# TropComplique/single-shot-detector

Hardware: AMD Instinct MI355X
Metric: images/sec at 896x640, MobileNet-v1 RetinaNet (whole hot path incl. decode + per-class NMS) (higher is better)
Workload: dtype f32

## Files before the change

single-shot-detector_amd/_lib.py:

```python
import ctypes
import os
import subprocess

_HERE = os.path.dirname(os.path.abspath(__file__))
_CSRC = os.path.join(_HERE, "csrc")
_SOURCES = ["abi.hip", "weights.hip", "plan.hip", "stages.hip", "igemm.hip", "igemm_lat.hip", "igemm16.hip", "dwpw_stream.hip", "sn_pw.hip", "front.hip",
            "elementwise.hip", "postprocess.hip", "loss.hip", "augment.hip", "update.hip", "train_head.hip", "wgrad.hip", "train_backbone.hip"]
_LIB_PATH = os.path.join(_CSRC, "libssd_hip.so")
_DIAG_PATH = os.path.join(_CSRC, "libssd_hip_diag.so")
_lib = None
_diag = False

HIPCC_FLAGS = ["--offload-arch=gfx950", "-O3", "-ffp-contract=off", "-fPIC", "-shared", "-std=c++17"]


class SsdError(RuntimeError):
    """A non-zero return code from libssd_hip.so (message from ssd_last_error())."""


def lib_path():
    return _LIB_PATH


def build(force=False, verbose=False, diag=False):
    srcs = [os.path.join(_CSRC, s) for s in _SOURCES]
    deps = srcs + [os.path.join(_CSRC, "ssd_internal.h"), os.path.join(_CSRC, "host.h"), os.path.join(_CSRC, "igemm_mfma16.h"),
                   os.path.join(_CSRC, "train_head.h"), os.path.join(_CSRC, "first_pixels.h"),
                   os.path.join(_HERE, "..", "include", "ssd_hip.h"),
                   os.path.join(_HERE, "..", "include", "ssd_hip_diag.h"), os.path.join(_CSRC, "exports.map")]
    target = _DIAG_PATH if diag else _LIB_PATH
    import hashlib
    hh = hashlib.sha256(" ".join(HIPCC_FLAGS + (["-DSSD_DIAG"] if diag else [])).encode())
    for d in deps:
        with open(d, "rb") as f:
            hh.update(f.read())
    digest = hh.hexdigest()
    stamp = target + ".sha"
    def fresh():
        if not (os.path.exists(target) and os.path.exists(stamp)):
            return False
        with open(stamp) as f:
            return f.read().strip() == digest
    if not force and fresh():
        return target
    import fcntl
    with open(os.path.join(_CSRC, ".build.lock"), "w") as lock:
        fcntl.flock(lock, fcntl.LOCK_EX)
        try:
            if not force and fresh():
                return target
            hipcc = os.environ.get("HIPCC", "/opt/rocm/bin/hipcc")
            tmp = "%s.tmp.%d" % (target, os.getpid())
            objdir = os.path.join(_CSRC, "build", "diag" if diag else "ship")
            os.makedirs(objdir, exist_ok=True)
            hdrs = deps[len(srcs):]
            cflags = [f for f in HIPCC_FLAGS if f != "-shared"] + (["-DSSD_DIAG"] if diag else [])
            jobs = []
            for src in srcs:
                obj = os.path.join(objdir, os.path.basename(src) + ".o")
                oh = hashlib.sha256(" ".join(cflags).encode())
                for d in [src] + hdrs:
                    with open(d, "rb") as f:
                        oh.update(f.read())
                ostamp, odig = obj + ".sha", oh.hexdigest()
                if force or not os.path.exists(obj) or not os.path.exists(ostamp) or open(ostamp).read().strip() != odig:
                    jobs.append(([hipcc] + cflags + ["-c", src, "-o", obj], ostamp, odig))
            if verbose:
                for j in jobs:
                    print(" ".join(j[0]))
            procs = [subprocess.Popen(j[0]) for j in jobs]
            rcs = [p.wait() for p in procs]
            if any(rcs):
                raise subprocess.CalledProcessError(max(rcs), "hipcc -c")
            for _cmd, ostamp, odig in jobs:
                with open(ostamp, "w") as f:
                    f.write(odig)
            objs = [os.path.join(objdir, os.path.basename(src) + ".o") for src in srcs]
            cmd = [hipcc, "--offload-arch=gfx950", "-shared", "-fPIC", "-Wl,--version-script=" + os.path.join(_CSRC, "exports.map"),
                   "-o", tmp] + objs
            if verbose:
                print(" ".join(cmd))
            subprocess.check_call(cmd)
            ctypes.CDLL(tmp)
            os.replace(tmp, target)
            with open(stamp, "w") as f:
                f.write(digest)
        finally:
            fcntl.flock(lock, fcntl.LOCK_UN)
    return target


_f = ctypes.POINTER(ctypes.c_float)
_i32p = ctypes.POINTER(ctypes.c_int32)
_vp = ctypes.c_void_p
_i = ctypes.c_int32


class SsdConfig(ctypes.Structure):
    _fields_ = [("backbone", ctypes.c_int32), ("depth_multiplier", ctypes.c_float),
                ("num_classes", ctypes.c_int32), ("score_threshold", ctypes.c_float),
                ("iou_threshold", ctypes.c_float), ("max_boxes_per_class", ctypes.c_int32),
                ("min_dimension", ctypes.c_int32), ("device", ctypes.c_int32)]


class SsdLossConfig(ctypes.Structure):
    _fields_ = [("alpha", ctypes.c_double), ("gamma", ctypes.c_float), ("positives_threshold", ctypes.c_float),
                ("negatives_threshold", ctypes.c_float), ("n_levels", ctypes.c_int32),
                ("anchors_per_level", ctypes.c_int64 * 8)]


class SsdUpdateTensor(ctypes.Structure):
    _fields_ = [("w", ctypes.c_void_p), ("grad", ctypes.c_void_p), ("m", ctypes.c_void_p), ("v", ctypes.c_void_p),
                ("ema", ctypes.c_void_p), ("count", ctypes.c_int64), ("decay", ctypes.c_int32), ("first_block", ctypes.c_int32)]


class SsdUpdateScalars(ctypes.Structure):
    _fields_ = [("alpha", ctypes.c_float), ("one_minus_beta1", ctypes.c_float), ("one_minus_beta2", ctypes.c_float),
                ("epsilon", ctypes.c_float), ("weight_decay", ctypes.c_float), ("one_minus_decay", ctypes.c_float)]


class SsdConvLevel(ctypes.Structure):
    _fields_ = [("H", ctypes.c_int32), ("W", ctypes.c_int32), ("x", ctypes.c_void_p), ("dy", ctypes.c_void_p), ("out", ctypes.c_void_p)]


class SsdBnLevel(ctypes.Structure):
    _fields_ = [("rows", ctypes.c_int64)] + [(n, ctypes.c_void_p) for n in (
        "x", "dy", "out", "gamma", "beta", "moving_mean", "moving_variance", "mean", "var", "invstd", "dgamma", "dbeta")]


SIGNATURES = {
    "ssd_create": (ctypes.c_int, [ctypes.POINTER(SsdConfig), ctypes.POINTER(_vp)]),
    "ssd_destroy": (None, [_vp]),
    "ssd_last_error": (ctypes.c_char_p, []),
    "ssd_load_weight": (ctypes.c_int, [_vp, ctypes.c_char_p, _f, ctypes.POINTER(ctypes.c_int64), _i]),
    "ssd_finalize": (ctypes.c_int, [_vp]),
    "ssd_forward": (ctypes.c_int, [_vp, _vp, _i, _i, _i, _vp, _vp, _vp, _vp, _vp]),
    "ssd_record_words": (ctypes.c_int32, [_vp]),
    "ssd_forward_records": (ctypes.c_int, [_vp, _vp, _i, _i, _i, _vp, _vp]),
    "ssd_forward_host": (ctypes.c_int, [_vp, _vp, _i, _i, _i, _vp, _vp]),
    "ssd_network_shape": (ctypes.c_int, [_vp, _i, _i, _i32p]),
    "ssd_forward_mixed": (ctypes.c_int, [_vp, _vp, _i, _i32p, ctypes.POINTER(ctypes.c_int64), _vp, _vp]),
    "ssd_forward_mixed_host": (ctypes.c_int, [_vp, ctypes.POINTER(ctypes.c_void_p), _i, _i32p, _vp, _vp]),
    "ssd_detect_host": (ctypes.c_int, [_vp, _vp, _i, _i, ctypes.c_float, _vp, _vp, _vp, _vp, _i, _i32p, _vp]),
    "ssd_get_tensor": (ctypes.c_int, [_vp, ctypes.c_char_p, _f, ctypes.c_int64, _i32p]),
    "ssd_get_tensor_dev": (ctypes.c_int, [_vp, ctypes.c_char_p, _vp, ctypes.c_int64, _i32p, _vp]),
    "ssd_plan_cache_stats": (ctypes.c_int, [_vp, ctypes.POINTER(ctypes.c_int64)]),
    "ssd_plan_cache_clear": (ctypes.c_int, [_vp]),
    "ssd_profile_enable": (ctypes.c_int, [_vp, _i]),
    "ssd_profile_read": (ctypes.c_int, [_vp, _i, ctypes.POINTER(ctypes.c_double),
                                        ctypes.POINTER(ctypes.c_int64),
                                        ctypes.POINTER(ctypes.c_double),
                                        ctypes.POINTER(ctypes.c_double)]),
    "ssd_profile_reset": (ctypes.c_int, [_vp]),
    "ssd_num_anchors": (ctypes.c_int32, [_i, _i]),
    "ssd_anchors": (ctypes.c_int, [_i, _i, _f]),
    "ssd_anchors_ex": (ctypes.c_int64, [_i, _i, _i, _i32p, ctypes.POINTER(ctypes.c_double), _i, ctypes.POINTER(ctypes.c_double),
                                        _i, ctypes.POINTER(ctypes.c_double), _f, ctypes.c_int64]),
    "ssd_conv2d": (ctypes.c_int, [_vp, _i, _i, _i, _i, _f, _i, _i, _i, _i, _i, _i, _f, _f, _f, _f,
                                  _vp, _i, _vp, _vp]),
    "ssd_conv2d_f16x3": (ctypes.c_int, [_vp, _i, _i, _i, _i, _f, _i, _i, _i, _i, _i, _i, _f, _f, _f, _f,
                                        _vp, _i, _vp, _vp]),
    "ssd_set_option": (ctypes.c_int, [_vp, ctypes.c_char_p, _i]),
    "ssd_get_option": (ctypes.c_int, [_vp, ctypes.c_char_p, _i32p]),
    "ssd_set_precision": (ctypes.c_int, [_vp, _i]),
    "ssd_get_precision": (ctypes.c_int, [_vp]),
    "ssd_status": (ctypes.c_int, [_vp, _i32p]),
    "ssd_depthwise3x3": (ctypes.c_int, [_vp, _i, _i, _i, _i, _f, _i, _i, _i, _i, _f, _f, _f, _i,
                                        _vp, _vp]),
    "ssd_dw_pw": (ctypes.c_int, [_vp, _i, _i, _i, _i, _f, _i, _f, _f, _f, _i, _f, _i, _f, _f, _f, _i, _vp, _vp]),
    "ssd_first_conv": (ctypes.c_int, [_vp, _i, _i, _i, _f, _i, _f, _f, _f, _i, _vp, _vp]),
    "ssd_front_block": (ctypes.c_int, [_vp, _i, _i, _i, _f, _i, _f, _f, _f, _i, _f, _f, _f, _f, _i, _f, _i, _f, _f, _f, _i, _vp, _vp]),
    "ssd_first_conv_maxpool": (ctypes.c_int, [_vp, _i, _i, _i, _f, _i, _f, _f, _f, _i, _vp, _vp]),
    "ssd_maxpool3x3s2": (ctypes.c_int, [_vp, _i, _i, _i, _i, _vp, _vp]),
    "ssd_concat_shuffle_split": (ctypes.c_int, [_vp, _vp, ctypes.c_int64, _i, _vp, _vp, _vp]),
    "ssd_shuffle_conv1x1": (ctypes.c_int, [_vp, _vp, ctypes.c_int64, _i, _f, _i, _f, _f, _f, _i, _vp, _vp]),
    "ssd_postprocess_workspace_bytes": (ctypes.c_size_t, [_i, _i, _i, _i]),
    "ssd_postprocess": (ctypes.c_int, [_vp, _vp, _vp, _i, _i, _i, ctypes.c_float, ctypes.c_float,
                                       _i, _f, _vp, _vp, _vp, _vp, _vp, ctypes.c_size_t, _vp]),
    "ssd_loss_workspace_bytes": (ctypes.c_size_t, [_i, _i, _i]),
    "ssd_training_targets": (ctypes.c_int, [_vp, _i, _vp, _vp, _vp, _i, _i, ctypes.POINTER(SsdLossConfig),
                                            _vp, _vp, _vp, _vp, ctypes.c_size_t, _vp]),
    "ssd_loss": (ctypes.c_int, [_vp, _vp, _vp, _i, _i, _i, _vp, _vp, _vp, _i, ctypes.POINTER(SsdLossConfig),
                                _vp, _vp, _vp, _vp, _vp, ctypes.c_size_t, _vp]),
    "ssd_loss_backward": (ctypes.c_int, [_vp, _vp, _i, _i, _i, _vp, _vp, _vp, _vp, _i, ctypes.POINTER(SsdLossConfig),
                                         _vp, _vp, _vp, _vp]),
    "ssd_augment": (ctypes.c_int, [_vp, _vp, _vp, _i, _i, _i, _i, _vp, _vp]),
    "ssd_train_update": (ctypes.c_int, [_vp, _vp, _i, ctypes.POINTER(SsdUpdateScalars), _vp]),
    "ssd_conv3x3_train_workspace_bytes": (ctypes.c_size_t, [ctypes.POINTER(SsdConvLevel), _i, _i, _i, _i]),
    "ssd_conv3x3_train_forward": (ctypes.c_int, [ctypes.POINTER(SsdConvLevel), _i, _i, _i, _i, _vp, _vp, _vp, ctypes.c_size_t, _vp]),
    "ssd_conv3x3_train_backward": (ctypes.c_int, [ctypes.POINTER(SsdConvLevel), _i, _i, _i, _i, _vp, _vp, _vp, _vp, ctypes.c_size_t, _vp]),
    "ssd_bn_relu_train_workspace_bytes": (ctypes.c_size_t, [ctypes.POINTER(SsdBnLevel), _i, _i]),
    "ssd_bn_relu_train_forward": (ctypes.c_int, [ctypes.POINTER(SsdBnLevel), _i, _i, _i, ctypes.c_float, ctypes.c_float, _vp,
                                                 ctypes.c_size_t, _vp]),
    "ssd_bn_relu_train_backward": (ctypes.c_int, [ctypes.POINTER(SsdBnLevel), _i, _i, _vp, ctypes.c_size_t, _vp]),
    "ssd_conv_train_workspace_bytes": (ctypes.c_size_t, [ctypes.POINTER(SsdConvLevel), _i, _i, _i, _i, _i, _i, _i]),
    "ssd_conv_train_forward": (ctypes.c_int, [ctypes.POINTER(SsdConvLevel), _i, _i, _i, _i, _i, _i, _vp, _vp, ctypes.POINTER(_vp), _vp,
                                              ctypes.c_size_t, _vp]),
    "ssd_conv_train_backward": (ctypes.c_int, [ctypes.POINTER(SsdConvLevel), _i, _i, _i, _i, _i, _i, _vp, _vp, _vp, _vp, ctypes.c_size_t, _vp]),
    "ssd_fpn_merge_backward": (ctypes.c_int, [_vp, _vp, _vp, _i, _i, _i, _i, _i, _vp, _vp]),
    "ssd_depthwise_train_forward": (ctypes.c_int, [_vp, _i, _i, _i, _i, _vp, _i, _vp, _vp]),
    "ssd_depthwise_train_workspace_bytes": (ctypes.c_size_t, [_i, _i, _i, _i, _i]),
    "ssd_depthwise_train_backward": (ctypes.c_int, [_vp, _vp, _i, _i, _i, _i, _vp, _i, _vp, _vp, _vp, ctypes.c_size_t, _vp]),
    "ssd_pointwise_train_workspace_bytes": (ctypes.c_size_t, [ctypes.POINTER(SsdConvLevel), _i, _i, _i, _i]),
    "ssd_pointwise_train_backward": (ctypes.c_int, [ctypes.POINTER(SsdConvLevel), _i, _i, _i, _i, _vp, _vp, _vp, ctypes.c_size_t, _vp]),
    "ssd_bn_act_train_forward": (ctypes.c_int, [ctypes.POINTER(SsdBnLevel), _i, _i, _i, _i, ctypes.c_float, ctypes.c_float, _vp,
                                                ctypes.c_size_t, _vp]),
    "ssd_bn_act_train_backward": (ctypes.c_int, [ctypes.POINTER(SsdBnLevel), _i, _i, _i, _vp, ctypes.c_size_t, _vp]),
    "ssd_first_conv_train_forward": (ctypes.c_int, [_vp, _i, _i, _i, _vp, _i, _vp, _vp]),
    "ssd_first_conv_train_workspace_bytes": (ctypes.c_size_t, [_i, _i, _i, _i]),
    "ssd_first_conv_train_backward": (ctypes.c_int, [_vp, _vp, _i, _i, _i, _i, _vp, _vp, ctypes.c_size_t, _vp]),
}


DIAG_SIGNATURES = {
    "ssd_bench_conv": (ctypes.c_int, [_i, _i, _i, _i, _i, _i, _i, _i, _i, _i,
                                      ctypes.POINTER(ctypes.c_double), ctypes.POINTER(ctypes.c_double)]),
    "ssd_bench_dwpw": (ctypes.c_int, [_i, _i, _i, _i, _i, _i, _i, _i, ctypes.POINTER(ctypes.c_double)]),
}


def use_diag():
    global _diag
    if _lib is not None and not _diag:
        raise RuntimeError("use_diag() after libssd_hip.so was loaded")
    _diag = True


def lib():
    global _lib
    if _lib is None:
        target = _DIAG_PATH if _diag else _LIB_PATH
        try:
            path = build(diag=_diag)
        except (FileNotFoundError, subprocess.CalledProcessError, OSError) as e:
            if not os.path.exists(target):
                raise RuntimeError("single-shot-detector_amd: %s is missing and cannot be built here (%r); there is no "
                                   "fallback" % (os.path.basename(target), e)) from e
            import warnings
            warnings.warn("single-shot-detector_amd: loading the existing %s without a freshness check (%r)"
                          % (os.path.basename(target), e))
            path = target
        _lib = ctypes.CDLL(path)
        sigs = dict(SIGNATURES, **DIAG_SIGNATURES) if _diag else SIGNATURES
        for name, (res, args) in sigs.items():
            fn = getattr(_lib, name)
            fn.restype = res
            fn.argtypes = args
    return _lib


def set_option(key, value, handle=None):
    check(lib().ssd_set_option(handle, key.encode(), int(value)))


def get_option(key, handle=None):
    v = ctypes.c_int32()
    check(lib().ssd_get_option(handle, key.encode(), ctypes.byref(v)))
    return v.value


def check(rc):
    if rc != 0:
        msg = lib().ssd_last_error()
        raise SsdError("libssd_hip error %d: %s" % (rc, msg.decode() if msg else "?"))
```

single-shot-detector_amd/csrc/abi.hip:

```cpp
#include "host.h"

#include <algorithm>
#include <cmath>
#include <cstdio>
#include <cstring>

static thread_local std::string g_err;
int ssd_fail(int code, const std::string &msg) { g_err = msg; return code; }
extern "C" const char *ssd_last_error(void) { return g_err.c_str(); }

static Options g_opts;
static std::mutex g_opts_mu;
static const char *const OPT_NAMES[OPT_COUNT] = {"streams", "h2d_chunks", "front_fuse", "fuse_dw", "backbone_split", "event_fence", "plan_cache_mb",
                                                 "igemm_tile", "igemm16", "igemm_96", "igemm_lat", "igemm_deep64", "lateral_split", "fpn_group", "fpn_p7_group",
                                                 "fpn_early_lat", "nsub", "nms_fast_max", "first_conv_px", "debug_sync"};
int ssd_opt_index(const char *key)
{
    for (int i = 0; i < OPT_COUNT; ++i)
        if (key && !strcmp(key, OPT_NAMES[i])) return i;
    return -1;
}
int ssd_opt(const ssd_handle *h, int key, int dflt)
{
    if (h && h->opts.v[key] != SSD_OPT_UNSET) return h->opts.v[key];
    const int g = g_opts.v[key];
    return g != SSD_OPT_UNSET ? g : dflt;
}
unsigned ssd_sync_event_flags(const ssd_handle *h)
{
    return hipEventDisableTiming | (ssd_opt(h, OPT_EVENT_FENCE, 0) ? 0u : (unsigned)hipEventDisableSystemFence);
}
int nms_fast_max(const ssd_handle *h)
{
    const int v = ssd_opt(h, OPT_NMS_FAST_MAX, -1);
    return v < 0 ? 0 : (v == 0 ? -1 : v);
}

static int make_handle_events(ssd_handle *h)
{
    if (h->ev_last) { (void)hipEventDestroy(h->ev_last); h->ev_last = nullptr; }
    HIPCHK(hipEventCreateWithFlags(&h->ev_last, ssd_sync_event_flags(h)));
    h->have_last = false;
    return SSD_OK;
}

extern "C" int ssd_set_option(ssd_handle *h, const char *key, int32_t value)
{
    const int k = ssd_opt_index(key);
    if (k < 0) return ssd_fail(SSD_ERR_INVALID, std::string("ssd_set_option: unknown option ") + (key ? key : "(null)"));
    if (k == OPT_IGEMM_TILE && !(value == SSD_OPT_UNSET || value == 0 || value == 64 || value == 128 || igemm_is_lat(value)))
        return ssd_fail(SSD_ERR_INVALID, "ssd_set_option: igemm_tile must be 0 (auto), 128, 64 or a wave tile of igemm_lat.hip (20 .. 27, 30)");
    if (k == OPT_PLAN_CACHE_MB && value < 0 && value != SSD_OPT_UNSET) return ssd_fail(SSD_ERR_INVALID, "ssd_set_option: plan_cache_mb must be >= 0");
    if (!h) {
        std::lock_guard<std::mutex> g(g_opts_mu);
        g_opts.v[k] = value;
        return SSD_OK;
    }
    std::lock_guard<std::mutex> g(h->mu);
    if (h->opts.v[k] == value) return SSD_OK;
    HIPCHK(hipSetDevice(h->cfg.device));
    if (k == OPT_PLAN_CACHE_MB) {
        h->opts.v[k] = value;
        return trim_plan_cache(h, h->cur);
    }
    HIPCHK(hipDeviceSynchronize());
    free_plans(h);
    h->opts.v[k] = value;
    if (k == OPT_EVENT_FENCE) SSDCHK(make_handle_events(h));
    return SSD_OK;
}

extern "C" int ssd_get_option(ssd_handle *h, const char *key, int32_t *value)
{
    const int k = ssd_opt_index(key);
    if (k < 0 || !value) return ssd_fail(SSD_ERR_INVALID, "ssd_get_option: unknown option or null argument");
    *value = ssd_opt(h, k, SSD_OPT_UNSET);
    return SSD_OK;
}

extern "C" int ssd_create(const ssd_config *cfg, ssd_handle **out)
{
    if (!cfg || !out) return ssd_fail(SSD_ERR_INVALID, "ssd_create: null argument");
    if (cfg->backbone != SSD_BACKBONE_MOBILENET && cfg->backbone != SSD_BACKBONE_SHUFFLENET)
        return ssd_fail(SSD_ERR_INVALID, "ssd_create: unknown backbone");
    if (cfg->num_classes < 1 || cfg->max_boxes_per_class < 1)
        return ssd_fail(SSD_ERR_INVALID, "ssd_create: num_classes and max_boxes_per_class must be >= 1");
    int ndev = 0;
    HIPCHK(hipGetDeviceCount(&ndev));
    if (cfg->device < 0 || cfg->device >= ndev) return ssd_fail(SSD_ERR_INVALID, "ssd_create: no such HIP device");
    HIPCHK(hipSetDevice(cfg->device));
    ssd_handle *h = new ssd_handle();
    h->cfg = *cfg;
    if (make_handle_events(h) != SSD_OK) {
        if (h->ev_last) (void)hipEventDestroy(h->ev_last);
        delete h;
        return ssd_fail(SSD_ERR_HIP, "ssd_create: cannot create events");
    }
    if (hipMalloc((void **)&h->flags_dev, sizeof(int)) != hipSuccess || hipMemset(h->flags_dev, 0, sizeof(int)) != hipSuccess) {
        delete h;
        return ssd_fail(SSD_ERR_HIP, "ssd_create: cannot allocate the status word");
    }
    if (const char *e = getenv("SSD_PRECISION")) {
        if (!strcmp(e, "f16x3")) h->precision = SSD_PRECISION_F16X3;
        else if (!strcmp(e, "f32")) h->precision = SSD_PRECISION_F32;
        else { (void)hipFree(h->flags_dev); delete h; return ssd_fail(SSD_ERR_INVALID, "SSD_PRECISION must be f32 or f16x3"); }
    }
    *out = h;
    return SSD_OK;
}

extern "C" int ssd_set_precision(ssd_handle *h, int32_t mode)
{
    if (!h || (mode != SSD_PRECISION_F32 && mode != SSD_PRECISION_F16X3)) return ssd_fail(SSD_ERR_INVALID, "ssd_set_precision: bad arguments");
    std::lock_guard<std::mutex> g(h->mu);
    if (mode == h->precision) return SSD_OK;
    HIPCHK(hipSetDevice(h->cfg.device));
    HIPCHK(hipDeviceSynchronize());
    free_plans(h);
    h->precision = mode;
    return SSD_OK;
}

extern "C" int ssd_get_precision(ssd_handle *h)
{
    if (!h) return SSD_ERR_INVALID;
    std::lock_guard<std::mutex> g(h->mu);
    return h->precision;
}

extern "C" int ssd_status(ssd_handle *h, int32_t *flags_out)
{
    if (!h || !flags_out) return ssd_fail(SSD_ERR_INVALID, "ssd_status: null argument");
    std::lock_guard<std::mutex> g(h->mu);
    HIPCHK(hipSetDevice(h->cfg.device));
    HIPCHK(hipDeviceSynchronize());
    int v = 0;
    HIPCHK(hipMemcpy(&v, h->flags_dev, sizeof(int), hipMemcpyDeviceToHost));
    if (v) HIPCHK(hipMemset(h->flags_dev, 0, sizeof(int)));
    *flags_out = v;
    return SSD_OK;
}

extern "C" void ssd_destroy(ssd_handle *h)
{
    if (!h) return;
    (void)hipSetDevice(h->cfg.device);
    (void)hipDeviceSynchronize();
    for (auto &e : h->evs) { (void)hipEventDestroy(e.a); (void)hipEventDestroy(e.b); }
    for (auto r : h->ref_evs) (void)hipEventDestroy(r);
    for (auto r : h->ev_pool) (void)hipEventDestroy(r);
    free_plans(h);
    if (h->ev_last) (void)hipEventDestroy(h->ev_last);
    if (h->ev_stage) (void)hipEventDestroy(h->ev_stage);
    if (h->stage_pin) (void)hipHostFree(h->stage_pin);
    if (h->stage_dev) (void)hipFree(h->stage_dev);
    if (h->flags_dev) (void)hipFree(h->flags_dev);
    h->wpool.free_all();
    delete h;
}

extern "C" int ssd_load_weight(ssd_handle *h, const char *name, const float *host, const int64_t *shape, int32_t ndim)
{
    if (!h || !name || !host || !shape || ndim < 1 || ndim > 4) return ssd_fail(SSD_ERR_INVALID, "ssd_load_weight: bad arguments");
    std::lock_guard<std::mutex> g(h->mu);
    if (h->finalized) return ssd_fail(SSD_ERR_STATE, "ssd_load_weight after ssd_finalize");
    Tensor t;
    int64_t n = 1;
    for (int i = 0; i < ndim; ++i) {
        if (shape[i] < 1) return ssd_fail(SSD_ERR_INVALID, "ssd_load_weight: non-positive dimension");
        t.shape.push_back(shape[i]);
        n *= shape[i];
    }
    t.data.assign(host, host + n);
    h->vars[name] = std::move(t);
    return SSD_OK;
}

extern "C" int ssd_finalize(ssd_handle *h)
{
    if (!h) return ssd_fail(SSD_ERR_INVALID, "ssd_finalize: null handle");
    std::lock_guard<std::mutex> g(h->mu);
    if (h->finalized) return ssd_fail(SSD_ERR_STATE, "ssd_finalize called twice");
    HIPCHK(hipSetDevice(h->cfg.device));
    SSDCHK(finalize_weights(h));
    h->vars.clear();
    h->finalized = true;
    return SSD_OK;
}

struct MixedSel { const MixedCall *mx; int netH, netW; long long max_bytes; };
struct Outputs { float *boxes; int32_t *labels; float *scores; int32_t *num_boxes; long long stride; };

static int forward_locked(ssd_handle *h, const uint8_t *images_dev, int32_t B, int32_t H, int32_t W, const Outputs &o, hipStream_t s,
                          const MixedSel *ms = nullptr)
{
    HIPCHK(hipSetDevice(h->cfg.device));
    if (ms) SSDCHK(select_plans_net(h, B, ms->netH, ms->netW, 0, ms->max_bytes));
    else SSDCHK(select_plans(h, B, H, W));
    if (h->have_last && h->last_stream != s) {
        if (!h->multi_stream) {
            h->multi_stream = true;
            hipStreamCaptureStatus cs = hipStreamCaptureStatusNone;
            const bool known = hipStreamIsCapturing(h->last_stream, &cs) == hipSuccess;
            if (known && cs == hipStreamCaptureStatusNone && hipEventRecord(h->ev_last, h->last_stream) == hipSuccess)
                HIPCHK(hipStreamWaitEvent(s, h->ev_last, 0));
            else { (void)hipGetLastError(); HIPCHK(hipDeviceSynchronize()); }
        } else {
            hipStreamCaptureStatus cs = hipStreamCaptureStatusNone;
            if (hipStreamIsCapturing(s, &cs) != hipSuccess) { (void)hipGetLastError(); cs = hipStreamCaptureStatusNone; }
            if (cs != hipStreamCaptureStatusNone)
                return ssd_fail(SSD_ERR_STATE, "ssd_forward: this handle's previous forward ran on another stream; a capturing stream cannot wait "
                                               "for it -- synchronise that stream (or use one handle per captured stream) before capturing");
            HIPCHK(hipStreamWaitEvent(s, h->ev_last, 0));
        }
        h->have_last = false;
    }
    h->mixed = ms ? ms->mx : nullptr;
    const int rc = enqueue_forward(h, images_dev, o.boxes, o.labels, o.scores, o.num_boxes, o.stride, s);
    h->mixed = nullptr;
    return rc;
}

static int forward_checked_locked(ssd_handle *h, const uint8_t *images_dev, int32_t B, int32_t H, int32_t W, const Outputs &o, void *stream,
                                  const MixedSel *ms = nullptr)
{
    if (!h->finalized) return ssd_fail(SSD_ERR_STATE, "ssd_forward before ssd_finalize");
    if (B < 1 || H < 1 || W < 1 || h->cfg.min_dimension < 128 || h->cfg.min_dimension % 128)
        return ssd_fail(SSD_ERR_INVALID, "ssd_forward: B, H, W must be positive and min_dimension a multiple of 128 (pipeline.py:152)");
    {
        const ResizeDims rd = resize_dims(H, W, h->cfg.min_dimension, 128);
        if ((long long)(rd.nh + rd.ph) * (rd.nw + rd.pw) > (1LL << 26))
            return ssd_fail(SSD_ERR_INVALID, "ssd_forward: aspect ratio too extreme (resized image exceeds 64 Mpixel)");
    }
    hipStream_t s = (hipStream_t)stream;
    const int rc = forward_locked(h, images_dev, B, H, W, o, s, ms);
    if (rc == SSD_OK) {
        hipStreamCaptureStatus cs = hipStreamCaptureStatusNone;
        if (hipStreamIsCapturing(s, &cs) != hipSuccess) { (void)hipGetLastError(); cs = hipStreamCaptureStatusNone; }
        if (cs == hipStreamCaptureStatusNone) {
            h->last_stream = s;
            h->have_last = true;
            if (h->multi_stream) HIPCHK(hipEventRecord(h->ev_last, s));
        }
    }
    return rc;
}

static int forward_checked(ssd_handle *h, const uint8_t *images_dev, int32_t B, int32_t H, int32_t W, const Outputs &o, void *stream)
{
    if (!h || !images_dev || !o.boxes || !o.labels || !o.scores || !o.num_boxes)
        return ssd_fail(SSD_ERR_INVALID, "ssd_forward: null argument");
    std::lock_guard<std::mutex> g(h->mu);
    return forward_checked_locked(h, images_dev, B, H, W, o, stream);
}

extern "C" int ssd_forward(ssd_handle *h, const uint8_t *images_dev, int32_t B, int32_t H, int32_t W, float *boxes_dev,
                           int32_t *labels_dev, float *scores_dev, int32_t *num_boxes_dev, void *stream)
{
    return forward_checked(h, images_dev, B, H, W, {boxes_dev, labels_dev, scores_dev, num_boxes_dev, 0}, stream);
}

extern "C" int32_t ssd_record_words(const ssd_handle *h)
{
    return h ? 6 * h->cfg.num_classes * h->cfg.max_boxes_per_class + 1 : 0;
}

static Outputs record_outputs(const ssd_handle *h, void *records)
{
    const long long T = (long long)h->cfg.num_classes * h->cfg.max_boxes_per_class;
    int32_t *r = (int32_t *)records;
    return {(float *)r, r + 5 * T, (float *)(r + 4 * T), r + 6 * T, 6 * T + 1};
}

extern "C" int ssd_forward_records(ssd_handle *h, const uint8_t *images_dev, int32_t B, int32_t H, int32_t W, void *records_dev, void *stream)
{
    if (!h || !records_dev) return ssd_fail(SSD_ERR_INVALID, "ssd_forward_records: null argument");
    if ((reinterpret_cast<uintptr_t>(records_dev) & 3) != 0) return ssd_fail(SSD_ERR_INVALID, "ssd_forward_records: records must be 4-byte aligned");
    return forward_checked(h, images_dev, B, H, W, record_outputs(h, records_dev), stream);
}

static int stage_acquire(ssd_handle *h)
{
    if (!h->stage_busy) return SSD_OK;
    const hipError_t e = h->stage_by_event && h->ev_stage ? hipEventSynchronize(h->ev_stage) : hipStreamSynchronize(h->stage_stream);
    if (e != hipSuccess) { (void)hipGetLastError(); HIPCHK(hipDeviceSynchronize()); }
    h->stage_busy = false;
    return SSD_OK;
}
static int stage_release(ssd_handle *h, hipStream_t s, bool by_event)
{
    if (by_event) {
        if (!h->ev_stage) HIPCHK(hipEventCreateWithFlags(&h->ev_stage, hipEventDisableTiming));
        hipStreamCaptureStatus cs = hipStreamCaptureStatusNone;
        if (hipStreamIsCapturing(s, &cs) != hipSuccess) { (void)hipGetLastError(); cs = hipStreamCaptureStatusNone; }
        if (cs == hipStreamCaptureStatusNone) HIPCHK(hipEventRecord(h->ev_stage, s));
        else by_event = false;
    }
    h->stage_stream = s;
    h->stage_stream_set = true;
    h->stage_by_event = by_event;
    h->stage_busy = true;
    return SSD_OK;
}

static int grow_stage(ssd_handle *h, size_t bytes)
{
    if (bytes <= h->stage_bytes) return SSD_OK;
    size_t cap = (size_t)2 << 20;
    while (cap < bytes) cap <<= 1;
    HIPCHK(hipDeviceSynchronize());
    if (h->stage_pin) { (void)hipHostFree(h->stage_pin); h->stage_pin = nullptr; }
    if (h->stage_dev) { (void)hipFree(h->stage_dev); h->stage_dev = nullptr; }
    h->stage_bytes = 0;
    HIPCHK(hipHostMalloc((void **)&h->stage_pin, cap + 256, hipHostMallocDefault));
    HIPCHK(hipMalloc((void **)&h->stage_dev, cap + 256));
    h->stage_bytes = cap;
    return SSD_OK;
}

static int stage_begin(ssd_handle *h, hipStream_t s, size_t bytes)
{
    SSDCHK(stage_acquire(h));
    if (h->stage_stream_set && h->stage_stream != s) {
        if (hipStreamSynchronize(h->stage_stream) != hipSuccess) { (void)hipGetLastError(); HIPCHK(hipDeviceSynchronize()); }
    }
    return grow_stage(h, bytes);
}

static int forward_host_impl(ssd_handle *h, const uint8_t *images_host, int32_t B, int32_t H, int32_t W, void *records, void *stream, bool stage_event)
{
    if (!h || !images_host || !records) return ssd_fail(SSD_ERR_INVALID, "ssd_forward_host: null argument");
    if (B < 1 || H < 1 || W < 1) return ssd_fail(SSD_ERR_INVALID, "ssd_forward_host: B, H, W must be positive");
    if ((reinterpret_cast<uintptr_t>(records) & 3) != 0) return ssd_fail(SSD_ERR_INVALID, "ssd_forward_host: records must be 4-byte aligned");
    std::lock_guard<std::mutex> g(h->mu);
    HIPCHK(hipSetDevice(h->cfg.device));
    hipStream_t s = (hipStream_t)stream;
    const size_t bytes = (size_t)B * H * W * 3;
    SSDCHK(stage_begin(h, s, bytes));
    int nchunk = ssd_opt(h, OPT_H2D_CHUNKS, 2);
    if (nchunk < 1) nchunk = 1;
    if (nchunk > 16) nchunk = 16;
    if (bytes < ((size_t)1 << 20)) nchunk = 1;
    const size_t step = ((bytes + nchunk - 1) / nchunk + 4095) & ~(size_t)4095;
    for (size_t lo = 0; lo < bytes; lo += step) {
        const size_t n = bytes - lo < step ? bytes - lo : step;
        memcpy(h->stage_pin + lo, images_host + lo, n);
        HIPCHK(hipMemcpyAsync(h->stage_dev + lo, h->stage_pin + lo, n, hipMemcpyHostToDevice, s));
    }
    SSDCHK(stage_release(h, s, stage_event));
    return forward_checked_locked(h, h->stage_dev, B, H, W, record_outputs(h, records), stream);
}

extern "C" int ssd_forward_host(ssd_handle *h, const uint8_t *images_host, int32_t B, int32_t H, int32_t W, void *records, void *stream)
{
    return forward_host_impl(h, images_host, B, H, W, records, stream, true);
}

static int prepare_mixed(ssd_handle *h, int32_t B, const int32_t *hw, const int64_t *offsets, MixedSel *ms, const char *who)
{
    if (B < 1 || B > SSD_MIXED_MAX)
        return ssd_fail(SSD_ERR_INVALID, std::string(who) + ": 1 .. " + std::to_string(SSD_MIXED_MAX) + " frames per mixed-size batch");
    if (h->cfg.min_dimension < 128 || h->cfg.min_dimension % 128) return ssd_fail(SSD_ERR_INVALID, std::string(who) + ": min_dimension must be a multiple of 128");
    MixedCall &mc = h->mixed_store;
    long long off = 0, max_bytes = 0;
    ms->mx = &mc; ms->netH = ms->netW = 0;
    for (int b = 0; b < B; ++b) {
        const int H = hw[2 * b], W = hw[2 * b + 1];
        if (H < 1 || W < 1) return ssd_fail(SSD_ERR_INVALID, std::string(who) + ": frame sizes must be positive");
        const ResizeDims rd = resize_dims(H, W, h->cfg.min_dimension, 128);
        const int nH = rd.nh + rd.ph, nW = rd.nw + rd.pw;
        if ((long long)nH * nW > (1LL << 26)) return ssd_fail(SSD_ERR_INVALID, std::string(who) + ": aspect ratio too extreme (resized image exceeds 64 Mpixel)");
        if (b == 0) { ms->netH = nH; ms->netW = nW; }
        else if (nH != ms->netH || nW != ms->netW)
            return ssd_fail(SSD_ERR_INVALID, std::string(who) + ": frame " + std::to_string(b) + " (" + std::to_string(H) + " x " + std::to_string(W) + ") resizes to " +
                                             std::to_string(nH) + " x " + std::to_string(nW) + ", frame 0 to " + std::to_string(ms->netH) + " x " +
                                             std::to_string(ms->netW) + ": the frames of one batch must share the network shape (group them by ssd_network_shape)");
        const long long bytes = (long long)H * W * 3;
        const long long o = offsets ? offsets[b] : off;
        if (o < 0 || o + bytes >= (1LL << 31)) return ssd_fail(SSD_ERR_INVALID, std::string(who) + ": the frames of a batch must lie within 2 GiB of the base pointer");
        FrameGeom &g = mc.geom.f[b];
        g.off = (unsigned)o; g.srcH = H; g.srcW = W; g.nh = rd.nh; g.nw = rd.nw;
        g.hs = (float)H / (float)rd.nh; g.ws = (float)W / (float)rd.nw;
        mc.scaler[b][0] = rd.box_scaler[0]; mc.scaler[b][1] = rd.box_scaler[1];
        off = o + ((bytes + 15) & ~15LL);
        max_bytes = bytes > max_bytes ? bytes : max_bytes;
    }
    ms->max_bytes = max_bytes;
    return SSD_OK;
}

extern "C" int ssd_network_shape(ssd_handle *h, int32_t height, int32_t width, int32_t *net_hw)
{
    if (!h || !net_hw || height < 1 || width < 1) return ssd_fail(SSD_ERR_INVALID, "ssd_network_shape: bad arguments");
    if (h->cfg.min_dimension < 128 || h->cfg.min_dimension % 128) return ssd_fail(SSD_ERR_INVALID, "ssd_network_shape: min_dimension must be a multiple of 128");
    const ResizeDims rd = resize_dims(height, width, h->cfg.min_dimension, 128);
    net_hw[0] = rd.nh + rd.ph; net_hw[1] = rd.nw + rd.pw;
    return SSD_OK;
}

extern "C" int ssd_forward_mixed(ssd_handle *h, const uint8_t *images_dev, int32_t B, const int32_t *hw_host, const int64_t *offsets_host,
                                 void *records_dev, void *stream)
{
    if (!h || !images_dev || !hw_host || !records_dev) return ssd_fail(SSD_ERR_INVALID, "ssd_forward_mixed: null argument");
    if ((reinterpret_cast<uintptr_t>(records_dev) & 3) != 0) return ssd_fail(SSD_ERR_INVALID, "ssd_forward_mixed: records must be 4-byte aligned");
    std::lock_guard<std::mutex> g(h->mu);
    MixedSel ms;
    SSDCHK(prepare_mixed(h, B, hw_host, offsets_host, &ms, "ssd_forward_mixed"));
    return forward_checked_locked(h, images_dev, B, hw_host[0], hw_host[1], record_outputs(h, records_dev), stream, &ms);
}

extern "C" int ssd_forward_mixed_host(ssd_handle *h, const uint8_t *const *frames_host, int32_t B, const int32_t *hw_host, void *records, void *stream)
{
    if (!h || !frames_host || !hw_host || !records) return ssd_fail(SSD_ERR_INVALID, "ssd_forward_mixed_host: null argument");
    if ((reinterpret_cast<uintptr_t>(records) & 3) != 0) return ssd_fail(SSD_ERR_INVALID, "ssd_forward_mixed_host: records must be 4-byte aligned");
    std::lock_guard<std::mutex> g(h->mu);
    MixedSel ms;
    SSDCHK(prepare_mixed(h, B, hw_host, nullptr, &ms, "ssd_forward_mixed_host"));
    for (int b = 0; b < B; ++b)
        if (!frames_host[b]) return ssd_fail(SSD_ERR_INVALID, "ssd_forward_mixed_host: null frame pointer");
    HIPCHK(hipSetDevice(h->cfg.device));
    hipStream_t s = (hipStream_t)stream;
    const MixedCall &mc = h->mixed_store;
    const size_t bytes = (size_t)mc.geom.f[B - 1].off + (size_t)hw_host[2 * (B - 1)] * hw_host[2 * (B - 1) + 1] * 3;
    SSDCHK(stage_begin(h, s, bytes));
    for (int b = 0; b < B; ++b) {
        const size_t n = (size_t)hw_host[2 * b] * hw_host[2 * b + 1] * 3, lo = mc.geom.f[b].off;
        memcpy(h->stage_pin + lo, frames_host[b], n);
        HIPCHK(hipMemcpyAsync(h->stage_dev + lo, h->stage_pin + lo, n, hipMemcpyHostToDevice, s));
    }
    SSDCHK(stage_release(h, s, true));
    return forward_checked_locked(h, h->stage_dev, B, hw_host[0], hw_host[1], record_outputs(h, records), stream, &ms);
}

extern "C" int ssd_detect_host(ssd_handle *h, const uint8_t *image_host, int32_t H, int32_t W, float score_threshold, void *record,
                               float *boxes_out, int32_t *labels_out, float *scores_out, int32_t capacity, int32_t *n_out, void *stream)
{
    if (!h || !record || !boxes_out || !labels_out || !scores_out || !n_out || capacity < 0) return ssd_fail(SSD_ERR_INVALID, "ssd_detect_host: bad arguments");
    {
        std::lock_guard<std::mutex> g(h->mu);
        bool known = false;
        for (int i = 0; i < h->n_rec_ok; ++i) known = known || h->detect_rec_ok[i] == record;
        if (!known) {
            HIPCHK(hipSetDevice(h->cfg.device));
            hipPointerAttribute_t at;
            memset(&at, 0, sizeof(at));
            const hipError_t pe = hipPointerGetAttributes(&at, record);
            if (pe != hipSuccess) (void)hipGetLastError();
            const bool host_visible = pe == hipSuccess && (at.type == hipMemoryTypeHost || at.type == hipMemoryTypeManaged || at.isManaged);
            if (!host_visible)
                return ssd_fail(SSD_ERR_INVALID, "ssd_detect_host: `record` must be pinned (hipHostMalloc / hipHostRegister) or managed host memory -- "
                                                 "a device pointer or pageable memory cannot be written by the GPU and read by this call");
            h->detect_rec_ok[h->n_rec_ok < 8 ? h->n_rec_ok++ : (h->rec_ok_next++ & 7)] = record;
        }
    }
    int rc = forward_host_impl(h, image_host, 1, H, W, record, stream, false);
    if (rc != SSD_OK) return rc;
    HIPCHK(hipStreamSynchronize((hipStream_t)stream));
    const Outputs r = record_outputs(h, record);
    const long long T = (r.stride - 1) / 6;
    const int32_t n = *r.num_boxes;
    if (n < 0 || n > T) return ssd_fail(SSD_ERR_STATE, "ssd_detect_host: the record's num_boxes is out of range (is `record` host-visible memory?)");
    int32_t k = 0;
    for (int32_t i = 0; i < n; ++i)
        if (r.scores[i] > score_threshold) {
            if (k >= capacity) return ssd_fail(SSD_ERR_INVALID, "ssd_detect_host: capacity too small");
            memcpy(boxes_out + 4 * (size_t)k, r.boxes + 4 * (size_t)i, 16);
            labels_out[k] = r.labels[i];
            scores_out[k] = r.scores[i];
            ++k;
        }
    *n_out = k;
    return SSD_OK;
}

extern "C" int ssd_get_tensor(ssd_handle *h, const char *name, float *dst, int64_t cap, int32_t *dims)
{
    if (!h || !name || !dst || !dims) return ssd_fail(SSD_ERR_INVALID, "ssd_get_tensor: null argument");
    std::lock_guard<std::mutex> g(h->mu);
    if (!h->cur) return ssd_fail(SSD_ERR_STATE, "ssd_get_tensor before ssd_forward");
    HIPCHK(hipSetDevice(h->cfg.device));
    HIPCHK(hipDeviceSynchronize());
    long long done = 0;
    int Btot = 0;
    for (Plan *pl : h->cur->plans) {
        auto it = pl->retained.find(name);
        if (it == pl->retained.end()) return ssd_fail(SSD_ERR_INVALID, std::string("ssd_get_tensor: unknown tensor ") + name);
        const Retained &r = it->second;
        const long long rows = (long long)r.B * r.H * r.W;
        if (cap < done + rows * r.C) return ssd_fail(SSD_ERR_INVALID, "ssd_get_tensor: destination too small");
        std::vector<float> tmp((size_t)rows * r.Cp);
        HIPCHK(hipMemcpy(tmp.data(), r.dev, tmp.size() * sizeof(float), hipMemcpyDeviceToHost));
        for (long long q = 0; q < rows; ++q)
            for (int c = 0; c < r.C; ++c) {
                const int pc = !r.permuted ? c : (r.split > 0 ? twopart_phys(c, r.split, r.Cp / 2) : ssd_phys_of_logical(c));
                if (r.fmt) {
                    const _Float16 *row = (const _Float16 *)&tmp[q * r.Cp];
                    dst[done + q * r.C + c] = (float)row[(pc >> 3) * 16 + (pc & 7)] + (float)row[(pc >> 3) * 16 + 8 + (pc & 7)];
                } else {
                    dst[done + q * r.C + c] = tmp[q * r.Cp + pc];
                }
            }
        done += rows * r.C;
        Btot += r.B;
        dims[1] = r.H; dims[2] = r.W; dims[3] = r.C;
    }
    dims[0] = Btot;
    return SSD_OK;
}

extern "C" int ssd_get_tensor_dev(ssd_handle *h, const char *name, float *dst_dev, int64_t cap, int32_t *dims, void *stream)
{
    if (!h || !name || !dst_dev || !dims) return ssd_fail(SSD_ERR_INVALID, "ssd_get_tensor_dev: null argument");
    std::lock_guard<std::mutex> g(h->mu);
    if (!h->cur) return ssd_fail(SSD_ERR_STATE, "ssd_get_tensor_dev before ssd_forward");
    HIPCHK(hipSetDevice(h->cfg.device));
    long long done = 0;
    int Btot = 0;
    for (Plan *pl : h->cur->plans) {
        auto it = pl->retained.find(name);
        if (it == pl->retained.end()) return ssd_fail(SSD_ERR_INVALID, std::string("ssd_get_tensor_dev: unknown tensor ") + name);
        const Retained &r = it->second;
        const long long rows = (long long)r.B * r.H * r.W;
        if (cap < done + rows * r.C) return ssd_fail(SSD_ERR_INVALID, "ssd_get_tensor_dev: destination too small");
        if (r.permuted) HIPCHK(launch_permute_channels(r.dev, rows, r.C, r.Cp, r.fmt ? 2 : 0, dst_dev + done, (hipStream_t)stream, r.fmt ? 0 : r.split));
        else HIPCHK(hipMemcpyAsync(dst_dev + done, r.dev, (size_t)rows * r.C * sizeof(float), hipMemcpyDeviceToDevice, (hipStream_t)stream));
        done += rows * r.C;
        Btot += r.B;
        dims[1] = r.H; dims[2] = r.W; dims[3] = r.C;
    }
    dims[0] = Btot;
    return SSD_OK;
}

extern "C" int ssd_plan_cache_stats(ssd_handle *h, int64_t *out)
{
    if (!h || !out) return ssd_fail(SSD_ERR_INVALID, "ssd_plan_cache_stats: null argument");
    std::lock_guard<std::mutex> g(h->mu);
    HIPCHK(hipSetDevice(h->cfg.device));
    size_t total = 0;
    for (const PlanSet *ps : h->cache) total += ps->bytes;
    out[0] = (int64_t)h->cache.size();
    out[1] = (int64_t)total;
    out[2] = (int64_t)plan_cache_limit_bytes(h);
    out[3] = h->cache_hits; out[4] = h->cache_misses; out[5] = h->cache_evictions;
    out[6] = h->cur ? h->cur->key.netH : 0;
    out[7] = h->cur ? h->cur->key.netW : 0;
    return SSD_OK;
}

extern "C" int ssd_plan_cache_clear(ssd_handle *h)
{
    if (!h) return ssd_fail(SSD_ERR_INVALID, "ssd_plan_cache_clear: null handle");
    std::lock_guard<std::mutex> g(h->mu);
    HIPCHK(hipSetDevice(h->cfg.device));
    HIPCHK(hipDeviceSynchronize());
    h->cache_evictions += (long long)h->cache.size();
    free_plans(h);
    h->n_rec_ok = 0;
    return SSD_OK;
}

extern "C" int ssd_profile_enable(ssd_handle *h, int32_t on)
{
    if (!h) return ssd_fail(SSD_ERR_INVALID, "null handle");
    std::lock_guard<std::mutex> g(h->mu);
    h->profiling = on != 0;
    return SSD_OK;
}

static int drain_events(ssd_handle *h)
{
    std::vector<std::vector<std::pair<float, float>>> iv(SSD_NCLS);
    int cur_fwd = -1;
    auto flush = [&]() {
        for (int c = 0; c < SSD_NCLS; ++c) {
            auto &v = iv[c];
            std::sort(v.begin(), v.end());
            float lo = 0, hi = -1;
            for (auto &p : v) {
                if (hi < 0) { lo = p.first; hi = p.second; }
                else if (p.first <= hi) { if (p.second > hi) hi = p.second; }
                else { h->acc_ms[c] += hi - lo; lo = p.first; hi = p.second; }
            }
            if (hi >= 0) h->acc_ms[c] += hi - lo;
            v.clear();
        }
    };
    for (auto &e : h->evs) {
        HIPCHK(hipEventSynchronize(e.b));
        if (e.fwd != cur_fwd) { flush(); cur_fwd = e.fwd; }
        float t0 = 0, t1 = 0;
        if (e.fwd >= 0 && e.fwd < (int)h->ref_evs.size()) {
            HIPCHK(hipEventElapsedTime(&t0, h->ref_evs[e.fwd], e.a));
            HIPCHK(hipEventElapsedTime(&t1, h->ref_evs[e.fwd], e.b));
        } else {
            HIPCHK(hipEventElapsedTime(&t1, e.a, e.b));
        }
        iv[e.cls].push_back({t0, t1});
        h->ev_pool.push_back(e.a);
        h->ev_pool.push_back(e.b);
    }
    flush();
    h->evs.clear();
    for (auto r : h->ref_evs) h->ev_pool.push_back(r);
    h->ref_evs.clear();
    return SSD_OK;
}

extern "C" int ssd_profile_read(ssd_handle *h, int32_t cls, double *total_ms, int64_t *launches, double *flops, double *bytes)
{
    if (!h || cls < 0 || cls >= SSD_NCLS) return ssd_fail(SSD_ERR_INVALID, "ssd_profile_read: bad arguments");
    std::lock_guard<std::mutex> g(h->mu);
    SSDCHK(drain_events(h));
    if (total_ms) *total_ms = h->acc_ms[cls];
    if (launches) *launches = h->acc_n[cls];
    if (flops) *flops = h->acc_flops[cls];
    if (bytes) *bytes = h->acc_bytes[cls];
    return SSD_OK;
}

extern "C" int ssd_profile_reset(ssd_handle *h)
{
    if (!h) return ssd_fail(SSD_ERR_INVALID, "null handle");
    std::lock_guard<std::mutex> g(h->mu);
    SSDCHK(drain_events(h));
    for (int i = 0; i < SSD_NCLS; ++i) { h->acc_ms[i] = h->acc_flops[i] = h->acc_bytes[i] = 0; h->acc_n[i] = 0; }
    return SSD_OK;
}
```

single-shot-detector_amd/csrc/host.h:

```cpp
#pragma once
#include "../../include/ssd_hip.h"
#include "ssd_internal.h"

#include <climits>
#include <functional>
#include <map>
#include <mutex>
#include <string>
#include <vector>

int ssd_fail(int code, const std::string &msg);
#define HIPCHK(expr)                                                                         \
    do {                                                                                     \
        hipError_t e_ = (expr);                                                              \
        if (e_ != hipSuccess)                                                                \
            return ssd_fail(SSD_ERR_HIP, std::string(#expr) + ": " + hipGetErrorString(e_)); \
    } while (0)
#define SSDCHK(expr)                                                                         \
    do {                                                                                     \
        int r_ = (expr);                                                                     \
        if (r_ != SSD_OK) return r_;                                                         \
    } while (0)

enum SsdOpt {
    OPT_STREAMS = 0,
    OPT_H2D_CHUNKS,
    OPT_FRONT_FUSE,
    OPT_FUSE_DW,
    OPT_BACKBONE_SPLIT,
    OPT_EVENT_FENCE,
    OPT_PLAN_CACHE_MB,
    OPT_IGEMM_TILE,
    OPT_IGEMM16,
    OPT_IGEMM_96,
    OPT_IGEMM_LAT,
    OPT_IGEMM_DEEP64,
    OPT_LATERAL_SPLIT,
    OPT_FPN_GROUP,
    OPT_FPN_P7_GROUP,
    OPT_FPN_EARLY_LAT,
    OPT_NSUB,
    OPT_NMS_FAST_MAX,
    OPT_FIRST_CONV_PX,
    OPT_DEBUG_SYNC,
    OPT_COUNT
};
#define SSD_OPT_UNSET INT_MIN
struct Options { int v[OPT_COUNT]; Options() { for (int &x : v) x = SSD_OPT_UNSET; } };
int ssd_opt(const struct ssd_handle *h, int key, int dflt);
int ssd_opt_index(const char *key);
unsigned ssd_sync_event_flags(const struct ssd_handle *h);

struct Tensor {
    std::vector<int64_t> shape;
    std::vector<float> data;
};

struct DevPool {
    std::vector<void *> ptrs;
    size_t bytes = 0;
    int alloc(void **out, size_t nbytes)
    {
        HIPCHK(hipMalloc(out, nbytes + 256));
        ptrs.push_back(*out);
        bytes += nbytes + 256;
        return SSD_OK;
    }
    template <class T> int upload(T **out, const std::vector<T> &v)
    {
        void *p = nullptr;
        SSDCHK(alloc(&p, v.size() * sizeof(T)));
        if (!v.empty()) HIPCHK(hipMemcpy(p, v.data(), v.size() * sizeof(T), hipMemcpyHostToDevice));
        *out = (T *)p;
        return SSD_OK;
    }
    void free_all()
    {
        for (void *p : ptrs) (void)hipFree(p);
        ptrs.clear();
        bytes = 0;
    }
};

static inline int round_up(int v, int m) { return (v + m - 1) / m * m; }

std::vector<int> phys_map(int C, int Cp);
std::vector<int> ident_map(int C, int Cp);
std::vector<int> twopart_map(int D, int Dp);
static inline int twopart_phys(int c, int D, int Dp) { return c < D ? ssd_phys_of_logical(c) : Dp + ssd_phys_of_logical(c - D); }

struct BnHost { std::vector<float> mean, sf, beta; };

struct ConvW {
    float *wt = nullptr, *mean = nullptr, *sf = nullptr, *beta = nullptr, *bias = nullptr;
    float *wlat = nullptr;
    float *wt16 = nullptr;
    float *wt16w = nullptr;
    int CoutPad16 = 0;
    float scale16 = 1.0f;
    int CinP = 0, CoutP = 0, CoutPad = 0, taps = 1, tile = IGEMM_128x128;
    int Cin_l = 0, Cout_l = 0;
};

struct DwW {
    float *w = nullptr, *mean = nullptr, *sf = nullptr, *beta = nullptr;
    float *pack = nullptr;
    int Cp = 0;
};

#define SSD_NCLS 8
#define SSD_FUSE_DW_DEFAULT 0xfu
#define SSD_FUSE_SHUFFLE_DEFAULT true
#ifdef SSD_DIAG
extern int g_force_tile;
extern long long *g_dbg_ts;
#else
static constexpr int g_force_tile = -1;
static constexpr long long *g_dbg_ts = nullptr;
#endif

std::vector<float> permute_rows(const float *w, int rows, int C, const std::vector<int> &map);
BnHost permute_bn(const float *mean, const float *sf, const float *beta, const std::vector<int> &map,
                  BnHost o = BnHost());
void conv_geometry(const struct ssd_handle *h, int taps, int CinP, int CoutP, int Cin_l, int Cout_l, ConvW &cw);
int pack_conv(const struct ssd_handle *h, DevPool &pool, const float *w, int k, int Cin_l, int Cout_l, const std::vector<int> &inmap,
              const std::vector<int> &outmap, ConvW &cw);
int upload_bn(DevPool &pool, const BnHost &b, ConvW &cw);
int upload_dw(DevPool &pool, const std::vector<float> &w, const BnHost &b, DwW &d);
int pack_dw(DevPool &pool, const std::vector<float> &w9, const BnHost &b, DwW &d);
int finalize_weights(struct ssd_handle *h);

struct Op {
    int cls;
    int stream = 0;
    std::vector<int> deps;
    hipEvent_t done = nullptr;
    double flops, bytes;
    std::function<hipError_t(hipStream_t)> run;
};

struct LevelDesc {
    int H, W, OH, OW;
    long long in_off, out_off, out_bstride;
    int out_rstride, param_off;
    long long res_off;
    long long wt_off = 0;
    int stride = 0, pad = -1;
};

struct ConvIO {
    const float *in = nullptr;
    float *out = nullptr;
    float *out2 = nullptr;
    const float *res = nullptr;
    int in_fmt = 0, out_fmt = 0, res_fmt = 0;
    int *flags = nullptr;
};
Op make_conv_op(const struct ssd_handle *h, const ConvW &cw, const ConvIO &io, int B, int stride, int pad, int act,
                const std::vector<LevelDesc> &lv, bool dense, unsigned *scan_bits = nullptr, float scan_lo = 0.0f,
                bool *scan_marked = nullptr);
Op make_dw_op(const DwW &d, const float *in, int B, int H, int W, int stride, int act, float *out, int Cl, int out16 = 0,
              int *flags = nullptr);
bool dwpws_eligible(const DwW &d, const ConvW &cw, int B, int H, int W, int stride);
Op make_dwpws_op(const DwW &d, const ConvW &cw, const float *in, int B, int H, int W, int stride, int dact, int act,
                 float *out, int out_rs = 0 );
Op make_pw_gather_op(const ConvW &cw, const float *base, long long base_bytes, const int *src, int rs, long long M, int act, float *out);
LevelDesc dense_level(int H, int W, int OH, int OW, int CoutP, long long in_off = 0, long long out_off = 0,
                      int param_off = 0, long long res_off = 0);
float conservative_logit_bound(float thr);
int nms_fast_max(const struct ssd_handle *h);

struct ResizeDims { int nh, nw, ph, pw; float box_scaler[4]; };
ResizeDims resize_dims(int height, int width, int min_dimension, int divisor);
extern const int A_STRIDES[5];
extern const int MB_STRIDE[13];

struct Retained { const float *dev; int B, H, W, C, Cp; bool permuted; int fmt = 0;
                  int split = 0;  };

struct EvPair { hipEvent_t a, b; int cls; int fwd; };

struct Plan {
    int B = 0, img0 = 0, N = 0;
    DevPool pool;
    std::vector<Op> ops;
    PostArgs post;
    std::map<std::string, Retained> retained;
    hipStream_t s_aux = nullptr;
    hipStream_t s_bb[2] = {nullptr, nullptr};
    hipEvent_t ev_join = nullptr, ev_begin = nullptr;
    bool need_begin = false;
};

struct SrcGeom { int srcH = 0, srcW = 0, nh = 0, nw = 0; float box_scaler[4] = {1, 1, 1, 1}; };

struct MixedCall { MixedGeom geom; float scaler[SSD_MIXED_MAX][2]; };

struct PlanKey {
    int B = 0, netH = 0, netW = 0, ident = 0, nsub = 0;
    bool operator==(const PlanKey &o) const { return B == o.B && netH == o.netH && netW == o.netW && ident == o.ident && nsub == o.nsub; }
};
struct PlanSet {
    PlanKey key;
    std::vector<Plan *> plans;
    size_t bytes = 0;
    unsigned long long last_use = 0;
};

struct ssd_handle {
    ssd_config cfg;
    std::mutex mu;
    Options opts;
    std::map<std::string, Tensor> vars;
    bool finalized = false;
    DevPool wpool;
    DwW first;
    int firstCp = 0, firstAct = SSD_ACT_RELU6;
    std::vector<DwW> dw;
    std::vector<ConvW> pw;
    ConvW lat[3], pconv[5];
    ConvW pgroup;
    ConvW tower[2][4], final_[2];
    int c_ch[3] = {0, 0, 0};
    int c_split[3] = {0, 0, 0};
    struct SnStage { int pw = 0, dw = 0, units = 0; };
    SnStage sn_stage[3];
    int precision = SSD_PRECISION_F32;
    int *flags_dev = nullptr;
    std::vector<PlanSet *> cache;
    PlanSet *cur = nullptr;
    unsigned long long use_clock = 0;
    long long cache_hits = 0, cache_misses = 0, cache_evictions = 0;
    const uint8_t *cur_images = nullptr;
    SrcGeom src;
    const MixedCall *mixed = nullptr;
    MixedCall mixed_store;
    hipStream_t last_stream = nullptr;
    bool have_last = false;
    bool multi_stream = false;
    hipEvent_t ev_last = nullptr;
    const void *detect_rec_ok[8] = {nullptr};
    int n_rec_ok = 0, rec_ok_next = 0;
    uint8_t *stage_pin = nullptr, *stage_dev = nullptr;
    size_t stage_bytes = 0;
    hipStream_t stage_stream = nullptr;
    bool stage_busy = false, stage_stream_set = false;
    bool stage_by_event = false;
    hipEvent_t ev_stage = nullptr;
    bool profiling = false;
    std::vector<EvPair> evs;
    std::vector<hipEvent_t> ref_evs;
    std::vector<hipEvent_t> ev_pool;
    double acc_ms[SSD_NCLS] = {0}, acc_flops[SSD_NCLS] = {0}, acc_bytes[SSD_NCLS] = {0};
    long long acc_n[SSD_NCLS] = {0};
};

void free_plans(ssd_handle *h);
int select_plans(ssd_handle *h, int B, int H, int W);
int select_plans_net(ssd_handle *h, int B, int netH, int netW, int ident, long long max_src_bytes);
int trim_plan_cache(ssd_handle *h, const PlanSet *keep);
size_t plan_cache_limit_bytes(const ssd_handle *h);
int enqueue_forward(ssd_handle *h, const uint8_t *images_dev, float *boxes_dev, int32_t *labels_dev, float *scores_dev,
                    int32_t *num_boxes_dev, long long out_stride, hipStream_t s);
```

single-shot-detector_amd/csrc/plan.hip:

```cpp
#include "host.h"
#include <chrono>

#include <algorithm>
#include <cmath>
#include <cstdio>
#include <cstring>

Op make_conv_op(const ssd_handle *h, const ConvW &cw, const ConvIO &io, int B, int stride, int pad, int act,
                const std::vector<LevelDesc> &lv, bool dense, unsigned *scan_bits, float scan_lo, bool *scan_marked)
{
    const float *in = io.in, *res = io.res;
    float *out = io.out, *out2 = io.out2;
    const int in_fmt = io.in_fmt, out_fmt = io.out_fmt, res_fmt = io.res_fmt;
    int *flags = io.flags;
    IgemmArgs a;
    memset(&a, 0, sizeof(a));
    a.in = in; a.wt = in_fmt ? cw.wt16 : cw.wt; a.out = out; a.out2 = out2;
    a.wt_lat = in_fmt ? nullptr : cw.wlat;
    a.in_fmt = in_fmt; a.out_fmt = out_fmt; a.res_fmt = res ? res_fmt : 0;
    a.acc_scale = in_fmt ? cw.scale16 : 1.0f;
    a.flags = flags;
    a.mean = cw.mean; a.sf = cw.sf; a.beta = cw.beta; a.bias = cw.bias; a.res = res;
    a.B = B; a.Cin = cw.CinP; a.Cout = cw.CoutP; a.CoutPad = cw.CoutPad; a.taps = cw.taps;
    a.stride = stride; a.pad = pad; a.act = act;
// ... 450 lines not shown
}

struct StageGeo { int ch, cw, oh, ow, D, Dp, n_units; long long tbytes[2], toff[2], soff, total; };

static void sn_stage_geo(const ssd_handle *h, int H, int W, const int nb[2], StageGeo geo[3])
{
    int ch = H / 2 / 2, cw = W / 2 / 2;
    for (int st = 0; st < 3; ++st) {
        StageGeo &g = geo[st];
        g.ch = ch; g.cw = cw; g.oh = ch / 2; g.ow = cw / 2; g.n_units = h->sn_stage[st].units;
        const ConvW &after = h->pw[h->sn_stage[st].pw + 1];
        g.Dp = after.CoutP; g.D = after.Cout_l;
        long long off = 0;
        for (int c = 0; c < 2; ++c) {
            g.tbytes[c] = (long long)nb[c] * g.oh * g.ow * g.Dp * 4;
            g.toff[c] = off;
            off += g.tbytes[c] * g.n_units;
        }
        g.soff = off;
        g.total = off + (long long)(nb[0] + nb[1]) * g.oh * g.ow * 2 * g.Dp * 4;
        ch = g.oh; cw = g.ow;
    }
}

static int shufflenet_chain(Builder &b, const StageGeo *geo, float *const *stage, int c, int b0, int nb, float *C5, std::vector<Op> &ops)
{
    ssd_handle *const h = b.h;
    const int H = b.H, W = b.W, h2 = H / 2, w2 = W / 2, h4 = h2 / 2, w4 = w2 / 2, fc = h->firstCp, first_img = b.img0 + b0;
    bool sn_fuse = SSD_FUSE_SHUFFLE_DEFAULT;
    if (ssd_opt(h, OPT_FUSE_DW, -1) >= 0) sn_fuse = ssd_opt(h, OPT_FUSE_DW, -1) != 0;
    float *MP, *MID = nullptr;
    SSDCHK(b.falloc(&MP, (long long)nb * h4 * w4 * fc));
    auto pair = [&](const DwW &d, const ConvW &cw, const float *in, int hh, int ww, int stride, float *out, int out_rs) -> int {
        if (sn_fuse && dwpws_eligible(d, cw, nb, hh, ww, stride)) {
            ops.push_back(make_dwpws_op(d, cw, in, nb, hh, ww, stride, SSD_ACT_NONE, SSD_ACT_RELU, out, out_rs));
            return SSD_OK;
        }
        if (!MID) SSDCHK(b.falloc(&MID, (long long)nb * h4 * w4 * std::max(fc, 32)));
        const int oh = hh / stride, ow = ww / stride;
        if ((long long)nb * oh * ow * d.Cp > (long long)nb * h4 * w4 * std::max(fc, 32)) return ssd_fail(SSD_ERR_INVALID, "ssd_forward: depthwise scratch too small");
        ops.push_back(make_dw_op(d, in, nb, hh, ww, stride, SSD_ACT_NONE, MID, cw.Cin_l));
        LevelDesc lv = dense_level(oh, ow, oh, ow, cw.CoutP);
        lv.out_rstride = out_rs > 0 ? out_rs : cw.CoutP;
        lv.out_bstride = (long long)oh * ow * lv.out_rstride;
        ops.push_back(make_conv_op(h, cw, {MID, out}, nb, 1, 0, SSD_ACT_RELU, {lv}, true));
        return SSD_OK;
    };
    {
        const DwW f = h->first;
        const int act = h->firstAct;
        const FusedFront pool = [nb, H, W, f, act, MP](const uint8_t *img, const int *src, const MixedGeom *mixed, int first, hipStream_t s) {
            return launch_front_pool(img, nb, H, W, f.w, f.Cp, f.mean, f.sf, f.beta, act, MP, s, src, mixed, first);
        };
        if (front_fuse(h, b.ident && h->first.mean && front_pool_supports(b.B, H, W, fc))) {
            Op op;
            op.cls = 3;
            op.flops = 2.0 * 27 * (double)nb * h2 * w2 * 24;
            op.bytes = (double)nb * H * W * 3 + (double)nb * h4 * w4 * 24 * 4.0;
            op.run = [pool, h, first_img, H, W](hipStream_t s) { return pool(h->cur_images + (size_t)first_img * H * W * 3, nullptr, nullptr, 0, s); };
            ops.push_back(op);
        } else {
            float *F;
            SSDCHK(b.falloc(&F, (long long)nb * h2 * w2 * fc));
            const bool rt = front_fuse(h, !b.ident && h->first.mean && front_pool_supports(nb, H, W, fc));
            const FirstLayer fl = first_layer_op(b, first_img, nb, 24, rt ? pool : FusedFront(), F);
            ops.push_back(fl.op);
            Op mp;
            mp.cls = 5; mp.flops = 0;
            mp.bytes = ((double)nb * h2 * w2 + (double)nb * h4 * w4) * 24 * 4.0;
            const std::function<bool()> fused_now = fl.fused_now;
            mp.run = [fused_now, F, nb, h2, w2, fc, MP](hipStream_t s) { return fused_now() ? hipSuccess : launch_maxpool(F, nb, h2, w2, fc, MP, s); };
            ops.push_back(mp);
        }
    }
    const float *cur = MP;
    for (int st = 0; st < 3; ++st) {
        const StageGeo &g = geo[st];
        const ConvW *pw = &h->pw[h->sn_stage[st].pw];
        const DwW *dw = &h->dw[h->sn_stage[st].dw];
        const ConvW &before = pw[0], &after = pw[1], &after2 = pw[2];
        const DwW &d1 = dw[0], &d2 = dw[1];
        pw += 3; dw += 2;
        const int D = g.D, Dp = g.Dp, n_units = g.n_units;
        const long long rows = (long long)nb * g.oh * g.ow;
        float *t1, *U;
        SSDCHK(b.falloc(&t1, (long long)nb * g.ch * g.cw * before.CoutP));
        SSDCHK(b.falloc(&U, rows * Dp));
        float *sb = stage[st];
        auto tensor_off = [&](int p) { return g.toff[c] + (long long)p * g.tbytes[c]; };
        float *S_chain = sb + g.soff / 4 + (long long)b0 * g.oh * g.ow * 2 * Dp;
        struct Src { int prod, col; };
        std::vector<Src> x(D), y(D);
        for (int d = 0; d < D; ++d) { x[d] = Src{0, d}; y[d] = Src{1, d}; }
        auto table = [&](const std::vector<Src> &v) {
            std::vector<int> t(Dp, -1);
            for (int d = 0; d < D; ++d) t[ssd_phys_of_logical(d)] = (int)(tensor_off(v[d].prod) + (long long)ssd_phys_of_logical(v[d].col) * 4);
            return t;
        };
        std::vector<const int *> src_dev(n_units + 1, nullptr);
        for (int j = 2; j <= n_units; ++j) {
            std::vector<Src> z(2 * D);
            for (int d = 0; d < D; ++d) { z[2 * d] = x[d]; z[2 * d + 1] = y[d]; }
            std::vector<Src> xin(z.begin(), z.begin() + D);
            int *dv;
            SSDCHK(b.pl.pool.upload(&dv, table(xin)));
            src_dev[j] = dv;
            for (int d = 0; d < D; ++d) { x[d] = Src{j, d}; y[d] = z[D + d]; }
        }
        int *ysrc;
        SSDCHK(b.pl.pool.upload(&ysrc, table(y)));
        ops.push_back(make_conv_op(h, before, {cur, t1}, nb, 1, 0, SSD_ACT_RELU, {dense_level(g.ch, g.cw, g.ch, g.cw, before.CoutP)}, true));
        SSDCHK(pair(d1, after, t1, g.ch, g.cw, 2, sb + tensor_off(1) / 4, 0));
        SSDCHK(pair(d2, after2, cur, g.ch, g.cw, 2, sb + tensor_off(0) / 4, 0));
        for (int j = 2; j <= n_units; ++j, pw += 2, dw += 1) {
            const ConvW &b2 = pw[0], &a2 = pw[1];
            const DwW &dd = dw[0];
            if (b2.CinP != Dp || b2.taps != 1 || !b2.mean || b2.bias || !pw_gather_supports(b2.CinP, b2.CoutP, rows, Dp * 4, g.total, rows * b2.CoutP * 4))
                return ssd_fail(SSD_ERR_INVALID, "ssd_forward: a ShuffleNet unit's conv1x1_before is not a shape of the gathering kernel (sn_pw.hip)");
#ifdef SSD_DIAG
            if (const char *e = getenv("SSD_ABL_SKIP_PWG")) { if ((atoi(e) >> st) & 1) goto skip_before; }
#endif
            ops.push_back(make_pw_gather_op(b2, sb, g.total, src_dev[j], Dp * 4, rows, SSD_ACT_RELU, U));
#ifdef SSD_DIAG
        skip_before:
#endif
            if (j < n_units) SSDCHK(pair(dd, a2, U, g.oh, g.ow, 1, sb + tensor_off(j) / 4, 0));
            else SSDCHK(pair(dd, a2, U, g.oh, g.ow, 1, S_chain, 2 * Dp));
        }
        {
            Op gop;
            gop.cls = 5; gop.flops = 0; gop.bytes = 2.0 * rows * D * 4.0;
            const int rs = Dp * 4, ors = 2 * Dp;
            float *ydst = S_chain + Dp;
            gop.run = [sb, ysrc, rs, rows, Dp, ydst, ors](hipStream_t s) { return launch_gather_rows(sb, ysrc, rs, rows, Dp, ydst, ors, s); };
            ops.push_back(gop);
        }
        cur = S_chain;
    }
    const StageGeo &g2 = geo[2];
    const ConvW &c5w = h->pw.back();
    ConvIO io{cur, C5 + (long long)b0 * g2.oh * g2.ow * c5w.CoutP};
    io.out_fmt = b.X16; io.flags = b.FL;
    ops.push_back(make_conv_op(h, c5w, io, nb, 1, 0, SSD_ACT_RELU, {dense_level(g2.oh, g2.ow, g2.oh, g2.ow, c5w.CoutP)}, true));
    return SSD_OK;
}

static int shufflenet_backbone(Builder &b, Backbone &bb)
{
    ssd_handle *h = b.h;
    const int B = b.B;
    const int nchain = backbone_chains(h, B, 2);
    const int nb_of[2] = {nchain == 2 ? B / 2 : B, nchain == 2 ? B - B / 2 : 0};
    StageGeo geo[3];
    sn_stage_geo(h, b.H, b.W, nb_of, geo);
    for (const StageGeo &g : geo)
        if (g.total >= (1LL << 31)) return ssd_fail(SSD_ERR_INVALID, "ssd_forward: ShuffleNet stage allocation past 2 GiB (sub-batch split failed)");
    float *stage[3];
    for (int st = 0; st < 3; ++st) SSDCHK(b.falloc(&stage[st], geo[st].total / 4));
    const StageGeo &g2 = geo[2];
    const ConvW &c5w = h->pw.back();
    SSDCHK(b.falloc(&bb.C5, (long long)B * g2.oh * g2.ow * c5w.CoutP));
    std::vector<Op> chain_ops[2];
    for (int c = 0; c < nchain; ++c) SSDCHK(shufflenet_chain(b, geo, stage, c, c == 0 ? 0 : nb_of[0], nb_of[c], bb.C5, chain_ops[c]));
    for (int st = 0; st < 2; ++st) {
        float *S = stage[st] + geo[st].soff / 4;
        if (st == 0) bb.C3 = S; else bb.C4 = S;
        b.pl.retained[st == 0 ? "c3" : "c4"] = Retained{S, B, geo[st].oh, geo[st].ow, 2 * geo[st].D, 2 * geo[st].Dp, true, 0, geo[st].D};
    }
    b.pl.retained["c5"] = Retained{bb.C5, B, g2.oh, g2.ow, c5w.Cout_l, c5w.CoutP, true, b.X16};
    interleave_chains(b.pl, chain_ops, nchain, bb);
    return SSD_OK;
}

struct Fpn {
    Pyr py;
    float *P;
    int id_p3, id_p4, id_p7;
};

static LevelDesc pyr_level(const Pyr &py, int in, int out)
{
    LevelDesc d = dense_level(py.h[in], py.w[in], py.h[out], py.w[out], 256);
    d.out_off = py.off[out];
    return d;
}

static int fpn(Builder &b, const Backbone &bb, Fpn &f)
{
    ssd_handle *h = b.h;
    const int B = b.B, X16 = b.X16;
    f.py = make_pyr(B, b.H, b.W, 256);
    const Pyr &py = f.py;
    float *P, *X5, *X4, *X3, *T6;
    SSDCHK(b.falloc(&P, py.total));
    SSDCHK(b.falloc(&X5, (long long)B * py.h[2] * py.w[2] * 256));
    SSDCHK(b.falloc(&X4, (long long)B * py.h[1] * py.w[1] * 256));
    SSDCHK(b.falloc(&X3, (long long)B * py.h[0] * py.w[0] * 256));
    SSDCHK(b.falloc(&T6, (long long)B * py.h[3] * py.w[3] * 256));
    f.P = P;
    auto lvl = [&](int l) { return dense_level(py.h[l], py.w[l], py.h[l], py.w[l], 256); };
    const int id_c5 = bb.last[0] >= 0 ? bb.last[0] : (int)b.pl.ops.size() - 1;
    bool grouped = false;
    if (!X16 && h->pgroup.wt) {
        const long long b64 = (((long long)B * py.h[0] * py.w[0] + 63) / 64) * (256 / 64);
        grouped = b64 <= 640;
        const int pin = ssd_opt(h, OPT_FPN_GROUP, -1);
        if (pin >= 0) grouped = pin != 0;
    }
    const bool swap67 = grouped && B <= 2;
    const bool p7grouped = swap67 && ssd_opt(h, OPT_FPN_P7_GROUP, 1) != 0;
    const int s_lat = swap67 ? 2 : 0;
    bool early = swap67 && !X16 && bb.id_c4 >= 0;
    { const int pin = ssd_opt(h, OPT_FPN_EARLY_LAT, -1); if (pin >= 0) early = early && pin != 0; }
    float *L4T = nullptr;
    if (early) {
        SSDCHK(b.falloc(&L4T, (long long)B * py.h[1] * py.w[1] * 256));
        b.push(b.conv(h->lat[0], {bb.C3, X3}, 1, 0, SSD_ACT_NONE, {lvl(0)}), s_lat, {bb.id_c4});
        b.push(b.conv(h->lat[1], {bb.C4, L4T}, 1, 0, SSD_ACT_NONE, {lvl(1)}), s_lat);
    }
    std::vector<int> l5_deps;
    for (int c = 1; c < 4; ++c) if (bb.last[c] >= 0) l5_deps.push_back(bb.last[c]);
    if (swap67) l5_deps.push_back(id_c5);
    const int id_l5 = b.push(b.conv(h->lat[2], b.io16(bb.C5, X5), 1, 0, SSD_ACT_NONE, {lvl(2)}), s_lat, l5_deps);
    std::vector<int> p6_deps = {id_c5};
    for (int c = 1; c < 4; ++c) if (c != 2 && bb.last[c] >= 0) p6_deps.push_back(bb.last[c]);
    {
        ConvIO io = b.io16(bb.C5, P);
        io.out2 = T6 - py.off[3];
        b.push(b.conv(h->pconv[3], io, 2, 1, SSD_ACT_RELU, {pyr_level(py, 2, 3)}), swap67 ? 0 : 2, p6_deps);
    }
    f.id_p7 = p7grouped ? -1 : b.push(b.conv(h->pconv[4], b.io16(T6, P), 2, 1, SSD_ACT_RELU, {pyr_level(py, 3, 4)}), swap67 ? 0 : 2);
    if (!grouped)
        b.push(b.conv(h->pconv[2], b.io16(X5, P), 1, 1, SSD_ACT_RELU, {pyr_level(py, 2, 2)}), 1, {id_l5});
    int LF = X16 && h->lat[1].tile == IGEMM_128x128 && h->lat[0].tile == IGEMM_128x128 ? 2 : 0;
    if (!ssd_opt(h, OPT_LATERAL_SPLIT, 1)) LF = 0;
    auto lateral = [&](const ConvW &cw, const float *c, float *x, const float *up, int l) {
        ConvIO io = b.io16(c, x);
        io.in_fmt = LF; io.res = up; io.res_fmt = X16;
        return b.conv(cw, io, 1, 0, SSD_ACT_NONE, {lvl(l)});
    };
    int id_l4, id_merge = -1;
    if (early) {
        Op m;
        m.cls = 5; m.flops = 0;
        m.bytes = ((double)B * py.h[0] * py.w[0] * 2 + (double)B * py.h[1] * py.w[1] * 2 + (double)B * py.h[2] * py.w[2]) * 256 * 4.0;
        const int mh = py.h[0], mw = py.w[0];
        m.run = [X5, L4T, X4, X3, B, mh, mw](hipStream_t s) { return launch_fpn_merge(X5, L4T, X4, X3, B, mh, mw, 256, s); };
        id_l4 = id_merge = b.push(m, s_lat);
    } else {
        id_l4 = b.push(lateral(h->lat[1], bb.C4, X4, X5, 1), s_lat);
    }
    if (!grouped) f.id_p4 = b.push(b.conv(h->pconv[1], b.io16(X4, P), 1, 1, SSD_ACT_RELU, {pyr_level(py, 1, 1)}), 1, {id_l4});
    const int id_l3 = early ? id_merge : b.push(lateral(h->lat[0], bb.C3, X3, X4, 0), s_lat);
    if (!grouped) {
        f.id_p3 = b.push(b.conv(h->pconv[0], b.io16(X3, P), 1, 1, SSD_ACT_RELU, {pyr_level(py, 0, 0)}), 0);
    } else {
        const ConvW &g = h->pgroup;
        const float *xin[3] = {X3, X4, X5};
        std::vector<LevelDesc> lv3;
        for (int l = 0; l < 3; ++l) {
            LevelDesc d = pyr_level(py, l, l);
            d.in_off = xin[l] - X3;
            d.param_off = l * g.CoutP;
            d.wt_off = (long long)l * g.taps * g.CoutPad * g.CinP;
            lv3.push_back(d);
        }
        if (p7grouped) {
            LevelDesc d = pyr_level(py, 3, 4);
            d.in_off = T6 - X3;
            d.param_off = 3 * g.CoutP;
            d.wt_off = (long long)3 * g.taps * g.CoutPad * g.CinP;
            d.stride = 2; d.pad = 1;
            lv3.push_back(d);
        }
        std::vector<int> gdeps;
        if (swap67) gdeps.push_back(id_l3);
        f.id_p3 = f.id_p4 = b.push(b.conv(g, {X3, P}, 1, 1, SSD_ACT_RELU, lv3), 0, gdeps);
        if (p7grouped) f.id_p7 = f.id_p3;
    }
    for (int l = 0; l < 5; ++l) {
        char nm[8];
        snprintf(nm, sizeof nm, "p%d", l + 3);
        b.pl.retained[nm] = Retained{P + py.off[l], B, py.h[l], py.w[l], 256, 256, true, X16};
    }
    return SSD_OK;
}

static int heads(Builder &b, const Backbone &bb, const Fpn &f)
{
    ssd_handle *h = b.h;
    Plan &pl = b.pl;
    const Pyr &py = f.py;
    const int B = b.B, C = h->cfg.num_classes, A = 6;
    long long N = 0, aoff[5];
    for (int l = 0; l < 5; ++l) { aoff[l] = N; N += (long long)py.h[l] * py.w[l] * A; }
    pl.N = (int)N;
    float *logits, *codes;
    SSDCHK(b.falloc(&logits, (long long)B * N * C));
    SSDCHK(b.falloc(&codes, (long long)B * N * 4));
    std::vector<float> anc((size_t)N * 4);
    SSDCHK(ssd_anchors(b.H, b.W, anc.data()));
    float *anc_dev;
    SSDCHK(pl.pool.upload(&anc_dev, anc));
    float *TAB[2][2];
    unsigned char *keys_home = nullptr;
    {
        const size_t slot = scratch_slot((size_t)py.total * sizeof(float));
        unsigned char *tb = bb.scratch;
        size_t tb_bytes = bb.scratch_bytes;
        if (!bb.scratch || 4 * slot > bb.scratch_bytes) {
            SSDCHK(pl.pool.alloc((void **)&tb, 4 * slot));
            tb_bytes = 4 * slot;
        }
        for (int t = 0; t < 2; ++t)
            for (int k = 0; k < 2; ++k) TAB[t][k] = (float *)(tb + (size_t)(2 * t + k) * slot);
        if (post_keys_bytes(B, (int)N, C) <= tb_bytes) keys_home = tb;
    }
    void *ws;
    const size_t wsb = post_workspace_bytes(B, (int)N, C, h->cfg.max_boxes_per_class, keys_home == nullptr);
    SSDCHK(pl.pool.alloc(&ws, wsb));
    PostArgs &p = pl.post;
    memset(&p, 0, sizeof(p));
    p.logits = logits; p.codes = codes; p.anchors = anc_dev;
    p.B = B; p.N = (int)N; p.C = C;
    p.score_thr = h->cfg.score_threshold; p.iou_thr = h->cfg.iou_threshold;
    p.max_per_class = h->cfg.max_boxes_per_class;
    p.fast_max = nms_fast_max(h);
    for (int k = 0; k < 4; ++k) p.box_scaler[k] = 1.0f;
    post_carve(p, ws, keys_home);
    HIPCHK(hipMemset(p.scan_bits, 0, post_scan_bitmap_bytes(B, (int)N, C)));
    HIPCHK(hipMemset(p.counts, 0, (size_t)B * C * sizeof(int)));
    p.self_clean = 1;
    std::vector<Op> tower_ops[2];
    bool all_marked = true;
    for (int t = 0; t < 2; ++t) {
        const float *in = f.P;
        int cur = 0;
        for (int i = 0; i < 4; ++i) {
            std::vector<LevelDesc> lv;
            for (int l = 0; l < 5; ++l) lv.push_back(dense_level(py.h[l], py.w[l], py.h[l], py.w[l], 256, py.off[l], py.off[l], l * 256));
            tower_ops[t].push_back(b.conv(h->tower[t][i], b.io16(in, TAB[t][cur]), 1, 1, SSD_ACT_RELU, lv));
            in = TAB[t][cur];
            cur ^= 1;
        }
        const int per = t == 0 ? 4 : C;
        const bool can_mark = t == 1 && ((long long)N * C) % 8 == 0 && (6 * C) % 8 == 0;
        std::vector<LevelDesc> lv;
        for (int l = 0; l < 5; ++l) {
            LevelDesc d = dense_level(py.h[l], py.w[l], py.h[l], py.w[l], 0, py.off[l]);
            d.out_off = aoff[l] * per;
            d.out_bstride = N * per;
            d.out_rstride = A * per;
            d.param_off = 0;
            lv.push_back(d);
        }
        ConvIO io = b.io16(in, t == 0 ? codes : logits);
        io.out_fmt = 0;
        bool marked = false;
        Op fop = make_conv_op(h, h->final_[t], io, B, 1, 1, SSD_ACT_NONE, lv, false, can_mark ? p.scan_bits : nullptr,
                              conservative_logit_bound(h->cfg.score_threshold), &marked);
        if (t == 1) all_marked = all_marked && marked;
        tower_ops[t].push_back(fop);
    }
    p.scan_fused = all_marked ? 1 : 0;
    for (size_t i = 0; i < tower_ops[0].size(); ++i)
        for (int t = 1; t >= 0; --t) {
            std::vector<int> deps;
            if (i == 0) { deps.push_back(t == 0 ? f.id_p4 : f.id_p3); deps.push_back(f.id_p7); }
            b.push(tower_ops[t][i], t, deps);
        }
    pl.retained["encoded_boxes"] = Retained{codes, B, 1, (int)N, 4, 4, false};
    pl.retained["class_predictions"] = Retained{logits, B, 1, (int)N, C, C, false};
    return SSD_OK;
}

static int build_plan(ssd_handle *h, Plan &pl, int B, int H, int W, bool ident, int img0)
{
    pl.B = B;
    pl.img0 = img0;
    Builder b{h, pl, B, H, W, ident, img0, h->precision == SSD_PRECISION_F16X3 ? 1 : 0, h->flags_dev};
    Backbone bb;
    SSDCHK(h->cfg.backbone == SSD_BACKBONE_MOBILENET ? mobilenet_backbone(b, bb) : shufflenet_backbone(b, bb));
    Fpn f;
    SSDCHK(fpn(b, bb, f));
    SSDCHK(heads(b, bb, f));
    bool seen[4] = {true, false, false, false};
    for (const Op &op : pl.ops) {
        if (!seen[op.stream] && op.deps.empty()) pl.need_begin = true;
        seen[op.stream] = true;
    }
    for (const Op &op : pl.ops)
        for (int d : op.deps)
            if (!pl.ops[d].done) HIPCHK(hipEventCreateWithFlags(&pl.ops[d].done, ssd_sync_event_flags(h)));
    return SSD_OK;
}

float conservative_logit_bound(float thr)
{
    if (!(thr > 0.0f)) return -INFINITY;
    if (!(thr < 1.0f)) return INFINITY;
    const double l = log((double)thr / (1.0 - (double)thr));
    return (float)(l - 1e-3 * (1.0 + fabs(l)));
}

static hipError_t pool_event(ssd_handle *h, hipEvent_t *e)
{
    if (!h->ev_pool.empty()) { *e = h->ev_pool.back(); h->ev_pool.pop_back(); return hipSuccess; }
    return hipEventCreate(e);
}

static hipError_t run_op(ssd_handle *h, const Op &op, hipStream_t s)
{
    if (ssd_opt(h, OPT_DEBUG_SYNC, 0)) {
        fprintf(stderr, "[ssd] op class %d stream %d flops %.3g bytes %.3g ...", op.cls, op.stream, op.flops, op.bytes);
        fflush(stderr);
        (void)hipDeviceSynchronize();
        const auto t0 = std::chrono::steady_clock::now();
        hipError_t r = op.run(s);
        hipError_t r2 = hipDeviceSynchronize();
        const double us = std::chrono::duration<double, std::micro>(std::chrono::steady_clock::now() - t0).count();
        fprintf(stderr, " %s  %.1f us alone (launch + wait included): %.1f TFLOP/s, %.2f TB/s\n", r == hipSuccess && r2 == hipSuccess ? "ok" : "FAILED",
                us, op.flops / us * 1e-6, op.bytes / us * 1e-6);
        return r != hipSuccess ? r : r2;
    }
    if (!h->profiling) return op.run(s);
    EvPair e;
    e.cls = op.cls;
    e.fwd = (int)h->ref_evs.size() - 1;
    hipError_t r = pool_event(h, &e.a);
    if (r != hipSuccess) return r;
    r = pool_event(h, &e.b);
    if (r != hipSuccess) return r;
    (void)hipEventRecord(e.a, s);
    r = op.run(s);
    (void)hipEventRecord(e.b, s);
    h->evs.push_back(e);
    h->acc_flops[op.cls] += op.flops;
    h->acc_bytes[op.cls] += op.bytes;
    h->acc_n[op.cls] += 1;
    return r;
}

size_t plan_cache_limit_bytes(const ssd_handle *h)
{
    const int mb = ssd_opt(h, OPT_PLAN_CACHE_MB, 0);
    if (mb > 0) return (size_t)mb << 20;
    static std::mutex mu;
    static std::map<int, size_t> total;
    std::lock_guard<std::mutex> lk(mu);
    auto it = total.find(h->cfg.device);
    if (it != total.end()) return it->second;
    size_t fr = 0, tot = 0;
    if (hipMemGetInfo(&fr, &tot) != hipSuccess) { (void)hipGetLastError(); tot = (size_t)64 << 30; }
    return total[h->cfg.device] = tot / 4;
}

int trim_plan_cache(ssd_handle *h, const PlanSet *keep)
{
    const size_t limit = plan_cache_limit_bytes(h);
    bool drained = false;
    for (;;) {
        size_t total = 0;
        for (const PlanSet *ps : h->cache) total += ps->bytes;
        if ((total <= limit && h->cache.size() <= 64) || h->cache.size() <= 1) break;
        size_t victim = h->cache.size();
        for (size_t i = 0; i < h->cache.size(); ++i)
            if (h->cache[i] != keep && (victim == h->cache.size() || h->cache[i]->last_use < h->cache[victim]->last_use)) victim = i;
        if (victim == h->cache.size()) break;
        if (!drained) { HIPCHK(hipDeviceSynchronize()); drained = true; }
        if (h->cur == h->cache[victim]) h->cur = nullptr;
        free_planset(h->cache[victim]);
        h->cache.erase(h->cache.begin() + victim);
        h->cache_evictions += 1;
    }
    return SSD_OK;
}

static int build_planset(ssd_handle *h, PlanSet &ps)
{
    const PlanKey &key = ps.key;
    int img0 = 0;
    for (int k = 0; k < key.nsub; ++k) {
        const int bk = key.B / key.nsub + (k < key.B % key.nsub ? 1 : 0);
        Plan *pl = new Plan();
        ps.plans.push_back(pl);
        {
            static std::mutex pool_mu;
            static std::map<int, std::vector<hipStream_t>> pool;
            std::lock_guard<std::mutex> lk(pool_mu);
            std::vector<hipStream_t> &pv = pool[h->cfg.device];
            if (pv.size() < 3) pv.resize(3, nullptr);
            for (int i = 0; i < 3; ++i)
                if (!pv[i]) HIPCHK(hipStreamCreateWithFlags(&pv[i], hipStreamNonBlocking));
            pl->s_aux = pv[0];
            pl->s_bb[0] = pv[1];
            pl->s_bb[1] = pv[2];
        }
        HIPCHK(hipEventCreateWithFlags(&pl->ev_join, ssd_sync_event_flags(h)));
        HIPCHK(hipEventCreateWithFlags(&pl->ev_begin, ssd_sync_event_flags(h)));
        SSDCHK(build_plan(h, *pl, bk, key.netH, key.netW, key.ident != 0, img0));
        img0 += bk;
        ps.bytes += pl->pool.bytes;
    }
    return SSD_OK;
}

int select_plans(ssd_handle *h, int B, int H, int W)
{
    const ResizeDims rd = resize_dims(H, W, h->cfg.min_dimension, 128);
    const int netH = rd.nh + rd.ph, netW = rd.nw + rd.pw;
    const int ident = (H == netH && W == netW && rd.nh == H && rd.nw == W) ? 1 : 0;
    h->src.srcH = H; h->src.srcW = W; h->src.nh = rd.nh; h->src.nw = rd.nw;
    for (int k = 0; k < 4; ++k) h->src.box_scaler[k] = rd.box_scaler[k];
    return select_plans_net(h, B, netH, netW, ident, (long long)H * W * 3);
}

int select_plans_net(ssd_handle *h, int B, int netH, int netW, int ident, long long max_src_bytes)
{
    PlanKey key;
    key.B = B;
    key.netH = netH;
    key.netW = netW;
    key.ident = ident;
    int nsub = 1;
    { const int v = ssd_opt(h, OPT_NSUB, 0); if (v >= 1 && v <= 8) nsub = v; }
    {
        const int nH = key.netH, nW = key.netW;
        const int cmax = h->cfg.backbone == SSD_BACKBONE_MOBILENET && !h->pw.empty() ? std::max(h->firstCp, h->pw[0].CoutP) : h->firstCp;
        long long per_img = (long long)(nH / 2) * (nW / 2) * cmax * 4;
        const Pyr py1 = make_pyr(1, nH, nW, 256);
        per_img = std::max(per_img, py1.total * 4);
        per_img = std::max(per_img, (long long)ssd_num_anchors(nH, nW) * std::max(h->cfg.num_classes, 4) * 4);
        per_img = std::max(per_img, max_src_bytes);
        if (h->cfg.backbone == SSD_BACKBONE_SHUFFLENET) {
            const int one[2] = {1, 0};
            StageGeo geo[3];
            sn_stage_geo(h, nH, nW, one, geo);
            for (const StageGeo &g : geo) per_img = std::max(per_img, g.total);
        }
        const long long bmax = ((1LL << 31) - 1) / per_img;
        if (bmax < 1) return ssd_fail(SSD_ERR_INVALID, "ssd_forward: image too large for one launch");
        const int need = (int)((B + bmax - 1) / bmax);
        if (need > nsub) nsub = need;
    }
    if (nsub > B) nsub = B;
    key.nsub = nsub;
    h->use_clock += 1;
    if (h->cur && h->cur->key == key) {
        h->cur->last_use = h->use_clock;
        h->cache_hits += 1;
        return SSD_OK;
    }
    for (PlanSet *ps : h->cache)
        if (ps->key == key) {
            ps->last_use = h->use_clock;
            h->cur = ps;
            h->cache_hits += 1;
            return SSD_OK;
        }
    h->cache_misses += 1;
    PlanSet *ps = new PlanSet();
    ps->key = key;
    ps->last_use = h->use_clock;
    int rc = build_planset(h, *ps);
    if (rc == SSD_ERR_HIP && !h->cache.empty()) {
        (void)hipGetLastError();
        free_planset(ps);
        HIPCHK(hipDeviceSynchronize());
        h->cache_evictions += (long long)h->cache.size();
        free_plans(h);
        ps = new PlanSet();
        ps->key = key;
        ps->last_use = h->use_clock;
        rc = build_planset(h, *ps);
    }
    if (rc != SSD_OK) {
        const std::string msg = ssd_last_error();
        (void)hipDeviceSynchronize();
        free_planset(ps);
        return ssd_fail(rc, msg);
    }
    h->cache.push_back(ps);
    h->cur = ps;
    return trim_plan_cache(h, ps);
}

int enqueue_forward(ssd_handle *h, const uint8_t *images_dev, float *boxes_dev, int32_t *labels_dev,
                           float *scores_dev, int32_t *num_boxes_dev, long long out_stride, hipStream_t s)
{
    if (!h->cur) return ssd_fail(SSD_ERR_STATE, "enqueue_forward: no plan selected");
    h->cur_images = images_dev;
    if (h->profiling) {
        hipEvent_t ref;
        HIPCHK(pool_event(h, &ref));
        HIPCHK(hipEventRecord(ref, s));
        h->ref_evs.push_back(ref);
    }
    const int T = h->cfg.num_classes * h->cfg.max_boxes_per_class;
    const std::vector<Plan *> &plans = h->cur->plans;
    for (size_t k = 0; k < plans.size(); ++k) {
        Plan &pl = *plans[k];
        if (pl.need_begin) HIPCHK(hipEventRecord(pl.ev_begin, s));
        const bool single = ssd_opt(h, OPT_STREAMS, 0) == 1;
        bool used[4] = {true, false, false, false};
        for (const Op &op : pl.ops) {
            const int os = single ? 0 : op.stream;
            hipStream_t st = os == 0 ? s : (os == 1 ? pl.s_aux : pl.s_bb[os - 2]);
            if (!used[os] && op.deps.empty())
                HIPCHK(hipStreamWaitEvent(st, pl.ev_begin, 0));
            used[os] = true;
            for (int d : op.deps)
                if (!single && pl.ops[d].stream != op.stream) HIPCHK(hipStreamWaitEvent(st, pl.ops[d].done, 0));
            HIPCHK(run_op(h, op, st));
            if (op.done && !single) HIPCHK(hipEventRecord(op.done, st));
        }
        if (used[1]) {
            HIPCHK(hipEventRecord(pl.ev_join, pl.s_aux));
            HIPCHK(hipStreamWaitEvent(s, pl.ev_join, 0));
        }
        PostArgs p = pl.post;
        for (int q = 0; q < 4; ++q) p.box_scaler[q] = h->src.box_scaler[q];
        if (h->mixed) {
            p.per_image_scaler = 1;
            for (int b = 0; b < pl.B && pl.img0 + b < SSD_MIXED_MAX; ++b) {
                p.scaler_img[b][0] = h->mixed->scaler[pl.img0 + b][0];
                p.scaler_img[b][1] = h->mixed->scaler[pl.img0 + b][1];
            }
        }
        p.out_stride = out_stride;
        p.boxes = boxes_dev + (out_stride ? (size_t)pl.img0 * out_stride : (size_t)pl.img0 * T * 4);
        p.labels = labels_dev + (out_stride ? (size_t)pl.img0 * out_stride : (size_t)pl.img0 * T);
        p.scores = scores_dev + (out_stride ? (size_t)pl.img0 * out_stride : (size_t)pl.img0 * T);
        p.num = num_boxes_dev + (out_stride ? (size_t)pl.img0 * out_stride : (size_t)pl.img0);
        p.logit_lo = conservative_logit_bound(p.score_thr);
        Op pop;
        pop.cls = 4;
        pop.flops = 0;
        pop.bytes = (double)pl.B * p.N * (p.C + 8) * 4.0;
        pop.run = [p](hipStream_t st) { return launch_postprocess(p, st); };
        HIPCHK(run_op(h, pop, s));
    }
    return SSD_OK;
}
```

single-shot-detector_amd/csrc/ssd_internal.h:

```cpp
#pragma once
#include <hip/hip_runtime.h>
#include <stdint.h>

__host__ __device__ static inline int ssd_phys_of_logical(int l) { int o = l & ~7, r = l & 7; return o + ((r & 1) ? 4 + (r >> 1) : (r >> 1)); }
__host__ __device__ static inline int ssd_logical_of_phys(int p) { int o = p & ~7, r = p & 7; return o + (r < 4 ? 2 * r : 2 * (r - 4) + 1); }

#define SSD_MAX_LEVELS 10

#include <atomic>
static inline hipError_t ssd_allow_lds(const void *fn, int bytes, std::atomic<unsigned> &done)
{
    int dev = 0;
    hipError_t e = hipGetDevice(&dev);
    if (e != hipSuccess) return e;
    if (dev >= 0 && dev < 32 && ((done.load(std::memory_order_relaxed) >> dev) & 1u)) return hipSuccess;
    e = hipFuncSetAttribute(fn, hipFuncAttributeMaxDynamicSharedMemorySize, bytes);
    if (e == hipSuccess && dev >= 0 && dev < 32) done.fetch_or(1u << dev, std::memory_order_relaxed);
    return e;
}

struct UDiv { unsigned mag; int sh; };
static inline UDiv ssd_udiv_make(unsigned d)
{
    UDiv u;
    if (d <= 1) { u.mag = 0; u.sh = -1; return u; }
    int l = 0;
    while ((1u << l) < d) ++l;
    u.mag = (unsigned)((((unsigned long long)1 << (31 + l)) + d - 1) / d);
    u.sh = l - 1;
    return u;
}

struct IgemmLevel {
    int H, W;
    int OH, OW;
    int M;
    int tile_begin;
    int param_off;
    int out_rstride;
    long long in_off;
    long long out_off;
    long long out_bstride;
    long long res_off;
    long long wt_off;
    UDiv dP, dOW;
    int stride, pad;
};

struct IgemmArgs {
    const float *in;
    const float *wt;
    const float *wt_lat;
    float *out;
    float *out2;
    const float *mean, *sf, *beta;
    const float *bias;
    const float *res;
    int B, Cin, Cout, CoutPad;
    int taps;
    int stride, pad;
    int act;
    int nlevels;
    int n_tiles_n;
    UDiv dN;
    int n_major;
    int tiles_m;
    UDiv dM;
    int dense_out;
    int in_fmt;
    int out_fmt;
    int res_fmt;
    float acc_scale;
    int *flags;
    float scan_lo;
    unsigned *scan_bits;
    long long *ts;
    IgemmLevel lv[SSD_MAX_LEVELS];
};

enum IgemmTile { IGEMM_128x128 = 0, IGEMM_128x64 = 1, IGEMM_128x32 = 2, IGEMM_128x256 = 3, IGEMM_256x128 = 4, IGEMM_64x64 = 5, IGEMM_128x96 = 6,
                 IGEMM_64x64D = 7  };
int igemm_tile_bm(int tile);
int igemm_tile_bn(int tile);
hipError_t launch_igemm(int tile, const IgemmArgs &a, int total_tiles_m, hipStream_t s);
enum IgemmLatTile { IGEMM_LAT_1x1 = 20, IGEMM_LAT_1x2 = 21, IGEMM_LAT_2x1 = 22, IGEMM_LAT_2x2 = 23,
                    IGEMM_LAT_W2_1x1 = 24, IGEMM_LAT_W4_1x1 = 25, IGEMM_LAT_W4_2x1 = 26, IGEMM_LAT_W4_1x2 = 27,
                    IGEMM_LAT_1x1_IL = 28, IGEMM_LAT_1x1_D8 = 29, IGEMM_LAT_1x1_D16 = 30, IGEMM_LAT_1x1_NM = 31, IGEMM_LAT_1x1_D8_NM = 32 };
#ifdef SSD_DIAG
static inline bool igemm_is_lat(int tile) { return tile >= IGEMM_LAT_1x1 && tile <= 36; }
#else
static inline bool igemm_is_lat(int tile) { return (tile >= IGEMM_LAT_1x1 && tile <= IGEMM_LAT_W4_1x2) || tile == IGEMM_LAT_1x1_D16; }
#endif
int igemm_lat_bm(int tile);
int igemm_lat_bn(int tile);
bool igemm_lat_n_major(int tile);
bool igemm_lat_supports(const IgemmArgs &a);
hipError_t launch_igemm_lat(int tile, const IgemmArgs &a, int total_tiles_m, hipStream_t s);
#define IGEMM16_TILE 100
hipError_t launch_igemm16(const IgemmArgs &a, int total_tiles_m, hipStream_t s);

struct DwPwSArgs {
    const float *in;
    const float *dwpack;
    const float *wt;
    const float *mean, *sf, *beta;
    float *out;
    int out_rs;
    int B, H, W, K, OH, OW, Cout, wt_rows;
    int pad;
    int dact, act;
    int tiles_y, tiles_x, m_tiles, n_tiles;
    int out_bytes;
    long long *ts;
    int abl;
};
int dwpws_tile_m(int stride);
int dwpws_tile_n(int stride, int CoutP);
hipError_t launch_dwpw_stream(int stride, const DwPwSArgs &a, hipStream_t s);

struct PwGArgs {
    const float *base;
    int base_bytes;
    const int *src;
    int rs;
    const float *wt;
    const float *mean, *sf, *beta;
    float *out;
    int out_rs, out_bytes;
    int M, K, Cout, wt_rows, act;
    int m_tiles, n_tiles;
};
int pw_gather_tile_n(int CoutP);
bool pw_gather_supports(int K, int CoutP, long long M, int rs, long long base_bytes, long long out_bytes);
hipError_t launch_pw_gather(const PwGArgs &a, hipStream_t s);

#define SSD_MIXED_MAX 64
struct FrameGeom { unsigned off; int srcH, srcW, nh, nw; float hs, ws; };
struct MixedGeom { FrameGeom f[SSD_MIXED_MAX]; };
inline FrameGeom frame_geom(int srcH, int srcW, int nh, int nw) { return {0u, srcH, srcW, nh, nw, (float)srcH / (float)nh, (float)srcW / (float)nw}; }
inline unsigned frame_base_round(const uint8_t *&img, unsigned long long &bytes)
{
    const unsigned adj = (unsigned)((uintptr_t)img & 3u);
    img -= adj;
    bytes = (bytes + adj + 3) & ~3ull;
    return adj;
}
inline unsigned frame_base_align(const uint8_t *&img, unsigned long long bytes, FrameGeom &g)
{
    g.off += frame_base_round(img, bytes);
    return (unsigned)bytes;
}
inline unsigned frame_base_align(const uint8_t *&img, unsigned long long bytes, MixedGeom &mg, int first, int B)
{
    const unsigned adj = frame_base_round(img, bytes);
    for (int b = first; b < first + B; ++b) mg.f[b].off += adj;
    return (unsigned)bytes;
}
struct FrontArgs {
    const uint8_t *img;
    const float *w0, *m0, *s0, *b0;
    const float *dwpack;
    const float *wt;
    const float *mean, *sf, *beta;
    float *out;
    int B, H, W;
    int act0, dact, act;
    int tiles_y, tiles_x;
    int resized;
    int srcH, srcW, nh, nw;
    const MixedGeom *mixed;
    int mixed_first;
};
bool front_supports(int B, int H, int W, int C0, int K, int Cout);
bool front_gen_supports(int B, int srcH, int srcW, int nh, int nw);
bool front_mixed_supports(const MixedGeom &mg, int first, int B, int H, int W, unsigned *end_bytes = nullptr);
int front_tile_y();
int front_tile_x();
hipError_t launch_front(const FrontArgs &q, hipStream_t s);
bool front_pool_supports(int B, int H, int W, int C0);
hipError_t launch_front_pool(const uint8_t *img, int B, int H, int W, const float *w0, int C0, const float *m0, const float *s0, const float *b0,
                             int act0, float *out, hipStream_t s, const int *src = nullptr ,
                             const MixedGeom *mixed = nullptr, int first = 0);

hipError_t launch_first_conv(const uint8_t *img, int B, int srcH, int srcW, int nh, int nw, int H, int W,
                             const float *w , int Cout, const float *mean, const float *sf,
                             const float *beta, int act, float *out, hipStream_t s,
                             int variant = 0 );
hipError_t launch_first_conv_mixed(const uint8_t *img, const MixedGeom &mg, int first, int B, int H, int W, const float *w, int Cout,
                                   const float *mean, const float *sf, const float *beta, int act, float *out, hipStream_t s, int variant = 0);
hipError_t launch_depthwise(const float *in, int B, int H, int W, int C, const float *w ,
                            int stride, int pad, int OH, int OW, const float *mean, const float *sf,
                            const float *beta, int act, float *out, hipStream_t s, int out16 = 0 ,
                            int *flags = nullptr );
hipError_t launch_maxpool(const float *in, int B, int H, int W, int C, float *out, hipStream_t s);
hipError_t launch_fpn_merge(const float *x5, const float *l4, float *x4, float *x3, int B, int H3, int W3, int C, hipStream_t s);
hipError_t launch_gather_channels(const float *x, int xs, const float *y, int ys, long long rows, const int *tab,
                                  int Cout, float *out, hipStream_t s);
hipError_t launch_permute_channels(const float *in, long long rows, int C, int Cpad, int to_phys, float *out,
                                   hipStream_t s, int split = 0 );
hipError_t launch_gather_rows(const float *base, const int *src, int rs, long long rows, int Cw, float *out, int ors, hipStream_t s);

struct PostArgs {
    const float *logits, *codes, *anchors;
    int B, N, C;
    float score_thr, iou_thr;
    float logit_lo;
    int max_per_class;
    int fast_max;
    int mid_max;
    int self_clean;
    float box_scaler[4];
    int per_image_scaler;
    float scaler_img[SSD_MIXED_MAX][2];
    float *boxes; int32_t *labels; float *scores; int32_t *num;
    long long out_stride;
    unsigned long long *keys;
    int *counts;
    float *dec;
    float *cls_boxes;
    float *cls_scores;
    int *cls_counts;
    unsigned *scan_bits;
    int scan_fused;
};
size_t post_workspace_bytes(int B, int N, int C, int max_per_class, bool with_keys = true);
size_t post_keys_bytes(int B, int N, int C);
size_t post_scan_bitmap_bytes(int B, int N, int C);
void post_carve(PostArgs &p, void *ws, void *keys_elsewhere = nullptr);
hipError_t launch_postprocess(const PostArgs &p, hipStream_t s);
```

single-shot-detector_amd/csrc/weights.hip:

```cpp
#include "host.h"

#include <cmath>
#include <cstdio>
#include <cstring>

std::vector<int> phys_map(int C, int Cp)
{
    std::vector<int> m(Cp);
    for (int p = 0; p < Cp; ++p) {
        int l = ssd_logical_of_phys(p);
        m[p] = l < C ? l : -1;
    }
    return m;
}
std::vector<int> ident_map(int C, int Cp)
{
    std::vector<int> m(Cp);
    for (int p = 0; p < Cp; ++p) m[p] = p < C ? p : -1;
    return m;
}

std::vector<int> twopart_map(int D, int Dp)
{
    std::vector<int> m(2 * Dp, -1);
    for (int part = 0; part < 2; ++part)
        for (int p = 0; p < Dp; ++p) {
            const int l = ssd_logical_of_phys(p);
            if (l < D) m[part * Dp + p] = part * D + l;
        }
    return m;
}

std::vector<float> permute_rows(const float *w, int rows, int C, const std::vector<int> &map)
{
    const size_t Cp = map.size();
    std::vector<float> t((size_t)rows * Cp, 0.0f);
    for (int r = 0; r < rows; ++r)
        for (size_t p = 0; p < Cp; ++p)
            if (map[p] >= 0) t[r * Cp + p] = w[(size_t)r * C + map[p]];
    return t;
}

BnHost permute_bn(const float *mean, const float *sf, const float *beta, const std::vector<int> &map, BnHost o)
{
    if (!mean) return o;
    for (int p : map) {
        o.mean.push_back(p < 0 ? 0.f : mean[p]);
        o.sf.push_back(p < 0 ? 0.f : sf[p]);
        o.beta.push_back(p < 0 ? 0.f : beta[p]);
    }
    return o;
}

static void bn_pack(const float *gamma, const float *beta, const float *mean, const float *var, int C,
                    const std::vector<int> &outmap, BnHost &o)
{
    const float eps = 1e-3f;
    std::vector<float> sf(C);
    for (int c = 0; c < C; ++c) {
        float s = 1.0f / sqrtf(var[c] + eps);
        sf[c] = gamma[c] * s;
    }
    o = permute_bn(mean, sf.data(), beta, outmap, std::move(o));
}

static int pick_tile(const ssd_handle *h, int CoutP)
{
    if (CoutP <= 32) return IGEMM_128x32;
    if (CoutP <= 64) return IGEMM_128x64;
    if (ssd_opt(h, OPT_IGEMM_96, 1) && CoutP % 128 != 0 && CoutP % 96 == 0) return IGEMM_128x96;
    return IGEMM_128x128;
}

void conv_geometry(const ssd_handle *h, int taps, int CinP, int CoutP, int Cin_l, int Cout_l, ConvW &cw)
{
    cw.taps = taps;
    cw.CinP = CinP;
    cw.CoutP = CoutP;
    cw.tile = g_force_tile >= 0 ? g_force_tile : pick_tile(h, cw.CoutP);
    cw.CoutPad = round_up(cw.CoutP, igemm_tile_bn(cw.tile));
    cw.Cin_l = Cin_l;
    cw.Cout_l = Cout_l;
}

int pack_conv(const ssd_handle *h, DevPool &pool, const float *w, int k, int Cin_l, int Cout_l, const std::vector<int> &inmap,
                     const std::vector<int> &outmap, ConvW &cw)
{
    conv_geometry(h, k * k, (int)inmap.size(), (int)outmap.size(), Cin_l, Cout_l, cw);
    std::vector<float> t((size_t)cw.taps * cw.CoutPad * cw.CinP, 0.0f);
    for (int tap = 0; tap < cw.taps; ++tap)
        for (int n = 0; n < cw.CoutP; ++n) {
            if (outmap[n] < 0) continue;
            float *dst = &t[((size_t)tap * cw.CoutPad + n) * cw.CinP];
            for (int p = 0; p < cw.CinP; ++p)
                if (inmap[p] >= 0) dst[p] = w[((size_t)tap * Cin_l + inmap[p]) * Cout_l + outmap[n]];
        }
    SSDCHK(pool.upload(&cw.wt, t));
    {
        const int KC = cw.CinP / 32, NT = cw.CoutPad / 16;
        std::vector<float> wl(t.size());
        for (int tap = 0; tap < cw.taps; ++tap)
            for (int ct = 0; ct < NT; ++ct)
                for (int kc = 0; kc < KC; ++kc)
                    for (int hf = 0; hf < 2; ++hf)
                        for (int l = 0; l < 64; ++l)
                            for (int e = 0; e < 4; ++e) {
                                const int i = l & 15, kk = l >> 4, cl = 4 * (4 * hf + e) + kk;
                                const int phys = kc * 32 + ssd_phys_of_logical(cl);
                                wl[((((size_t)(tap * NT + ct) * KC + kc) * 2 + hf) * 64 + l) * 4 + e] =
                                    t[((size_t)tap * cw.CoutPad + ct * 16 + i) * cw.CinP + phys];
                            }
        SSDCHK(pool.upload(&cw.wlat, wl));
    }
    float mx = 0.0f;
    for (float v : t) mx = fmaxf(mx, fabsf(v));
    int sh = 0;
    if (mx > 0.0f && std::isfinite(mx)) sh = 8 - ilogbf(mx);
    sh = sh > 100 ? 100 : (sh < -100 ? -100 : sh);
    cw.scale16 = ldexpf(1.0f, -sh);
    std::vector<uint16_t> t16(t.size() * 2);
    for (size_t r = 0; r < t.size() / 8; ++r)
        for (int e = 0; e < 8; ++e) {
            const float x = ldexpf(t[r * 8 + e], sh);
            const _Float16 hh = (_Float16)x;
            const _Float16 ll = (_Float16)(x - (float)hh);
            memcpy(&t16[r * 16 + e], &hh, 2);
            memcpy(&t16[r * 16 + 8 + e], &ll, 2);
        }
    uint16_t *d16 = nullptr;
    SSDCHK(pool.upload(&d16, t16));
    cw.wt16 = (float *)d16;
    cw.CoutPad16 = cw.CoutPad;
    if (cw.CoutP >= 256 && cw.CoutPad % 256 != 0) {
        cw.CoutPad16 = round_up(cw.CoutP, 256);
        const size_t rowh = (size_t)cw.CinP * 2;
        std::vector<uint16_t> w16((size_t)cw.taps * cw.CoutPad16 * rowh, 0);
        for (int tap = 0; tap < cw.taps; ++tap)
            memcpy(&w16[(size_t)tap * cw.CoutPad16 * rowh], &t16[(size_t)tap * cw.CoutPad * rowh], (size_t)cw.CoutPad * rowh * 2);
        uint16_t *dw = nullptr;
        SSDCHK(pool.upload(&dw, w16));
        cw.wt16w = (float *)dw;
    }
    return SSD_OK;
}

int upload_bn(DevPool &pool, const BnHost &b, ConvW &cw)
{
    SSDCHK(pool.upload(&cw.mean, b.mean));
    SSDCHK(pool.upload(&cw.sf, b.sf));
    return pool.upload(&cw.beta, b.beta);
}

int pack_dw(DevPool &pool, const std::vector<float> &w9, const BnHost &b, DwW &d)
{
    if (d.Cp % 32 || b.mean.empty()) return SSD_OK;
    const int KC = d.Cp / 32;
    std::vector<float> p((size_t)KC * 12 * 32);
    for (int s = 0; s < KC; ++s)
        for (int c = 0; c < 32; ++c) {
            for (int t = 0; t < 9; ++t) p[((size_t)s * 12 + t) * 32 + c] = w9[(size_t)t * d.Cp + s * 32 + c];
            p[((size_t)s * 12 + 9) * 32 + c] = b.mean[s * 32 + c];
            p[((size_t)s * 12 + 10) * 32 + c] = b.sf[s * 32 + c];
            p[((size_t)s * 12 + 11) * 32 + c] = b.beta[s * 32 + c];
        }
    return pool.upload(&d.pack, p);
}

int upload_dw(DevPool &pool, const std::vector<float> &w, const BnHost &b, DwW &d)
{
    if (!w.empty()) SSDCHK(pool.upload(&d.w, w));
    if (!b.mean.empty()) SSDCHK(pool.upload(&d.mean, b.mean));
    if (!b.sf.empty()) SSDCHK(pool.upload(&d.sf, b.sf));
    if (!b.beta.empty()) SSDCHK(pool.upload(&d.beta, b.beta));
    return w.size() == (size_t)9 * d.Cp ? pack_dw(pool, w, b, d) : SSD_OK;
}

static const Tensor *getvar(ssd_handle *h, const std::string &n, std::initializer_list<int64_t> shape)
{
    auto it = h->vars.find(n);
    if (it == h->vars.end()) { ssd_fail(SSD_ERR_WEIGHT, "missing variable " + n); return nullptr; }
    const Tensor &t = it->second;
    std::vector<int64_t> want(shape);
    if (t.shape != want) {
        std::string s = "variable " + n + " has shape [";
        for (auto d : t.shape) s += std::to_string(d) + ",";
        s += "] expected [";
        for (auto d : want) s += std::to_string(d) + ",";
        ssd_fail(SSD_ERR_WEIGHT, s + "]");
        return nullptr;
    }
    return &t;
}

static int get_bn(ssd_handle *h, const std::string &scope, int C, const std::vector<int> &outmap, BnHost &o)
{
    const Tensor *g = getvar(h, scope + "/gamma", {C}), *b = getvar(h, scope + "/beta", {C});
    const Tensor *m = getvar(h, scope + "/moving_mean", {C}), *v = getvar(h, scope + "/moving_variance", {C});
    if (!g || !b || !m || !v) return SSD_ERR_WEIGHT;
    bn_pack(g->data.data(), b->data.data(), m->data.data(), v->data.data(), C, outmap, o);
    return SSD_OK;
}

static int load_conv(ssd_handle *h, const std::string &wname, const std::string &bnscope, int k, int Cin, int Cout,
                     ConvW &cw, bool out_identity = false, int in_split = 0)
{
    const Tensor *w = getvar(h, wname, {k, k, Cin, Cout});
    if (!w) return SSD_ERR_WEIGHT;
    std::vector<int> inmap = in_split > 0 ? twopart_map(in_split, round_up(in_split, 32)) : phys_map(Cin, round_up(Cin, 32));
    std::vector<int> outmap = out_identity ? ident_map(Cout, Cout) : phys_map(Cout, round_up(Cout, 32));
    SSDCHK(pack_conv(h, h->wpool, w->data.data(), k, Cin, Cout, inmap, outmap, cw));
    if (!bnscope.empty()) {
        BnHost b;
        SSDCHK(get_bn(h, bnscope, Cout, outmap, b));
        SSDCHK(upload_bn(h->wpool, b, cw));
    }
    return SSD_OK;
}

static int load_dw(ssd_handle *h, const std::string &scope, const std::string &bnname, int C, DwW &d, int in_split = 0)
{
    const Tensor *w = getvar(h, scope + "/depthwise_weights", {3, 3, C, 1});
    if (!w) return SSD_ERR_WEIGHT;
    d.Cp = in_split > 0 ? 2 * round_up(in_split, 32) : round_up(C, 32);
    std::vector<int> map = in_split > 0 ? twopart_map(in_split, round_up(in_split, 32)) : phys_map(C, d.Cp);
    BnHost b;
    SSDCHK(get_bn(h, scope + "/" + bnname, C, map, b));
    return upload_dw(h->wpool, permute_rows(w->data.data(), 9, C, map), b, d);
}

static int load_first(ssd_handle *h, const std::string &scope, const std::string &bnname, int Cout)
{
    const Tensor *w = getvar(h, scope + "/weights", {3, 3, 3, Cout});
    if (!w) return SSD_ERR_WEIGHT;
    const int Cp = round_up(Cout, 32);
    std::vector<int> map = phys_map(Cout, Cp);
    h->first.Cp = h->firstCp = Cp;
    BnHost b;
    SSDCHK(get_bn(h, scope + "/" + bnname, Cout, map, b));
    return upload_dw(h->wpool, permute_rows(w->data.data(), 27, Cout, map), b, h->first);
}

const int MB_STRIDE[13] = {1, 2, 1, 2, 1, 2, 1, 1, 1, 1, 1, 2, 1};
static const int MB_FILT[13] = {64, 128, 128, 256, 256, 512, 512, 512, 512, 512, 512, 1024, 1024};
static int mb_depth(int x, float dm) { int v = (int)(x * dm); return v > 8 ? v : 8; }

static int shuffle_initial_depth(float dm)
{
    if (dm == 0.5f) return 48;
    if (dm == 1.0f) return 116;
    if (dm == 1.5f) return 176;
    if (dm == 2.0f) return 224;
    return -1;
}

static int finalize_mobilenet(ssd_handle *h)
{
    const float dm = h->cfg.depth_multiplier;
    int c = mb_depth(32, dm);
    SSDCHK(load_first(h, "MobilenetV1/Conv2d_0", "BatchNorm", c));
    h->firstAct = SSD_ACT_RELU6;
    h->dw.resize(13);
    h->pw.resize(13);
    for (int i = 0; i < 13; ++i) {
        char s[96];
        snprintf(s, sizeof s, "MobilenetV1/Conv2d_%d_depthwise", i + 1);
        SSDCHK(load_dw(h, s, "BatchNorm", c, h->dw[i]));
        const int f = mb_depth(MB_FILT[i], dm);
        snprintf(s, sizeof s, "MobilenetV1/Conv2d_%d_pointwise", i + 1);
        SSDCHK(load_conv(h, std::string(s) + "/weights", std::string(s) + "/BatchNorm", 1, c, f, h->pw[i]));
        c = f;
        if (i == 4) h->c_ch[0] = c;
        if (i == 10) h->c_ch[1] = c;
        if (i == 12) h->c_ch[2] = c;
    }
    return SSD_OK;
}

static int finalize_shufflenet(ssd_handle *h)
{
    const int D0 = shuffle_initial_depth(h->cfg.depth_multiplier);
    if (D0 < 0) return ssd_fail(SSD_ERR_INVALID, "shufflenet depth_multiplier must be 0.5, 1.0, 1.5 or 2.0");
    SSDCHK(load_first(h, "ShuffleNetV2/Conv1", "batch_norm", 24));
    h->firstAct = SSD_ACT_RELU;
    const int units[3] = {4, 8, 4};
    int cin = 24, out = D0, split = 0;
    for (int st = 0; st < 3; ++st) {
        const int D = out / 2;
        h->sn_stage[st] = ssd_handle::SnStage{(int)h->pw.size(), (int)h->dw.size(), units[st]};
        char base[64];
        snprintf(base, sizeof base, "ShuffleNetV2/Stage%d", st + 2);
        std::string u1 = std::string(base) + "/unit_1";
        ConvW cw; DwW d;
        SSDCHK(load_conv(h, u1 + "/conv1x1_before/weights", u1 + "/conv1x1_before/batch_norm", 1, cin, cin, cw, false, split)); h->pw.push_back(cw);
        SSDCHK(load_dw(h, u1 + "/depthwise", "batch_norm", cin, d)); h->dw.push_back(d);
        cw = ConvW();
        SSDCHK(load_conv(h, u1 + "/conv1x1_after/weights", u1 + "/conv1x1_after/batch_norm", 1, cin, D, cw)); h->pw.push_back(cw);
        d = DwW();
        SSDCHK(load_dw(h, u1 + "/second_branch/depthwise", "batch_norm", cin, d, split)); h->dw.push_back(d);
        cw = ConvW();
        SSDCHK(load_conv(h, u1 + "/second_branch/conv1x1_after/weights", u1 + "/second_branch/conv1x1_after/batch_norm", 1, cin, D, cw, false, split)); h->pw.push_back(cw);
        for (int j = 2; j <= units[st]; ++j) {
            std::string u = std::string(base) + "/unit_" + std::to_string(j);
            cw = ConvW();
            SSDCHK(load_conv(h, u + "/conv1x1_before/weights", u + "/conv1x1_before/batch_norm", 1, D, D, cw)); h->pw.push_back(cw);
            if (!pw_gather_supports(cw.CinP, cw.CoutP, 1, cw.CinP * 4, cw.CinP * 4, cw.CoutP * 4))
                return ssd_fail(SSD_ERR_INVALID, "ssd_finalize: " + u + "/conv1x1_before (" + std::to_string(D) + " -> " + std::to_string(D) +
                                                 " channels) is not a shape of the gathering 1x1 kernel (sn_pw.hip: 32 <= padded input channels <= 512)");
            d = DwW();
            SSDCHK(load_dw(h, u + "/depthwise", "batch_norm", D, d)); h->dw.push_back(d);
            cw = ConvW();
            SSDCHK(load_conv(h, u + "/conv1x1_after/weights", u + "/conv1x1_after/batch_norm", 1, D, D, cw)); h->pw.push_back(cw);
        }
        cin = out;
        split = D;
        if (st == 0) { h->c_ch[0] = out; h->c_split[0] = D; }
        if (st == 1) { h->c_ch[1] = out; h->c_split[1] = D; }
        out *= 2;
    }
    const int fin = h->cfg.depth_multiplier == 2.0f ? 2048 : 1024;
    ConvW cw;
    SSDCHK(load_conv(h, "ShuffleNetV2/Conv5/weights", "ShuffleNetV2/Conv5/batch_norm", 1, cin, fin, cw, false, split));
    h->pw.push_back(cw);
    h->c_ch[2] = fin;
    return SSD_OK;
}

static int finalize_fpn_heads(ssd_handle *h)
{
    for (int i = 0; i < 3; ++i) {
        char n[48];
        snprintf(n, sizeof n, "fpn/lateral%d/kernel", i + 3);
        SSDCHK(load_conv(h, n, "", 1, h->c_ch[i], 256, h->lat[i], false, h->c_split[i]));
    }
    for (int i = 0; i < 5; ++i) {
        char n[48], b[48];
        snprintf(n, sizeof n, "fpn/p%d/kernel", i + 3);
        snprintf(b, sizeof b, "fpn/p%d_batch_norm", i + 3);
        SSDCHK(load_conv(h, n, b, 3, i == 3 ? h->c_ch[2] : 256, 256, h->pconv[i]));
    }
    {
        const int src_of[4] = {0, 1, 2, 4};
        ConvW &g = h->pgroup;
        g = h->pconv[0];
        g.wt16 = g.wt16w = nullptr;
        const bool have_lat = h->pconv[0].wlat && h->pconv[1].wlat && h->pconv[2].wlat && h->pconv[4].wlat;
        g.wlat = nullptr;
        const size_t wn = (size_t)g.taps * g.CoutPad * g.CinP, pn = (size_t)g.CoutP;
        for (int i = 1; i < 4; ++i)
            if (h->pconv[src_of[i]].CoutPad != g.CoutPad || h->pconv[src_of[i]].CinP != g.CinP || h->pconv[src_of[i]].CoutP != g.CoutP)
                return ssd_fail(SSD_ERR_WEIGHT, "fpn p3 / p4 / p5 / p7 kernels differ in shape");
        SSDCHK(h->wpool.alloc((void **)&g.wt, 4 * wn * sizeof(float)));
        SSDCHK(h->wpool.alloc((void **)&g.mean, 4 * pn * sizeof(float)));
        SSDCHK(h->wpool.alloc((void **)&g.sf, 4 * pn * sizeof(float)));
        SSDCHK(h->wpool.alloc((void **)&g.beta, 4 * pn * sizeof(float)));
        if (have_lat) SSDCHK(h->wpool.alloc((void **)&g.wlat, 4 * wn * sizeof(float)));
        for (int i = 0; i < 4; ++i) {
            const ConvW &src = h->pconv[src_of[i]];
            if (have_lat) HIPCHK(hipMemcpy(g.wlat + i * wn, src.wlat, wn * sizeof(float), hipMemcpyDeviceToDevice));
            HIPCHK(hipMemcpy(g.wt + i * wn, src.wt, wn * sizeof(float), hipMemcpyDeviceToDevice));
            HIPCHK(hipMemcpy(g.mean + i * pn, src.mean, pn * sizeof(float), hipMemcpyDeviceToDevice));
            HIPCHK(hipMemcpy(g.sf + i * pn, src.sf, pn * sizeof(float), hipMemcpyDeviceToDevice));
            HIPCHK(hipMemcpy(g.beta + i * pn, src.beta, pn * sizeof(float), hipMemcpyDeviceToDevice));
        }
    }
    const char *nets[2] = {"box_net", "class_net"};
    const int A = 6, C = h->cfg.num_classes;
    for (int t = 0; t < 2; ++t) {
        for (int i = 0; i < 4; ++i) {
            char n[64];
            snprintf(n, sizeof n, "%s/conv3x3_%d/kernel", nets[t], i);
            ConvW &cw = h->tower[t][i];
            SSDCHK(load_conv(h, n, "", 3, 256, 256, cw));
            BnHost b;
            std::vector<int> outmap = phys_map(256, 256);
            for (int l = 3; l <= 7; ++l) {
                char s[80];
                snprintf(s, sizeof s, "%s/batch_norm_%d_for_level_%d", nets[t], i, l);
                SSDCHK(get_bn(h, s, 256, outmap, b));
            }
            SSDCHK(upload_bn(h->wpool, b, cw));
        }
        const int Cout = t == 0 ? 4 * A : C * A;
        const std::string scope = std::string(nets[t]) + (t == 0 ? "/encoded_boxes" : "/logits");
        ConvW &cw = h->final_[t];
        SSDCHK(load_conv(h, scope + "/kernel", "", 3, 256, Cout, cw, true));
        const Tensor *bias = getvar(h, scope + "/bias", {Cout});
        if (!bias) return SSD_ERR_WEIGHT;
        std::vector<float> bpad(bias->data);
        bpad.resize((size_t)round_up(Cout, 4), 0.0f);
        SSDCHK(h->wpool.upload(&cw.bias, bpad));
    }
    return SSD_OK;
}

int finalize_weights(ssd_handle *h)
{
    int r = h->cfg.backbone == SSD_BACKBONE_MOBILENET ? finalize_mobilenet(h) : finalize_shufflenet(h);
    if (r == SSD_OK) r = finalize_fpn_heads(h);
    if (r != SSD_OK) {
        h->wpool.free_all();
        h->dw.clear(); h->pw.clear();
    }
    return r;
}
```

single-shot-detector_amd/evaluation.py:

```python
import os

import numpy as np

from .coco_eval import Evaluator
from .config import load_loss_config
from .ssd import (AnchorGenerator, batch_multiclass_non_max_suppression, mixed_batches, network_input_size, split_records,
                  ssd_loss, _torch)

_METRIC_NAMES = ("AP", "precision", "recall", "mean_iou_for_TP", "best_threshold", "total_FP", "total_FN")


def l2_sum(weights):
    s = 0.0
    for name in sorted(weights):
        if ("weights" in name or "kernel" in name) and "depthwise_weights" not in name:
            k = np.asarray(weights[name], np.float64).reshape(-1)
            s += float(np.dot(k, k)) / 2.0
    return s


def regularization_loss(weights, weight_decay):
    return np.float32(float(weight_decay) * l2_sum(weights))


def total_loss(localization, classification, regularization, loss_config):
    lw = np.float32(loss_config["localization_loss_weight"]) * np.float32(localization)
    cw = np.float32(loss_config["classification_loss_weight"]) * np.float32(classification)
    return np.float32(float(lw) + float(cw) + float(regularization))


class _Run:

    def __init__(self, engine):
        self.engine = engine
        self.anchors = {}

    def anchors_for(self, shape):
        a = self.anchors.get(shape)
        if a is None:
            gen = AnchorGenerator()
            t = _torch().from_numpy(gen(*shape)).to("cuda:%d" % self.engine.device)
            a = self.anchors[shape] = (t, list(gen.num_anchors_per_feature_map))
        return a

    def __call__(self, frames, gts, loss_config):
        torch = _torch()
        eng, p = self.engine, self.engine.params
        dev = "cuda:%d" % eng.device
        shape = eng.network_shape(frames[0].shape[0], frames[0].shape[1])
        anchors, per_level = self.anchors_for(shape)
        B, N, C = len(frames), int(anchors.shape[0]), int(p["num_classes"])
        eng.forward_mixed([torch.from_numpy(np.require(f, np.uint8, ["C", "W"])).to(dev) for f in frames])
        logits = eng.get_tensor_dev("class_predictions", (B, N, C))
        codes = eng.get_tensor_dev("encoded_boxes", (B, N, 4))
        G = max(1, max(len(g[1]) for g in gts))
        boxes = np.zeros((B, G, 4), np.float32)
        labels = np.zeros((B, G), np.int32)
        num = np.zeros((B,), np.int32)
        scaled = []
        for b, (f, (gb, gl)) in enumerate(zip(frames, gts)):
            bs = network_input_size(f.shape[0], f.shape[1], p["min_dimension"])[2]
            s = np.asarray(gb, np.float32).reshape(-1, 4) * bs
            scaled.append(s)
            boxes[b, :len(s)] = s
            labels[b, :len(s)] = gl
            num[b] = len(s)
        _losses, per_image = ssd_loss(logits, codes, anchors, {"boxes": boxes, "labels": labels, "num_boxes": num},
                                      gamma=loss_config["gamma"], alpha=loss_config["alpha"], anchors_per_level=per_level)
        pb, ps, pc, pn = batch_multiclass_non_max_suppression(codes, anchors, logits, p["score_threshold"], p["iou_threshold"],
                                                              p["max_boxes_per_class"], box_scaler=None)
        per_image, pb, ps, pc, pn = (t.cpu().numpy() for t in (per_image, pb, ps, pc, pn))
        out = []
        for b in range(B):
            n = int(pn[b])
            out.append((per_image[b, :3], scaled[b], (pb[b, :n], pc[b, :n], ps[b, :n])))
        return out


def image_losses(per_image_row, regularization, loss_config):
    norm = max(np.float32(per_image_row[2]), np.float32(1.0))
    loc = np.float32(per_image_row[0]) / norm
    cls = np.float32(per_image_row[1]) / norm
    return loc, cls, total_loss(loc, cls, regularization, loss_config)


def evaluate(detector, val_dataset, config, max_batch=32, read_workers=None, decode=None, group=None, chunk=256):
    from concurrent.futures import ThreadPoolExecutor
    from . import tfrecords
    from .distributed import ChunkAssignment
    lc = load_loss_config(config)
    eng = detector.engine
    reg = detector.regularization_loss(lc["weight_decay"])
    if decode is None:
        decode = tfrecords.decode_image
    data = tfrecords.read_dataset(val_dataset) if isinstance(val_dataset, (str, os.PathLike)) else val_dataset
    evaluator = Evaluator(int(eng.params["num_classes"]))
    run = _Run(eng)
    sums = np.zeros(4, np.float64)
    count = 0
    workers = max(1, int(read_workers if read_workers is not None else min(16, os.cpu_count() or 1)))
    if group is None:
        world, rank = 1, 0
    else:
        import torch.distributed as dist
        world, rank = dist.get_world_size(group), dist.get_rank(group)
    assign = ChunkAssignment(world, rank, chunk)

    def run_items(items):
        results = [None] * len(items)
        for part in mixed_batches(eng, [frame.shape[:2] for frame, _gb, _gl in items], max_batch):
            with eng.lock:
                res = run([items[i][0] for i in part], [(items[i][1], items[i][2]) for i in part], lc)
            for i, r in zip(part, res):
                results[i] = r
        return results

    def add(result, gl):
        nonlocal count, sums
        row, gt_scaled, (bx, lb, sc) = result
        loc, cls, tot = image_losses(row, reg, lc)
        sums = sums + np.array([float(tot), float(loc), float(cls), float(reg)])
        count += 1
        evaluator.add_image(gt_scaled, gl, bx, lb, sc)

    def flush(items):
        own = [(f.result(), gb, gl) for f, gb, gl in items[rank * chunk:(rank + 1) * chunk]]
        results = run_items(own)
        if group is not None:
            results = _exchange(eng, own, results, items, group, chunk)
        for result, (_f, _gb, gl) in zip(results, items):
            add(result, gl)

    with ThreadPoolExecutor(max_workers=workers) as pool:
        items = []
        for i, (img, gb, gl) in enumerate(data):
            items.append((pool.submit(decode, img) if assign.mine(i) else None, gb, gl))
            if len(items) == world * chunk:
                flush(items)
                items = []
        if items:
            flush(items)
    if count == 0:
        raise ValueError("the validation dataset is empty")
    means = sums / count
    out = {"loss": float(np.float32(means[0])), "localization_loss": float(np.float32(means[1])),
           "classification_loss": float(np.float32(means[2])), "regularization_loss": float(np.float32(means[3]))}
    m = evaluator.evaluate()
    if evaluator.num_classes == 1:
        for k in _METRIC_NAMES:
            out["metrics/" + k] = float(np.float32(m[0][k]))
    else:
        out["metrics/mAP"] = float(np.float32(m["mAP"]))
    out["num_images"] = count
    return out


def _exchange(eng, own, results, items, group, chunk):
    import torch.distributed as dist
    from .distributed import gather_records
    torch = _torch()
    world, rank = dist.get_world_size(group), dist.get_rank(group)
    per = min(chunk, len(items))
    rows = np.zeros((per, 5 + eng.record_words), np.int32)
    boxes, labels, scores, num = split_records(rows[:, 5:])
    for j, ((frame, _gb, _gl), (row, _s, (bx, lb, sc))) in enumerate(zip(own, results)):
        n = len(sc)
        rows[j, 0:3] = np.asarray(row[:3], np.float32).view(np.int32)
        rows[j, 3:5] = frame.shape[:2]
        boxes[j, :n], labels[j, :n], scores[j, :n], num[j] = bx, lb, sc, n
    dev = torch.device("cuda", eng.device) if dist.get_backend(group) == "nccl" else torch.device("cpu")
    got = gather_records(torch.from_numpy(rows).to(dev), group).cpu().numpy()
    boxes, labels, scores, num = split_records(got[:, 5:])
    out = []
    for q, (_f, gb, _gl) in enumerate(items):
        r, j = divmod(q, chunk)
        i, n = r * per + j, int(num[r * per + j])
        bs = network_input_size(int(got[i, 3]), int(got[i, 4]), eng.params["min_dimension"])[2]
        out.append((got[i, 0:3].view(np.float32), np.asarray(gb, np.float32).reshape(-1, 4) * bs,
                    (boxes[i, :n], labels[i, :n], scores[i, :n])))
    return out


def main(argv=None):
    import argparse
    import json
    import sys
    from .detector import Detector
    ap = argparse.ArgumentParser(description="train.py's evaluation of a checkpoint: validation loss and AP")
    ap.add_argument("model_path", help="checkpoint prefix / model_dir / frozen graph / .npz")
    ap.add_argument("--config", required=True, help="the reference's JSON config")
    ap.add_argument("--val_dataset", default=None, help="directory of .tfrecords shards (default: the config's val_dataset)")
    ap.add_argument("--use_ema", action="store_true", help="the moving averages, as RestoreMovingAverageHook restores them")
    ap.add_argument("--max_batch", type=int, default=32)
    ap.add_argument("--gpus", type=int, default=1,
                    help="processes to shard the images over: N > 1 starts torch.distributed.run with N ranks as a child process "
                         "(rank r on device LOCAL_RANK %% device_count; RCCL only when every rank has a device of its own, else "
                         "gloo); inside such a launch the collective path runs, also at N = 1")
    a = ap.parse_args(argv)
    if a.gpus < 1:
        ap.error("--gpus must be >= 1")
    if a.gpus > 1 and "WORLD_SIZE" not in os.environ:
        from .distributed import launch_local
        sys.exit(launch_local(a.gpus, "ssd_amd.evaluation", sys.argv[1:] if argv is None else list(argv)))
    val = a.val_dataset or json.load(open(a.config))["val_dataset"]
    if "WORLD_SIZE" not in os.environ:
        with Detector(a.model_path, config=a.config, use_ema=a.use_ema) as det:
            print(json.dumps(evaluate(det, val, a.config, max_batch=a.max_batch), sort_keys=True))
        return
    import torch.distributed as dist
    from .distributed import init_node_process_group
    if a.gpus != int(os.environ["WORLD_SIZE"]):
        raise SystemExit("--gpus (%d) != WORLD_SIZE (%s)" % (a.gpus, os.environ["WORLD_SIZE"]))
    device, _backend = init_node_process_group()
    try:
        with Detector(a.model_path, config=a.config, use_ema=a.use_ema, visible_device_list=str(device)) as det:
            res = evaluate(det, val, a.config, max_batch=a.max_batch, group=dist.group.WORLD)
        if dist.get_rank() == 0:
            print(json.dumps(res, sort_keys=True), flush=True)
    finally:
        dist.destroy_process_group()


if __name__ == "__main__":
    main()
```

single-shot-detector_amd/ssd.py:

```python
import ctypes
import threading

import numpy as np

from . import _lib
from ._lib import SsdConfig, SsdLossConfig, check, lib

ACT = {None: 0, "none": 0, "relu": 1, "relu6": 2}


def _torch():
    import torch
    if not torch.cuda.is_available():
        raise RuntimeError("single-shot-detector_amd needs an AMD GPU (HIP device): there is "
                           "no CPU path")
    return torch


def _stream(torch):
    return ctypes.c_void_p(torch.cuda.current_stream().cuda_stream)


def _ptr(t):
    return ctypes.c_void_p(t.data_ptr())
# ... 521 lines not shown
        torch = _torch()
        if records.dtype != torch.int32 or tuple(records.shape) != (B, self.record_words) or not records.is_contiguous():
            raise ValueError("records must be a contiguous int32 tensor [B, %d]" % self.record_words)
        if not (records.is_cuda or records.is_pinned()):
            raise ValueError("records must live in device memory or in pinned host memory")

    def _out_slot(self, B, index=0):
        torch = _torch()
        slot = self._static.get(("out", B, index))
        if slot is None:
            block = self.new_records(B, "cuda:%d" % self.device)
            pin_out = torch.empty(block.shape, dtype=torch.int32).pin_memory()
            slot = {"block": block, "views": self.record_views(block), "pin_out": pin_out, "host": self.record_views(pin_out.numpy())}
            while sum(1 for k in self._static if k[0] == "out") >= 32:
                self._static.pop(next(k for k in self._static if k[0] == "out"))
            self._static[("out", B, index)] = slot
        return slot

    def _in_slot(self, shape, index=0, pinned=False):
        torch = _torch()
        n = 1
        for d in shape:
            n *= int(d)
        slot = self._static.setdefault(("in", index), {"cap": 0, "dev": None, "pin": None, "ev": None, "events": None})
        if n > slot["cap"] or (pinned and slot["pin"] is None):
            cap = max(slot["cap"], 2 << 20)
            while cap < n:
                cap <<= 1
            torch.cuda.synchronize(self.device)
            slot["dev"] = torch.empty((cap,), dtype=torch.uint8, device="cuda:%d" % self.device)
            slot["pin"] = torch.empty((cap,), dtype=torch.uint8).pin_memory() if pinned or slot["pin"] is not None else None
            slot["cap"] = cap
        dev_in = slot["dev"][:n].view(shape)
        pin_in = slot["pin"][:n].view(shape) if slot["pin"] is not None else None
        return slot, dev_in, pin_in

    def forward_cached(self, images):
        torch = _torch()
        if isinstance(images, np.ndarray):
            images = torch.from_numpy(np.ascontiguousarray(images))
        if images.dtype != torch.uint8 or images.dim() != 4 or images.shape[3] != 3:
            raise ValueError("images must be uint8 with shape [B,H,W,3]")
        with self.lock:
            slot, dev_in, _ = self._in_slot(tuple(images.shape))
            out = self._out_slot(int(images.shape[0]))
            cur = torch.cuda.current_stream()
            if slot["ev"] is not None:
                cur.wait_event(slot["ev"])
            else:
                slot["ev"] = torch.cuda.Event()
            dev_in.copy_(images, non_blocking=True)
            res = self.forward(dev_in, records=out["block"])
            slot["ev"].record(cur)
            return res

    def detect_host(self, images):
        torch = _torch()
        images = np.asarray(images)
        if images.dtype != np.uint8 or images.ndim != 4 or images.shape[3] != 3:
            raise ValueError("images must be a uint8 array of shape [B, height, width, 3]")
        with self.lock:
            src = np.ascontiguousarray(images)
            B, H, W, _ = src.shape
            return self._host_result(self._out_slot(B), B, lambda rec: check(
                lib().ssd_forward_host(self._h, src.ctypes.data, B, H, W, _ptr(rec), _stream(torch))))

    def _host_result(self, slot, B, enqueue, wait=True):
        torch = _torch()
        zc = B <= self.zero_copy_max_batch
        enqueue(slot["pin_out"] if zc else slot["block"])
        if not zc:
            slot["pin_out"].copy_(slot["block"], non_blocking=True)
        if not wait:
            if slot.get("done") is None:
                slot["done"] = torch.cuda.Event()
            slot["done"].record()
            return slot
        torch.cuda.current_stream().synchronize()
        return slot["host"]

    def detect_one(self, image, score_threshold):
        torch = _torch()
        H, W, _ = image.shape
        with self.lock:
            slot = self._out_slot(1)
            src = np.ascontiguousarray(image)
            sc = slot.get("one")
            if sc is None:
                T = self.T
                sc = (np.empty((T, 4), np.float32), np.empty((T,), np.int32), np.empty((T,), np.float32), ctypes.c_int32(0))
                sc = slot["one"] = sc + tuple(a.ctypes.data for a in sc[:3]) + (ctypes.byref(sc[3]), _ptr(slot["pin_out"]))
            check(lib().ssd_detect_host(self._h, src.ctypes.data, H, W, score_threshold, sc[8], sc[4], sc[5], sc[6],
                                        sc[0].shape[0], sc[7], _stream(torch)))
            n = sc[3].value
            return sc[0][:n].copy(), sc[1][:n].copy(), sc[2][:n].copy()

    MIXED_MAX = 64

    def network_shape(self, height, width):
        return network_input_size(height, width, self.params["min_dimension"])[:2]

    def forward_mixed(self, frames, records=None):
        torch = _torch()
        with self.lock:
            if records is not None:
                self._check_records(records, len(frames[1]) if isinstance(frames, tuple) else len(frames))
            if isinstance(frames, tuple):
                flat, hw, offsets = frames
                _check_dev(torch, flat, torch.uint8, "frames")
            else:
                hw = [(int(f.shape[0]), int(f.shape[1])) for f in frames]
                offsets, total = [], 0
                for h_, w_ in hw:
                    offsets.append(total)
                    total += (h_ * w_ * 3 + 15) & ~15
                _, flat, _ = self._in_slot((max(total, 16),), index=4)
                for f, o, (h_, w_) in zip(frames, offsets, hw):
                    _check_dev(torch, f, torch.uint8, "frames")
                    if f.dim() != 3 or f.shape[2] != 3:
                        raise ValueError("every frame must have shape [H, W, 3]")
                    flat[o:o + h_ * w_ * 3].view(h_, w_, 3).copy_(f, non_blocking=True)
            B = len(hw)
            if records is None:
                records = self.new_records(B, flat.device)
            hw_c = (ctypes.c_int32 * (2 * B))(*[v for pair in hw for v in pair])
            off_c = (ctypes.c_int64 * B)(*offsets) if offsets is not None else None
            check(lib().ssd_forward_mixed(self._h, _ptr(flat), B, hw_c, off_c, _ptr(records), _stream(torch)))
            return self.record_views(records)

    def detect_host_mixed(self, images, wait=True, index=0):
        with self.lock:
            enqueue = self._mixed_host_call(images)
            return self._host_result(self._out_slot(len(images), index), len(images), enqueue, wait)

    def forward_mixed_host(self, images, records):
        with self.lock:
            enqueue = self._mixed_host_call(images)
            self._check_records(records, len(images))
            enqueue(records)
            return self.record_views(records)

    def _mixed_host_call(self, images):
        torch = _torch()
        srcs = [np.ascontiguousarray(host_frame(im, "every image")) for im in images]

        def enqueue(records):
            B = len(srcs)
            ptrs = (ctypes.c_void_p * B)(*[im.ctypes.data for im in srcs])
            hw_c = (ctypes.c_int32 * (2 * B))(*[int(v) for im in srcs for v in im.shape[:2]])
            check(lib().ssd_forward_mixed_host(self._h, ptrs, B, hw_c, _ptr(records), _stream(torch)))
        return enqueue

    def detect_stream(self, batches):
        torch = _torch()
        dev = torch.device("cuda", self.device)
        if self._copy_streams is None:
            self._copy_streams = (torch.cuda.Stream(dev), torch.cuda.Stream(dev))
        s_in, s_out = self._copy_streams
        s_c = torch.cuda.current_stream(dev)
        pending = None
        k = 0

        def collect(p):
            oslot, e = p
            e["d2h"].synchronize()
            return tuple(np.array(v) for v in oslot["host"])

        for images in batches:
            images = np.asarray(images)
            if images.dtype != np.uint8 or images.ndim != 4 or images.shape[3] != 3:
                raise ValueError("every batch must be a uint8 array of shape [B, height, width, 3]")
            key = tuple(images.shape)
            j = k & 1
            islot, dev_in, pin_in = self._in_slot(key, index=1 + j, pinned=True)
            oslot = self._out_slot(key[0], index=1 + j)
            e = islot["events"]
            if e is None:
                e = islot["events"] = {n: torch.cuda.Event() for n in ("h2d", "cmp", "d2h")}
                for n in e:
                    e[n].record(s_c)
            e["h2d"].synchronize()
            e["d2h"].synchronize()
            np.copyto(pin_in.numpy(), images)
            with torch.cuda.stream(s_in):
                s_in.wait_event(e["cmp"])
                dev_in.copy_(pin_in, non_blocking=True)
                e["h2d"].record(s_in)
            s_c.wait_event(e["h2d"])
            self.forward(dev_in, records=oslot["block"])
            e["cmp"].record(s_c)
            with torch.cuda.stream(s_out):
                s_out.wait_event(e["cmp"])
                oslot["pin_out"].copy_(oslot["block"], non_blocking=True)
                e["d2h"].record(s_out)
            if pending is not None:
                yield collect(pending)
            pending = (oslot, e)
            k += 1
        if pending is not None:
            yield collect(pending)

    def plan_cache_stats(self):
        v = (ctypes.c_int64 * 8)()
        with self.lock:
            check(lib().ssd_plan_cache_stats(self._h, v))
        return {"plans": v[0], "arena_bytes": v[1], "budget_bytes": v[2], "hits": v[3], "misses": v[4], "evictions": v[5],
                "last_network_shape": [v[6], v[7]]}

    def plan_cache_clear(self):
        with self.lock:
            check(lib().ssd_plan_cache_clear(self._h))

    def get_tensor(self, name):
        dims = (ctypes.c_int32 * 4)()
        cap = 1 << 20
        while True:
            buf = np.empty((cap,), np.float32)
            with self.lock:
                rc = lib().ssd_get_tensor(self._h, name.encode(),
                                          buf.ctypes.data_as(ctypes.POINTER(ctypes.c_float)), cap, dims)
            if rc != 0 and b"too small" in (lib().ssd_last_error() or b"") and cap < (1 << 34):
                cap *= 8
                continue
            check(rc)
            n = dims[0] * dims[1] * dims[2] * dims[3]
            return buf[:n].reshape(dims[0], dims[1], dims[2], dims[3]).copy()

    def get_tensor_dev(self, name, shape):
        torch = _torch()
        out = torch.empty(tuple(shape), dtype=torch.float32, device="cuda:%d" % self.device)
        dims = (ctypes.c_int32 * 4)()
        with self.lock:
            check(lib().ssd_get_tensor_dev(self._h, name.encode(), _ptr(out), out.numel(), dims,
                                           _stream(torch)))
        return out

    def profile_enable(self, on=True):
        check(lib().ssd_profile_enable(self._h, 1 if on else 0))

    def profile_reset(self):
        check(lib().ssd_profile_reset(self._h))

    def profile_read(self):
        names = ["conv3x3_mfma", "pointwise_mfma", "depthwise", "first_conv", "postprocess", "other",
                 "depthwise_pointwise_fused", "conv3x3_f16x3_tile256"]
        out = {}
        for i, n in enumerate(names):
            ms, cnt = ctypes.c_double(), ctypes.c_int64()
            fl, by = ctypes.c_double(), ctypes.c_double()
            check(lib().ssd_profile_read(self._h, i, ctypes.byref(ms), ctypes.byref(cnt),
                                         ctypes.byref(fl), ctypes.byref(by)))
            out[n] = {"ms": ms.value, "launches": cnt.value, "flops": fl.value, "bytes": by.value}
        return out


def network_input_size(height, width, min_dimension, divisor=128):
    scale = np.float32(min_dimension / min(height, width))
    if height >= width:
        nh, nw = int(np.rint(np.float32(height) * scale)), int(min_dimension)
        ph, pw = -(-nh // divisor) * divisor - nh, 0
    else:
        nw, nh = int(np.rint(np.float32(width) * scale)), int(min_dimension)
        pw, ph = -(-nw // divisor) * divisor - nw, 0
    box_scaler = np.array([nh / (nh + ph), nw / (nw + pw)] * 2, np.float32)
    return nh + ph, nw + pw, box_scaler


class RetinaNetFeatureExtractor:

    def __init__(self, engine):
        self.engine = engine

    def __call__(self, images):
        B, H, W, _ = images.shape
        self.outputs = self.engine.forward(images)
        nh, nw, _bs = network_input_size(H, W, self.engine.params["min_dimension"])
        self.image_size = (nh, nw)
        return [self.engine.get_tensor_dev("p%d" % l, (B, -(-nh // s), -(-nw // s), 256)) for l, s in zip(range(3, 8), (8, 16, 32, 64, 128))]


class BackboneFeatures:

    def __init__(self, engine):
        self.engine = engine
        from .variables import variable_shapes
        shapes = variable_shapes(engine.params)
        self.channels = [shapes["fpn/lateral%d/kernel" % l][2] for l in (3, 4, 5)]

    def __call__(self, images):
        B, H, W, _ = images.shape
        self.engine.forward(images)
        nh, nw, _bs = network_input_size(H, W, self.engine.params["min_dimension"])
        self.image_size = (nh, nw)
        return [self.engine.get_tensor_dev("c%d" % l, (B, -(-nh // s), -(-nw // s), c)) for l, s, c in zip((3, 4, 5), (8, 16, 32), self.channels)]


class RetinaNetBoxPredictor:

    def __init__(self, engine, num_classes=None):
        self.engine = engine
        self.num_classes = engine.params["num_classes"] if num_classes is None else num_classes
        if self.num_classes != engine.params["num_classes"]:
            raise ValueError("num_classes differs from the engine's configuration")

    def __call__(self, image_features):
        B = image_features[0].shape[0]
        N = sum(int(f.shape[1]) * int(f.shape[2]) * 6 for f in image_features)
        return {"encoded_boxes": self.engine.get_tensor_dev("encoded_boxes", (B, N, 4)),
                "class_predictions": self.engine.get_tensor_dev("class_predictions", (B, N, self.num_classes))}


class SSD:

    def __init__(self, images, feature_extractor, anchor_generator=None, box_predictor=None, num_classes=None):
        torch = _torch()
        if isinstance(feature_extractor, Engine):
            engine = feature_extractor
            feature_extractor = RetinaNetFeatureExtractor(engine)
            box_predictor = RetinaNetBoxPredictor(engine, num_classes)
        if anchor_generator is None:
            anchor_generator = AnchorGenerator()
        if box_predictor is None:
            raise TypeError("SSD(images, feature_extractor, anchor_generator, box_predictor, num_classes)")
        self.engine = feature_extractor.engine
        self.num_classes = self.engine.params["num_classes"] if num_classes is None else num_classes
        if self.num_classes != self.engine.params["num_classes"]:
            raise ValueError("num_classes differs from the engine's configuration")
        feature_maps = feature_extractor(images)
        image_height, image_width = feature_extractor.image_size
        self.anchors = torch.from_numpy(anchor_generator(image_height, image_width)).to(images.device)
        self.num_anchors_per_feature_map = anchor_generator.num_anchors_per_feature_map
        self.raw_predictions = box_predictor(feature_maps)
        self.box_scaler = network_input_size(images.shape[1], images.shape[2], self.engine.params["min_dimension"])[2]

    def get_predictions(self, score_threshold=0.05, iou_threshold=0.5, max_boxes_per_class=20):
        boxes, scores, classes, num = batch_multiclass_non_max_suppression(
            self.raw_predictions["encoded_boxes"], self.anchors,
            self.raw_predictions["class_predictions"], score_threshold=score_threshold,
            iou_threshold=iou_threshold, max_boxes_per_class=max_boxes_per_class, box_scaler=self.box_scaler)
        return {"boxes": boxes, "labels": classes, "scores": scores, "num_boxes": num}

    def loss(self, groundtruth, params):
        losses, per_image = ssd_loss(self.raw_predictions["class_predictions"], self.raw_predictions["encoded_boxes"],
                                     self.anchors, groundtruth, gamma=params["gamma"], alpha=params["alpha"],
                                     anchors_per_level=self.num_anchors_per_feature_map)
        self.localization_losses_per_image = per_image[:, 0]
        self.classification_losses_per_image = per_image[:, 1]
        self.matches_per_image = per_image[:, 2]
        self.matches_per_level = per_image[:, 3:]
        return {"localization_loss": losses[0], "classification_loss": losses[1]}
```

Measured before the change: 814.2.

## Screen class-logit conv with fp16 upper bound and compute only surviving outputs

Adds a logit-screening path for the final classification conv. An fp16 MFMA pass computes a conservative upper bound on each logit, rounding inputs up and splitting weights into positive and negative parts. Only 8-channel groups whose bound reaches the score threshold are compacted into lists and computed exactly in fp32. This aims to skip most of the dense classification-head conv, whose logits mostly fall below the threshold. It adds convert, screen and compact kernels, and the full dense logits are rebuilt lazily when a caller asks for class_predictions, with the evaluation and predictor paths turning screening off.

```diff
diff --git a/single-shot-detector_amd/_lib.py b/single-shot-detector_amd/_lib.py
--- a/single-shot-detector_amd/_lib.py
+++ b/single-shot-detector_amd/_lib.py
@@ -4,7 +4,7 @@
 
 _HERE = os.path.dirname(os.path.abspath(__file__))
 _CSRC = os.path.join(_HERE, "csrc")
-_SOURCES = ["abi.hip", "weights.hip", "plan.hip", "stages.hip", "igemm.hip", "igemm_lat.hip", "igemm16.hip", "dwpw_stream.hip", "sn_pw.hip", "front.hip",
+_SOURCES = ["abi.hip", "weights.hip", "plan.hip", "stages.hip", "igemm.hip", "igemm_lat.hip", "igemm16.hip", "logit_screen.hip", "dwpw_stream.hip", "sn_pw.hip", "front.hip",
             "elementwise.hip", "postprocess.hip", "loss.hip", "augment.hip", "update.hip", "train_head.hip", "wgrad.hip", "train_backbone.hip"]
 _LIB_PATH = os.path.join(_CSRC, "libssd_hip.so")
 _DIAG_PATH = os.path.join(_CSRC, "libssd_hip_diag.so")
diff --git a/single-shot-detector_amd/csrc/abi.hip b/single-shot-detector_amd/csrc/abi.hip
--- a/single-shot-detector_amd/csrc/abi.hip
+++ b/single-shot-detector_amd/csrc/abi.hip
@@ -13,7 +13,7 @@
 static std::mutex g_opts_mu;
 static const char *const OPT_NAMES[OPT_COUNT] = {"streams", "h2d_chunks", "front_fuse", "fuse_dw", "backbone_split", "event_fence", "plan_cache_mb",
                                                  "igemm_tile", "igemm16", "igemm_96", "igemm_lat", "igemm_deep64", "lateral_split", "fpn_group", "fpn_p7_group",
-                                                 "fpn_early_lat", "nsub", "nms_fast_max", "first_conv_px", "debug_sync"};
+                                                 "fpn_early_lat", "nsub", "nms_fast_max", "first_conv_px", "debug_sync", "logits_screen"};
 int ssd_opt_index(const char *key)
 {
     for (int i = 0; i < OPT_COUNT; ++i)
@@ -488,6 +488,10 @@
         const Retained &r = it->second;
         const long long rows = (long long)r.B * r.H * r.W;
         if (cap < done + rows * r.C) return ssd_fail(SSD_ERR_INVALID, "ssd_get_tensor: destination too small");
+        if (pl->screened && !pl->logits_whole && !strcmp(name, "class_predictions")) {
+            SSDCHK(materialize_logits(h, *pl, nullptr));
+            HIPCHK(hipDeviceSynchronize());
+        }
         std::vector<float> tmp((size_t)rows * r.Cp);
         HIPCHK(hipMemcpy(tmp.data(), r.dev, tmp.size() * sizeof(float), hipMemcpyDeviceToHost));
         for (long long q = 0; q < rows; ++q)
@@ -522,6 +526,7 @@
         const Retained &r = it->second;
         const long long rows = (long long)r.B * r.H * r.W;
         if (cap < done + rows * r.C) return ssd_fail(SSD_ERR_INVALID, "ssd_get_tensor_dev: destination too small");
+        if (!strcmp(name, "class_predictions")) SSDCHK(materialize_logits(h, *pl, (hipStream_t)stream));
         if (r.permuted) HIPCHK(launch_permute_channels(r.dev, rows, r.C, r.Cp, r.fmt ? 2 : 0, dst_dev + done, (hipStream_t)stream, r.fmt ? 0 : r.split));
         else HIPCHK(hipMemcpyAsync(dst_dev + done, r.dev, (size_t)rows * r.C * sizeof(float), hipMemcpyDeviceToDevice, (hipStream_t)stream));
         done += rows * r.C;
diff --git a/single-shot-detector_amd/csrc/host.h b/single-shot-detector_amd/csrc/host.h
--- a/single-shot-detector_amd/csrc/host.h
+++ b/single-shot-detector_amd/csrc/host.h
@@ -43,6 +43,7 @@
     OPT_NMS_FAST_MAX,
     OPT_FIRST_CONV_PX,
     OPT_DEBUG_SYNC,
+    OPT_LOGITS_SCREEN,
     OPT_COUNT
 };
 #define SSD_OPT_UNSET INT_MIN
@@ -98,6 +99,8 @@
     float *wt16w = nullptr;
     int CoutPad16 = 0;
     float scale16 = 1.0f;
+    unsigned short *wscr = nullptr;
+    float *scst = nullptr;
     int CinP = 0, CoutP = 0, CoutPad = 0, taps = 1, tile = IGEMM_128x128;
     int Cin_l = 0, Cout_l = 0;
 };
@@ -110,6 +113,7 @@
 
 #define SSD_NCLS 8
 #define SSD_FUSE_DW_DEFAULT 0xfu
+#define SSD_SCREEN_MIN_ROWS 32768
 #define SSD_FUSE_SHUFFLE_DEFAULT true
 #ifdef SSD_DIAG
 extern int g_force_tile;
@@ -124,7 +128,7 @@
                   BnHost o = BnHost());
 void conv_geometry(const struct ssd_handle *h, int taps, int CinP, int CoutP, int Cin_l, int Cout_l, ConvW &cw);
 int pack_conv(const struct ssd_handle *h, DevPool &pool, const float *w, int k, int Cin_l, int Cout_l, const std::vector<int> &inmap,
-              const std::vector<int> &outmap, ConvW &cw);
+              const std::vector<int> &outmap, ConvW &cw, const float *screen_bias = nullptr );
 int upload_bn(DevPool &pool, const BnHost &b, ConvW &cw);
 int upload_dw(DevPool &pool, const std::vector<float> &w, const BnHost &b, DwW &d);
 int pack_dw(DevPool &pool, const std::vector<float> &w9, const BnHost &b, DwW &d);
@@ -190,6 +194,8 @@
     hipStream_t s_bb[2] = {nullptr, nullptr};
     hipEvent_t ev_join = nullptr, ev_begin = nullptr;
     bool need_begin = false;
+    bool screened = false, logits_whole = true;
+    Op logits_dense;
 };
 
 struct SrcGeom { int srcH = 0, srcW = 0, nh = 0, nw = 0; float box_scaler[4] = {1, 1, 1, 1}; };
@@ -260,5 +266,6 @@
 int select_plans_net(ssd_handle *h, int B, int netH, int netW, int ident, long long max_src_bytes);
 int trim_plan_cache(ssd_handle *h, const PlanSet *keep);
 size_t plan_cache_limit_bytes(const ssd_handle *h);
+int materialize_logits(ssd_handle *h, Plan &pl, hipStream_t s);
 int enqueue_forward(ssd_handle *h, const uint8_t *images_dev, float *boxes_dev, int32_t *labels_dev, float *scores_dev,
                     int32_t *num_boxes_dev, long long out_stride, hipStream_t s);
diff --git a/single-shot-detector_amd/csrc/logit_screen.hip b/single-shot-detector_amd/csrc/logit_screen.hip
--- /dev/null
+++ b/single-shot-detector_amd/csrc/logit_screen.hip
@@ -0,0 +1,391 @@
+#include "ssd_internal.h"
+#include <type_traits>
+
+typedef float v16f __attribute__((ext_vector_type(16)));
+typedef float v4f __attribute__((ext_vector_type(4)));
+typedef unsigned v4u __attribute__((ext_vector_type(4)));
+typedef _Float16 v8h __attribute__((ext_vector_type(8)));
+typedef __attribute__((address_space(3))) void *lds_ptr_t;
+
+__device__ __forceinline__ unsigned f16_up_bits(float x)
+{
+    if (!(x >= 0.0f)) return 0x7e00u;
+    if (x == 0.0f) return 0u;
+    const _Float16 h = (_Float16)x;
+    unsigned b = (unsigned)__builtin_bit_cast(unsigned short, h);
+    if ((float)h < x) b += 1u;
+    return b < 0x0400u ? 0x0400u : b;
+}
+
+__global__ __launch_bounds__(256) void logit_convert_kernel(const float *__restrict__ x, unsigned short *__restrict__ x16, long long n8,
+                                                            int *__restrict__ counts, int ncounts)
+{
+    if (blockIdx.x == 0 && (int)threadIdx.x < ncounts) counts[threadIdx.x] = 0;
+    for (long long i = (long long)blockIdx.x * 256 + threadIdx.x; i < n8; i += (long long)gridDim.x * 256) {
+        const v4f a = *(const v4f *)(x + i * 8), b = *(const v4f *)(x + i * 8 + 4);
+        v4u o;
+        o[0] = f16_up_bits(a[0]) | (f16_up_bits(a[1]) << 16);
+        o[1] = f16_up_bits(a[2]) | (f16_up_bits(a[3]) << 16);
+        o[2] = f16_up_bits(b[0]) | (f16_up_bits(b[1]) << 16);
+        o[3] = f16_up_bits(b[2]) | (f16_up_bits(b[3]) << 16);
+        *(v4u *)(x16 + i * 8) = o;
+    }
+}
+
+__device__ __forceinline__ ScreenLevel screen_level_of_tile(const ScreenArgs &a, int tile_m)
+{
+    ScreenLevel L = a.lv[0];
+#pragma unroll
+    for (int i = 1; i < SCREEN_MAX_LEVELS; ++i)
+        if (i < a.nlevels && tile_m >= a.lv[i].tile_begin) L = a.lv[i];
+    return L;
+}
+__device__ __forceinline__ ScreenLevel screen_level_of_row(const ScreenArgs &a, int r)
+{
+    ScreenLevel L = a.lv[0];
+#pragma unroll
+    for (int i = 1; i < SCREEN_MAX_LEVELS; ++i)
+        if (i < a.nlevels && r >= a.lv[i].row_begin) L = a.lv[i];
+    return L;
+}
+
+__global__ __launch_bounds__(256, 1) void logit_screen_kernel(const ScreenArgs a)
+{
+    constexpr int BM = 256;
+    constexpr int A_BYTES = BM * 128;
+    constexpr int STAGE = (BM + 256) * 128;
+    extern __shared__ __attribute__((aligned(16))) unsigned char lds[];
+
+    const int tid = threadIdx.x, lane = tid & 63;
+    const int wave = __builtin_amdgcn_readfirstlane(tid >> 6);
+    const int wave_m = wave >> 1, wave_n = wave & 1;
+    int swz;
+    {
+        const int nblk = gridDim.x, bid = blockIdx.x;
+        const int q = nblk >> 3, r = nblk & 7, xcd = bid & 7;
+        swz = (xcd < r ? xcd * (q + 1) : r * (q + 1) + (xcd - r) * q) + (bid >> 3);
+    }
+    const int tile_n = swz % a.NT;
+    const int tile_m = swz / a.NT;
+    const ScreenLevel L = screen_level_of_tile(a, tile_m);
+    const int H = L.H, W = L.W, P = L.P, M = L.M;
+    const int Cin = a.Cin;
+    const int m0 = (tile_m - L.tile_begin) * BM;
+
+    const __amdgpu_buffer_rsrc_t arsrc = __builtin_amdgcn_make_buffer_rsrc(
+        (void *)(a.x16 + L.in_off), 0, (int)((long long)a.B * P * Cin * 2), 0x00020000);
+    const __amdgpu_buffer_rsrc_t brsrc = __builtin_amdgcn_make_buffer_rsrc(
+        (void *)a.w16, 0, (int)((long long)9 * a.NT * 256 * Cin * 2), 0x00020000);
+    constexpr unsigned OOB = 0x80000000u;
+
+    int abase[8], aiy0[8], aix0[8];
+    unsigned offc[8];
+    int boff[8];
+#pragma unroll
+    for (int u = 0; u < 8; ++u) {
+        const int row = wave * 64 + u * 8 + (lane >> 3);
+        const int chunk = (lane & 7) ^ ((row >> 1) & 7);
+        const int m = m0 + row;
+        const bool rowok = m < M;
+        const int mm = rowok ? m : 0;
+        const int b = mm / P, p = mm - b * P;
+        const int oy = p / W, ox = p - oy * W;
+        abase[u] = b * P * Cin * 2 + chunk * 16;
+        aiy0[u] = rowok ? oy - 1 : -(1 << 20);
+        aix0[u] = ox - 1;
+        boff[u] = (tile_n * 256 + row) * Cin * 2 + chunk * 16;
+    }
+    auto tap_offsets = [&](int t) {
+        const int tky = t / 3, tkx = t - 3 * tky;
+#pragma unroll
+        for (int u = 0; u < 8; ++u) {
+            const int iy = aiy0[u] + tky, ix = aix0[u] + tkx;
+            const bool ok = ((unsigned)iy < (unsigned)H) & ((unsigned)ix < (unsigned)W);
+            offc[u] = ok ? (unsigned)(abase[u] + (iy * W + ix) * Cin * 2) : OOB;
+        }
+    };
+    const int b_tapstride = a.NT * 256 * Cin * 2;
+    const int KC = Cin >> 6;
+    const int KS = 9 * KC;
+    auto dma = [&](int stage, int tap, int kc) {
+        unsigned char *abuf = lds + stage * STAGE + wave * 64 * 128;
+        unsigned char *bbuf = lds + stage * STAGE + A_BYTES + wave * 64 * 128;
+        const int so = kc * 128, bso = tap * b_tapstride + kc * 128;
+#pragma unroll
+        for (int u = 0; u < 8; ++u)
+            __builtin_amdgcn_raw_ptr_buffer_load_lds(arsrc, (lds_ptr_t)(abuf + u * 1024), 16, (int)offc[u], so, 0, 0);
+#pragma unroll
+        for (int u = 0; u < 8; ++u)
+            __builtin_amdgcn_raw_ptr_buffer_load_lds(brsrc, (lds_ptr_t)(bbuf + u * 1024), 16, boff[u], bso, 0, 0);
+    };
+    int roff[4];
+#pragma unroll
+    for (int s = 0; s < 4; ++s) {
+        const int chunk = 2 * s + (lane >> 5);
+        roff[s] = (lane & 31) * 128 + ((chunk ^ (((lane & 31) >> 1) & 7)) << 4);
+    }
+    v16f acc[4][4];
+#pragma unroll
+    for (int i = 0; i < 4; ++i)
+#pragma unroll
+        for (int j = 0; j < 4; ++j)
+#pragma unroll
+            for (int r = 0; r < 16; ++r) acc[i][j][r] = 0.0f;
+
+    tap_offsets(0);
+    dma(0, 0, 0);
+    for (int ks = 0; ks < KS; ++ks) {
+        const int cur = ks & 1;
+        asm volatile("s_waitcnt vmcnt(0) lgkmcnt(0)" ::: "memory");
+        __builtin_amdgcn_s_barrier();
+        __builtin_amdgcn_sched_barrier(0);
+        if (ks + 1 < KS) {
+            const int kc = __builtin_amdgcn_readfirstlane((ks + 1) / 9), tap = ks + 1 - 9 * kc;
+            tap_offsets(tap);
+            dma(cur ^ 1, tap, kc);
+        }
+        const unsigned char *ab = lds + cur * STAGE + wave_m * 4 * 4096;
+        const unsigned char *bb = lds + cur * STAGE + A_BYTES + wave_n * 4 * 4096;
+#pragma unroll
+        for (int s = 0; s < 4; ++s) {
+            v4f fa[4], fb[4];
+#pragma unroll
+            for (int i = 0; i < 4; ++i) fa[i] = *(const v4f *)(ab + i * 4096 + roff[s]);
+#pragma unroll
+            for (int j = 0; j < 4; ++j) fb[j] = *(const v4f *)(bb + j * 4096 + roff[s]);
+#pragma unroll
+            for (int i = 0; i < 4; ++i)
+#pragma unroll
+                for (int j = 0; j < 4; ++j)
+                    acc[i][j] = __builtin_amdgcn_mfma_f32_32x32x16_f16(__builtin_bit_cast(v8h, fa[i]), __builtin_bit_cast(v8h, fb[j]), acc[i][j], 0, 0, 0);
+        }
+    }
+
+    asm volatile("s_waitcnt vmcnt(0) lgkmcnt(0)" ::: "memory");
+    __syncthreads();
+    float *mine = (float *)lds + wave * 4096;
+    const float *Pp = (const float *)lds + (wave_m * 2) * 4096, *Np = Pp + 4096;
+    float cst[4];
+    bool colok[4];
+#pragma unroll
+    for (int j = 0; j < 4; ++j) {
+        const int col = tile_n * 128 + j * 32 + (lane & 31);
+        colok[j] = col < a.Cout;
+        cst[j] = colok[j] ? a.cst[col] : 0.0f;
+    }
+    const float lo = a.lo;
+    const int rstride = a.out_rstride;
+    const long long bstride = a.out_bstride, out_off = L.out_off;
+    auto pass = [&](auto itag) __attribute__((always_inline)) {
+        constexpr int i = decltype(itag)::value;
+#pragma unroll
+        for (int j = 0; j < 4; ++j)
+#pragma unroll
+            for (int r = 0; r < 16; ++r) mine[(r * 4 + j) * 64 + lane] = acc[i][j][r];
+        __syncthreads();
+        const int rbase = m0 + wave_m * 128 + i * 32;
+#pragma unroll 1
+        for (int r = wave_n * 8; r < wave_n * 8 + 8; ++r) {
+            const int rowl = rbase + (r & 3) + 8 * (r >> 2) + 4 * (lane >> 5);
+#pragma unroll
+            for (int j = 0; j < 4; ++j) {
+                const float Pv = Pp[(r * 4 + j) * 64 + lane], Nv = Np[(r * 4 + j) * 64 + lane];
+                const float t1 = Pv * 1.001953125f, t2 = Nv * 0.998046875f;
+                const float U = ((t1 - t2) + cst[j]) + 3.814697265625e-06f * ((Pv + Nv) + __builtin_fabsf(cst[j]));
+                const bool flag = colok[j] && rowl < M && !(U < lo);
+                const unsigned long long mask = __ballot(flag);
+                if (mask != 0ull && lane < 8) {
+                    const unsigned byte = (unsigned)(mask >> (8 * lane)) & 0xffu;
+                    const int row = rbase + (r & 3) + 8 * (r >> 2) + 4 * (lane >> 2);
+                    const int col8 = tile_n * 128 + j * 32 + (lane & 3) * 8;
+                    if (byte && row < M && col8 < a.Cout) {
+                        const int b = row / P, p = row - b * P;
+                        const unsigned oct = (unsigned)((out_off + (long long)b * bstride + (long long)p * rstride + col8) >> 3);
+                        atomicOr(a.bits + (oct >> 5), 1u << (oct & 31));
+                    }
+                }
+            }
+        }
+        __syncthreads();
+    };
+    pass(std::integral_constant<int, 0>{});
+    pass(std::integral_constant<int, 1>{});
+    pass(std::integral_constant<int, 2>{});
+    pass(std::integral_constant<int, 3>{});
+}
+
+__global__ __launch_bounds__(256) void logit_compact_kernel(const ScreenArgs a, long long nwords)
+{
+    __shared__ int lcnt[SCREEN_MAX_OCT], lbase[SCREEN_MAX_OCT];
+    __shared__ unsigned short slot[256 * 32];
+    const int NO = a.Cout >> 3;
+    const unsigned NC = (unsigned)a.out_bstride;
+    for (long long w0 = (long long)blockIdx.x * 256; w0 < nwords; w0 += (long long)gridDim.x * 256) {
+        const long long w = w0 + threadIdx.x;
+        const unsigned bits = w < nwords ? a.bits[w] : 0u;
+        if (!__syncthreads_or(bits != 0u)) continue;
+        if ((int)threadIdx.x < NO) lcnt[threadIdx.x] = 0;
+        __syncthreads();
+        auto decode = [&](int bpos, int &o) -> int {
+            const unsigned e = ((unsigned)w * 32u + (unsigned)bpos) * 8u;
+            const unsigned b = e / NC, rem = e - b * NC;
+            int lvl = 0;
+#pragma unroll
+            for (int i = 1; i < SCREEN_MAX_LEVELS; ++i)
+                if (i < a.nlevels && rem >= (unsigned)a.lv[i].out_off) lvl = i;
+            const unsigned within = rem - (unsigned)a.lv[lvl].out_off;
+            const unsigned p = within / (unsigned)a.out_rstride;
+            o = (int)((within - p * (unsigned)a.out_rstride) >> 3);
+            return a.lv[lvl].row_begin + (int)b * a.lv[lvl].P + (int)p;
+        };
+        for (unsigned rest = bits; rest; rest &= rest - 1) {
+            const int bpos = __builtin_ctz(rest);
+            int o;
+            (void)decode(bpos, o);
+            slot[threadIdx.x * 32 + bpos] = (unsigned short)atomicAdd(&lcnt[o], 1);
+        }
+        __syncthreads();
+        if ((int)threadIdx.x < NO) lbase[threadIdx.x] = lcnt[threadIdx.x] ? atomicAdd(a.counts + threadIdx.x, lcnt[threadIdx.x]) : 0;
+        __syncthreads();
+        for (unsigned rest = bits; rest; rest &= rest - 1) {
+            const int bpos = __builtin_ctz(rest);
+            int o;
+            const int row = decode(bpos, o);
+            a.lists[(long long)o * a.rows_total + lbase[o] + slot[threadIdx.x * 32 + bpos]] = row;
+        }
+        __syncthreads();
+    }
+}
+
+#define FILL_CHUNK 64
+__global__ __launch_bounds__(512) void logit_fill_kernel(const ScreenArgs a)
+{
+    extern __shared__ __attribute__((aligned(16))) unsigned char lds[];
+    float *wl = (float *)lds;
+    __shared__ int cbeg[SCREEN_MAX_OCT + 1];
+    const int NO = a.Cout >> 3;
+    if (threadIdx.x == 0) {
+        int t = 0;
+        for (int o = 0; o < NO; ++o) { cbeg[o] = t; t += (a.counts[o] + FILL_CHUNK - 1) / FILL_CHUNK; }
+        cbeg[NO] = t;
+    }
+    __syncthreads();
+    const int total = cbeg[NO];
+    const int Cin = a.Cin, K = 9 * Cin;
+    const int c = threadIdx.x & 7;
+    int staged = -1, o = 0;
+    float bias = 0.0f;
+    for (int ch = blockIdx.x; ch < total; ch += gridDim.x) {
+        while (cbeg[o + 1] <= ch) ++o;
+        if (o != staged) {
+            __syncthreads();
+            for (int idx = threadIdx.x; idx < K * 8; idx += 512) {
+                const int k = idx % Cin, cc = (idx / Cin) & 7, tap = idx / (Cin * 8);
+                wl[(tap * Cin + k) * 8 + cc] = a.wt[((long long)tap * a.CoutPad + o * 8 + cc) * Cin + k];
+            }
+            __syncthreads();
+            staged = o;
+            bias = a.bias[o * 8 + c];
+        }
+        const int n = a.counts[o];
+        const int *list = a.lists + (long long)o * a.rows_total;
+        const int first = (ch - cbeg[o]) * FILL_CHUNK;
+        const int last = first + FILL_CHUNK < n ? first + FILL_CHUNK : n;
+        for (int it = first + (threadIdx.x >> 3); it < last; it += 64) {
+            const int r = list[it];
+            const ScreenLevel L = screen_level_of_row(a, r);
+            const int m = r - L.row_begin;
+            const int b = m / L.P, p = m - b * L.P;
+            const int oy = p / L.W, ox = p - oy * L.W;
+            const float *xb = a.x + L.in_off + (long long)b * L.P * Cin;
+            float acc = 0.0f;
+            for (int tap = 0; tap < 9; ++tap) {
+                const int ky = tap / 3, kx = tap - 3 * ky;
+                const int iy = oy + ky - 1, ix = ox + kx - 1;
+                const bool ok = ((unsigned)iy < (unsigned)L.H) & ((unsigned)ix < (unsigned)L.W);
+                const float *xp = xb + (long long)(ok ? iy * L.W + ix : 0) * Cin;
+                const float *wp = wl + tap * Cin * 8 + c;
+#pragma unroll 4
+                for (int k8 = 0; k8 < Cin; k8 += 8) {
+                    v4f v0 = *(const v4f *)(xp + k8), v1 = *(const v4f *)(xp + k8 + 4);
+                    if (!ok) { v0 = v4f{0.f, 0.f, 0.f, 0.f}; v1 = v0; }
+                    acc = __builtin_fmaf(v0[0], wp[(k8 + 0) * 8], acc);
+                    acc = __builtin_fmaf(v1[0], wp[(k8 + 4) * 8], acc);
+                    acc = __builtin_fmaf(v0[1], wp[(k8 + 1) * 8], acc);
+                    acc = __builtin_fmaf(v1[1], wp[(k8 + 5) * 8], acc);
+                    acc = __builtin_fmaf(v0[2], wp[(k8 + 2) * 8], acc);
+                    acc = __builtin_fmaf(v1[2], wp[(k8 + 6) * 8], acc);
+                    acc = __builtin_fmaf(v0[3], wp[(k8 + 3) * 8], acc);
+                    acc = __builtin_fmaf(v1[3], wp[(k8 + 7) * 8], acc);
+                }
+            }
+            a.logits[L.out_off + (long long)b * a.out_bstride + (long long)p * a.out_rstride + o * 8 + c] = acc + bias;
+        }
+    }
+}
+
+static bool screen_args_ok(const ScreenArgs &a)
+{
+    if (!a.x || !a.x16 || !a.w16 || !a.wt || !a.bias || !a.cst || !a.logits || !a.bits || !a.counts || !a.lists) return false;
+    if (a.Cin % 64 != 0 || a.Cin < 64 || a.Cout % 8 != 0 || a.Cout < 8 || a.Cout > 8 * SCREEN_MAX_OCT || a.Cout > a.CoutPad) return false;
+    if (a.NT != (a.Cout + 127) / 128 || a.nlevels < 1 || a.nlevels > SCREEN_MAX_LEVELS) return false;
+    if ((long long)9 * a.NT * 256 * a.Cin * 2 >= (1LL << 31) || (long long)9 * a.Cin * 8 * 4 > 160 * 1024 / 2) return false;
+    if (a.out_rstride != a.Cout || a.out_bstride <= 0 || (a.out_bstride & 7) || (long long)a.B * a.out_bstride * 4 >= (1LL << 31)) return false;
+    long long rows = 0, tiles = 0, outs = 0;
+    for (int i = 0; i < a.nlevels; ++i) {
+        const ScreenLevel &L = a.lv[i];
+        if (L.P != L.H * L.W || L.M != a.B * L.P || L.P < 1 || L.row_begin != rows || L.tile_begin != tiles) return false;
+        if ((long long)a.B * L.P * a.Cin * 4 >= (1LL << 31) || L.out_off != outs || (L.out_off & 7)) return false;
+        rows += L.M;
+        tiles += (L.M + 255) / 256;
+        outs += (long long)L.P * a.out_rstride;
+    }
+    return rows == a.rows_total && tiles == a.tiles_m && outs == a.out_bstride && tiles * a.NT <= 0x7fffffffLL;
+}
+
+hipError_t launch_logit_convert(const ScreenArgs &a, hipStream_t s)
+{
+    if (!screen_args_ok(a) || a.x_elems <= 0 || (a.x_elems & 7)) return hipErrorInvalidValue;
+    const long long n8 = a.x_elems / 8;
+    const long long nblk = (n8 + 255) / 256;
+    hipLaunchKernelGGL(logit_convert_kernel, dim3((unsigned)(nblk < 8192 ? nblk : 8192)), dim3(256), 0, s, a.x, a.x16, n8, a.counts, a.Cout / 8);
+    return hipGetLastError();
+}
+
+hipError_t launch_logit_screen(const ScreenArgs &a, hipStream_t s)
+{
+    if (!screen_args_ok(a)) return hipErrorInvalidValue;
+    constexpr int lds_bytes = 2 * (256 + 256) * 128;
+    static std::atomic<unsigned> attr_done{0};
+    hipError_t e = ssd_allow_lds((const void *)logit_screen_kernel, lds_bytes, attr_done);
+    if (e != hipSuccess) return e;
+    hipLaunchKernelGGL(logit_screen_kernel, dim3((unsigned)(a.tiles_m * a.NT)), dim3(256), lds_bytes, s, a);
+    return hipGetLastError();
+}
+
+hipError_t launch_logit_fill(const ScreenArgs &a, hipStream_t s)
+{
+    if (!screen_args_ok(a)) return hipErrorInvalidValue;
+    const long long nwords = ((long long)a.B * a.out_bstride / 8 + 31) / 32;
+    const long long cblk = (nwords + 255) / 256;
+    hipLaunchKernelGGL(logit_compact_kernel, dim3((unsigned)(cblk < 4096 ? cblk : 4096)), dim3(256), 0, s, a, nwords);
+    hipError_t e = hipGetLastError();
+    if (e != hipSuccess) return e;
+    const int lds_bytes = 9 * a.Cin * 8 * 4;
+    static std::atomic<unsigned> attr_done{0};
+    e = ssd_allow_lds((const void *)logit_fill_kernel, lds_bytes, attr_done);
+    if (e != hipSuccess) return e;
+    long long maxchunks = ((long long)a.rows_total + FILL_CHUNK - 1) / FILL_CHUNK * (a.Cout / 8);
+    static std::atomic<int> cu_count{0};
+    int cus = cu_count.load(std::memory_order_relaxed);
+    if (cus <= 0) {
+        int dev = 0;
+        cus = 256;
+        if (hipGetDevice(&dev) == hipSuccess) (void)hipDeviceGetAttribute(&cus, hipDeviceAttributeMultiprocessorCount, dev);
+        if (cus <= 0) cus = 256;
+        cu_count.store(cus, std::memory_order_relaxed);
+    }
+    const long long grid = maxchunks < 2LL * cus ? maxchunks : 2LL * cus;
+    hipLaunchKernelGGL(logit_fill_kernel, dim3((unsigned)grid), dim3(512), lds_bytes, s, a);
+    return hipGetLastError();
+}
diff --git a/single-shot-detector_amd/csrc/plan.hip b/single-shot-detector_amd/csrc/plan.hip
--- a/single-shot-detector_amd/csrc/plan.hip
+++ b/single-shot-detector_amd/csrc/plan.hip
@@ -776,6 +776,12 @@
     SSDCHK(ssd_anchors(b.H, b.W, anc.data()));
     float *anc_dev;
     SSDCHK(pl.pool.upload(&anc_dev, anc));
+    long long rows_total = 0;
+    for (int l = 0; l < 5; ++l) rows_total += (long long)B * py.h[l] * py.w[l];
+    const int scr_opt = ssd_opt(h, OPT_LOGITS_SCREEN, -1);
+    const bool screen = !b.X16 && scr_opt != 0 && ((long long)N * C) % 8 == 0 && (A * C) % 8 == 0 && A * C <= 8 * SCREEN_MAX_OCT &&
+                        h->final_[1].wscr && h->final_[1].scst && h->final_[1].CinP == 256 && h->final_[1].CoutP == A * C &&
+                        (scr_opt > 0 || rows_total >= SSD_SCREEN_MIN_ROWS);
     float *TAB[2][2];
     unsigned char *keys_home = nullptr;
     {
@@ -788,7 +794,7 @@
         }
         for (int t = 0; t < 2; ++t)
             for (int k = 0; k < 2; ++k) TAB[t][k] = (float *)(tb + (size_t)(2 * t + k) * slot);
-        if (post_keys_bytes(B, (int)N, C) <= tb_bytes) keys_home = tb;
+        if (post_keys_bytes(B, (int)N, C) <= tb_bytes && !screen) keys_home = tb;
     }
     void *ws;
     const size_t wsb = post_workspace_bytes(B, (int)N, C, h->cfg.max_boxes_per_class, keys_home == nullptr);
@@ -833,18 +839,67 @@
         bool marked = false;
         Op fop = make_conv_op(h, h->final_[t], io, B, 1, 1, SSD_ACT_NONE, lv, false, can_mark ? p.scan_bits : nullptr,
                               conservative_logit_bound(h->cfg.score_threshold), &marked);
+        if (t == 1 && screen) {
+            pl.logits_dense = make_conv_op(h, h->final_[t], io, B, 1, 1, SSD_ACT_NONE, lv, false);
+            pl.screened = true;
+            ScreenArgs sa;
+            memset(&sa, 0, sizeof(sa));
+            const ConvW &fc = h->final_[t];
+            sa.x = in;
+            sa.x16 = (unsigned short *)TAB[1][cur];
+            sa.w16 = fc.wscr; sa.wt = fc.wt; sa.bias = fc.bias; sa.cst = fc.scst;
+            sa.logits = logits; sa.bits = p.scan_bits;
+            SSDCHK(pl.pool.alloc((void **)&sa.counts, SCREEN_MAX_OCT * sizeof(int)));
+            SSDCHK(pl.pool.alloc((void **)&sa.lists, (size_t)(A * C / 8) * (size_t)rows_total * sizeof(int)));
+            HIPCHK(hipMemset(sa.counts, 0, SCREEN_MAX_OCT * sizeof(int)));
+            sa.lo = conservative_logit_bound(h->cfg.score_threshold);
+            sa.B = B; sa.Cin = fc.CinP; sa.Cout = fc.CoutP; sa.CoutPad = fc.CoutPad; sa.NT = (fc.CoutP + 127) / 128;
+            sa.nlevels = 5;
+            sa.out_rstride = A * C; sa.out_bstride = N * C;
+            sa.x_elems = py.total;
+            int rows = 0, tiles = 0;
+            for (int l = 0; l < 5; ++l) {
+                ScreenLevel &L = sa.lv[l];
+                L.H = py.h[l]; L.W = py.w[l]; L.P = L.H * L.W; L.M = B * L.P;
+                L.row_begin = rows; L.tile_begin = tiles;
+                L.in_off = py.off[l]; L.out_off = aoff[l] * C;
+                rows += L.M;
+                tiles += (L.M + 255) / 256;
+            }
+            sa.rows_total = rows; sa.tiles_m = tiles;
+            Op o;
+            o.cls = 4; o.flops = 0;
+            if (scr_opt == 2) {
+                const size_t lbytes = (size_t)B * N * C * sizeof(float);
+                o.bytes = (double)lbytes;
+                o.run = [logits, lbytes](hipStream_t s) { return hipMemsetAsync(logits, 0xff, lbytes, s); };
+                tower_ops[t].push_back(o);
+            }
+            o.bytes = (double)py.total * 6.0;
+            o.run = [sa](hipStream_t s) { return launch_logit_convert(sa, s); };
+            tower_ops[t].push_back(o);
+            o.bytes = (double)py.total * 2.0 + (double)fc.taps * sa.NT * 256 * fc.CinP * 2.0;
+            o.run = [sa](hipStream_t s) { return launch_logit_screen(sa, s); };
+            tower_ops[t].push_back(o);
+            o.bytes = (double)B * N * C / 64.0;
+            o.run = [sa](hipStream_t s) { return launch_logit_fill(sa, s); };
+            tower_ops[t].push_back(o);
+            continue;
+        }
         if (t == 1) all_marked = all_marked && marked;
         tower_ops[t].push_back(fop);
     }
     p.scan_fused = all_marked ? 1 : 0;
-    for (size_t i = 0; i < tower_ops[0].size(); ++i)
+    for (size_t i = 0; i < std::max(tower_ops[0].size(), tower_ops[1].size()); ++i)
         for (int t = 1; t >= 0; --t) {
+            if (i >= tower_ops[t].size()) continue;
             std::vector<int> deps;
             if (i == 0) { deps.push_back(t == 0 ? f.id_p4 : f.id_p3); deps.push_back(f.id_p7); }
             b.push(tower_ops[t][i], t, deps);
         }
     pl.retained["encoded_boxes"] = Retained{codes, B, 1, (int)N, 4, 4, false};
     pl.retained["class_predictions"] = Retained{logits, B, 1, (int)N, C, C, false};
+    pl.retained["class_logits_filled"] = Retained{logits, B, 1, (int)N, C, C, false};
     return SSD_OK;
 }
 
@@ -866,6 +921,15 @@
     for (const Op &op : pl.ops)
         for (int d : op.deps)
             if (!pl.ops[d].done) HIPCHK(hipEventCreateWithFlags(&pl.ops[d].done, ssd_sync_event_flags(h)));
+    return SSD_OK;
+}
+
+int materialize_logits(ssd_handle *h, Plan &pl, hipStream_t s)
+{
+    (void)h;
+    if (!pl.screened || pl.logits_whole) return SSD_OK;
+    HIPCHK(pl.logits_dense.run(s));
+    pl.logits_whole = true;
     return SSD_OK;
 }
 
@@ -1075,6 +1139,7 @@
     for (size_t k = 0; k < plans.size(); ++k) {
         Plan &pl = *plans[k];
         if (pl.need_begin) HIPCHK(hipEventRecord(pl.ev_begin, s));
+        if (pl.screened) pl.logits_whole = false;
         const bool single = ssd_opt(h, OPT_STREAMS, 0) == 1;
         bool used[4] = {true, false, false, false};
         for (const Op &op : pl.ops) {
diff --git a/single-shot-detector_amd/csrc/ssd_internal.h b/single-shot-detector_amd/csrc/ssd_internal.h
--- a/single-shot-detector_amd/csrc/ssd_internal.h
+++ b/single-shot-detector_amd/csrc/ssd_internal.h
@@ -99,6 +99,38 @@
 #define IGEMM16_TILE 100
 hipError_t launch_igemm16(const IgemmArgs &a, int total_tiles_m, hipStream_t s);
 
+#define SCREEN_MAX_LEVELS 5
+#define SCREEN_MAX_OCT 128
+struct ScreenLevel {
+    int H, W, P, M;
+    int row_begin;
+    int tile_begin;
+    long long in_off;
+    long long out_off;
+};
+struct ScreenArgs {
+    const float *x;
+    unsigned short *x16;
+    const unsigned short *w16;
+    const float *wt;
+    const float *bias;
+    const float *cst;
+    float *logits;
+    unsigned *bits;
+    int *counts;
+    int *lists;
+    float lo;
+    int B, Cin, Cout, CoutPad, NT;
+    int nlevels, tiles_m, rows_total;
+    int out_rstride;
+    long long out_bstride;
+    long long x_elems;
+    ScreenLevel lv[SCREEN_MAX_LEVELS];
+};
+hipError_t launch_logit_convert(const ScreenArgs &a, hipStream_t s);
+hipError_t launch_logit_screen(const ScreenArgs &a, hipStream_t s);
+hipError_t launch_logit_fill(const ScreenArgs &a, hipStream_t s);
+
 struct DwPwSArgs {
     const float *in;
     const float *dwpack;
diff --git a/single-shot-detector_amd/csrc/weights.hip b/single-shot-detector_amd/csrc/weights.hip
--- a/single-shot-detector_amd/csrc/weights.hip
+++ b/single-shot-detector_amd/csrc/weights.hip
@@ -83,8 +83,52 @@
     cw.Cout_l = Cout_l;
 }
 
+static int pack_screen(DevPool &pool, const std::vector<float> &t, const float *bias, ConvW &cw)
+{
+    const int NT = (cw.CoutP + 127) / 128, rows = NT * 256;
+    std::vector<uint16_t> s((size_t)cw.taps * rows * cw.CinP, 0);
+    std::vector<double> wn_sum(cw.CoutP, 0.0);
+    auto bits_of = [](_Float16 v) { uint16_t b; memcpy(&b, &v, 2); return b; };
+    for (int tap = 0; tap < cw.taps; ++tap)
+        for (int n = 0; n < cw.CoutP; ++n) {
+            const float *src = &t[((size_t)tap * cw.CoutPad + n) * cw.CinP];
+            uint16_t *dp = &s[((size_t)tap * rows + (n / 128) * 256 + n % 128) * cw.CinP], *dn = dp + (size_t)128 * cw.CinP;
+            for (int p = 0; p < cw.CinP; ++p) {
+                const float v = src[p];
+                if (v != v) { dp[p] = 0x7e00; continue; }
+                if (v > 0.0f) {
+                    const _Float16 hh = (_Float16)v;
+                    uint16_t b = bits_of(hh);
+                    if ((float)hh < v) b += 1;
+                    dp[p] = b < 0x0400 ? 0x0400 : b;
+                } else if (v < 0.0f) {
+                    const float m = -v;
+                    const _Float16 hh = (_Float16)m;
+                    uint16_t b = bits_of(hh);
+                    if ((float)hh > m) b -= 1;
+                    if (b >= 0x7c00) b = 0x7bff;
+                    if (b < 0x0400) b = 0;
+                    dn[p] = b;
+                    _Float16 back;
+                    memcpy(&back, &b, 2);
+                    wn_sum[n] += (double)(float)back;
+                }
+            }
+        }
+    std::vector<float> cst(cw.CoutP);
+    for (int n = 0; n < cw.CoutP; ++n) {
+        const double b = bias[n];
+        const double c = b + ldexp(wn_sum[n] * (1.0 + 1e-9), -14) + ldexp(fabs(b), -20) + 1e-30;
+        float f = (float)c;
+        if ((double)f < c) f = nextafterf(f, INFINITY);
+        cst[n] = f;
+    }
+    SSDCHK(pool.upload(&cw.wscr, s));
+    return pool.upload(&cw.scst, cst);
+}
+
 int pack_conv(const ssd_handle *h, DevPool &pool, const float *w, int k, int Cin_l, int Cout_l, const std::vector<int> &inmap,
-                     const std::vector<int> &outmap, ConvW &cw)
+                     const std::vector<int> &outmap, ConvW &cw, const float *screen_bias)
 {
     conv_geometry(h, k * k, (int)inmap.size(), (int)outmap.size(), Cin_l, Cout_l, cw);
     std::vector<float> t((size_t)cw.taps * cw.CoutPad * cw.CinP, 0.0f);
@@ -96,6 +140,7 @@
                 if (inmap[p] >= 0) dst[p] = w[((size_t)tap * Cin_l + inmap[p]) * Cout_l + outmap[n]];
         }
     SSDCHK(pool.upload(&cw.wt, t));
+    if (screen_bias && cw.taps == 9 && cw.CinP % 64 == 0 && cw.CoutP % 8 == 0 && cw.CoutP == Cout_l) SSDCHK(pack_screen(pool, t, screen_bias, cw));
     {
         const int KC = cw.CinP / 32, NT = cw.CoutPad / 16;
         std::vector<float> wl(t.size());
@@ -202,13 +247,13 @@
 }
 
 static int load_conv(ssd_handle *h, const std::string &wname, const std::string &bnscope, int k, int Cin, int Cout,
-                     ConvW &cw, bool out_identity = false, int in_split = 0)
+                     ConvW &cw, bool out_identity = false, int in_split = 0, const float *screen_bias = nullptr)
 {
     const Tensor *w = getvar(h, wname, {k, k, Cin, Cout});
     if (!w) return SSD_ERR_WEIGHT;
     std::vector<int> inmap = in_split > 0 ? twopart_map(in_split, round_up(in_split, 32)) : phys_map(Cin, round_up(Cin, 32));
     std::vector<int> outmap = out_identity ? ident_map(Cout, Cout) : phys_map(Cout, round_up(Cout, 32));
-    SSDCHK(pack_conv(h, h->wpool, w->data.data(), k, Cin, Cout, inmap, outmap, cw));
+    SSDCHK(pack_conv(h, h->wpool, w->data.data(), k, Cin, Cout, inmap, outmap, cw, out_identity ? screen_bias : nullptr));
     if (!bnscope.empty()) {
         BnHost b;
         SSDCHK(get_bn(h, bnscope, Cout, outmap, b));
@@ -383,9 +428,9 @@
         const int Cout = t == 0 ? 4 * A : C * A;
         const std::string scope = std::string(nets[t]) + (t == 0 ? "/encoded_boxes" : "/logits");
         ConvW &cw = h->final_[t];
-        SSDCHK(load_conv(h, scope + "/kernel", "", 3, 256, Cout, cw, true));
         const Tensor *bias = getvar(h, scope + "/bias", {Cout});
         if (!bias) return SSD_ERR_WEIGHT;
+        SSDCHK(load_conv(h, scope + "/kernel", "", 3, 256, Cout, cw, true, 0, t == 1 ? bias->data.data() : nullptr));
         std::vector<float> bpad(bias->data);
         bpad.resize((size_t)round_up(Cout, 4), 0.0f);
         SSDCHK(h->wpool.upload(&cw.bias, bpad));
diff --git a/single-shot-detector_amd/evaluation.py b/single-shot-detector_amd/evaluation.py
--- a/single-shot-detector_amd/evaluation.py
+++ b/single-shot-detector_amd/evaluation.py
@@ -34,6 +34,7 @@
     def __init__(self, engine):
         self.engine = engine
         self.anchors = {}
+        engine.set_option("logits_screen", 0)
 
     def anchors_for(self, shape):
         a = self.anchors.get(shape)
diff --git a/single-shot-detector_amd/ssd.py b/single-shot-detector_amd/ssd.py
--- a/single-shot-detector_amd/ssd.py
+++ b/single-shot-detector_amd/ssd.py
@@ -847,6 +847,7 @@
         self.num_classes = engine.params["num_classes"] if num_classes is None else num_classes
         if self.num_classes != engine.params["num_classes"]:
             raise ValueError("num_classes differs from the engine's configuration")
+        engine.set_option("logits_screen", 0)
 
     def __call__(self, image_features):
         B = image_features[0].shape[0]
```

Result: faster. 871.3, median of 6 (+7.0%).
